# gradientpm/gvpm

Hardware: AMD Instinct MI355X
Metric: photon gather+shift evaluations per second (G-BRE 3D) (higher is better)
Workload: dtype f32; 1 GPU; BASELINE configs[1]: S-cbox + homogeneous medium, G-BRE 3D kernel, 512x512 frame, 1000000 photons/iter, 227 SPPM iters, initialScaleVolume 1.0; technique=bre3d, scene=cbox, photons_per_iter=1000000

## Files before the change

### gvpm_amd/csrc/build_chain.hip

```cpp
#include <hip/hip_runtime.h>

#include <algorithm>

#include "bundle_grid.h"
#include "device_types.h"
#include "shift_device.h"
#include "tile_walk.h"
#include "vec.h"
#include "grid_cells.h"
#include "photon_scatter.h"
#include "scan_block.h"

namespace gvpm {

__device__ __forceinline__ bool lastBlockArrives(uint32_t *ctl, uint32_t blockId, uint32_t nblocks) {
  __shared__ uint32_t isLast;
  asm volatile("s_waitcnt vmcnt(0)" ::: "memory");
  __syncthreads();
  if (threadIdx.x == 0) {
    const uint32_t S = nblocks < 64u ? nblocks : 64u;
    const uint32_t sl = blockId % S;
    const uint32_t expect = (nblocks - sl + S - 1u) / S;
    uint32_t last = 0u;
    if (atomicAdd(&ctl[1u + sl], 1u) == expect - 1u) {
      atomicExch(&ctl[1u + sl], 0u);
      if (atomicAdd(&ctl[0], 1u) == S - 1u) {
        atomicExch(&ctl[0], 0u);
        last = 1u;
      }
    }
    isLast = last;
  }
  __syncthreads();
  return isLast != 0u;
}
__device__ __forceinline__ uint32_t coherentRead(uint32_t *p) { return atomicAdd(p, 0u); }

__device__ __forceinline__ uint32_t ordCode(float f) {
  const uint32_t u = __float_as_uint(f);
  return (u >> 31) ? ~u : (u | 0x80000000u);
}
__device__ __forceinline__ float ordDecode(uint32_t o) { return __uint_as_float((o >> 31) ? (o & 0x7FFFFFFFu) : ~o); }
__global__ void chain_init_buckets_kernel(uint32_t *buckets) {
  const uint32_t t = threadIdx.x;
  buckets[t] = (t % 6u) < 3u ? 0xFFFFFFFFu : 0u;
}

__global__ __launch_bounds__(256) void chain_count_kernel(ChainArgs c) {
  __shared__ float red[6][4];
  const uint32_t b = blockIdx.x;
  if (b == 0) {
    if (threadIdx.x < 8) c.queueCtl[threadIdx.x] = 0u;
    if (threadIdx.x == 8) *c.overflowCtr = 0u;
    if (threadIdx.x == 9) c.nearExt[0] = 1u;
  }
  float mn[3] = {INFINITY, INFINITY, INFINITY}, mx[3] = {-INFINITY, -INFINITY, -INFINITY};
  const bool photons = b < c.nPhBlocks;
  if (photons) {
    const uint32_t i = b * 256u + threadIdx.x;
    if (i < c.n) {
      const float px = c.pos[3 * (size_t)i + 0], py = c.pos[3 * (size_t)i + 1], pz = c.pos[3 * (size_t)i + 2];
      mn[0] = px; mn[1] = py; mn[2] = pz;
      mx[0] = px; mx[1] = py; mx[2] = pz;
      const Grid &g = c.g;
      if (g.mode == 1) {
        const uint32_t k = bundlePhotonKey(g, px, py, pz);
        c.keys[i] = k;
        if (k == GVPM_BUNDLE_DUMP_CELL(g.dim[0])) {
          c.rank[i] = 0xFFFFFFFFu;
        } else {
          c.rank[i] = 0u;
          (void)atomicAdd(&c.sub[(size_t)(i % CELL_STRIPES) * g.ncells + k], 1u);
        }
      } else {
        const int cx = cellCoord(px, g.org[0], g.invCell, g.dim[0]);
        const int cy = cellCoord(py, g.org[1], g.invCell, g.dim[1]);
        const int cz = cellCoord(pz, g.org[2], g.invCell, g.dim[2]);
        const uint32_t k = ((uint32_t)cz * g.dim[1] + cy) * g.dim[0] + cx;
        c.keys[i] = k;
        (void)atomicAdd(&c.counts[k], 1u);
      }
    }
  } else {
    const uint32_t i = (b - c.nPhBlocks) * 256u + threadIdx.x;
    if (i < c.nsets) {
      const gvpm_camera_ray &r = c.rays[(size_t)i * 5];
      const uint32_t px = r.pixel & 0xFFFFu, py = r.pixel >> 16;
      const uint32_t tilesX = (c.width + c.tw - 1) / c.tw;
      const uint32_t tile = (py / c.th) * tilesX + px / c.tw;
      const uint32_t inTile = (py % c.th) * c.tw + px % c.tw;
      const uint32_t k = tile * (uint32_t)(c.tw * c.th) + inTile;
      c.bKeys[i] = k;
      (void)atomicAdd(&c.counts[(size_t)c.beamOff + k], 1u);
      if (GVPM_RAY_VALID(r.info)) {
#pragma unroll
        for (int k3 = 0; k3 < 3; ++k3) {
          const float e0 = r.o[k3], e1 = r.o[k3] + r.d[k3] * r.len;
          mn[k3] = fminf(e0, e1);
          mx[k3] = fmaxf(e0, e1);
        }
      }
    }
  }
  const int wave = threadIdx.x / 64, lane = threadIdx.x % 64;
#pragma unroll
  for (int k = 0; k < 3; ++k) {
    const float lo = wave_min(mn[k]), hi = wave_max(mx[k]);
    if (lane == 0) {
      red[k][wave] = lo;
      red[3 + k][wave] = hi;
    }
  }
  __syncthreads();
  if (threadIdx.x < 6) {
    const int k = threadIdx.x;
    float v = red[k][0];
    for (int w = 1; w < 4; ++w) v = k < 3 ? fminf(v, red[k][w]) : fmaxf(v, red[k][w]);
    uint32_t *slot = c.buckets + (photons ? 0u : 384u) + (b % 64u) * 6u + k;
    if (k < 3) (void)atomicMin(slot, ordCode(v));
    else (void)atomicMax(slot, ordCode(v));
  }
}

__global__ __launch_bounds__(256) void chain_stripes_kernel(const uint32_t *__restrict__ sub, uint32_t *__restrict__ prefix, uint32_t ncells,
                                                            uint32_t *__restrict__ count) {
  const uint32_t k = blockIdx.x * blockDim.x + threadIdx.x;
  if (k >= ncells) return;
  uint32_t run = 0;
#pragma unroll
  for (uint32_t st = 0; st < CELL_STRIPES; ++st) {
    prefix[(size_t)st * ncells + k] = run;
    run += sub[(size_t)st * ncells + k];
  }
  count[k] = run;
}

__global__ __launch_bounds__(256) void chain_scan_reduce_kernel(ChainArgs c) {
  __shared__ uint32_t lds[4];
  __shared__ float red[6][4];
  const uint32_t n = c.scanLen;
  {
    const uint32_t *__restrict__ counts = c.counts;
    const uint32_t base = blockIdx.x * SCAN_TILE + threadIdx.x * SCAN_PER_THREAD;
    uint32_t v = 0;
#pragma unroll
    for (uint32_t k = 0; k < SCAN_PER_THREAD; ++k)
      if (base + k < n) v += counts[base + k];
    uint32_t total;
    (void)block_scan_excl(v, lds, total);
    if (threadIdx.x == 0) (void)atomicExch(&c.blockSum[blockIdx.x], total);
  }
  if (!lastBlockArrives(c.ctl, blockIdx.x, gridDim.x)) return;
  const uint32_t nblocks = gridDim.x;
  const uint32_t per = (nblocks + SCAN_BLOCK - 1u) / SCAN_BLOCK;
  const uint32_t i0 = min(nblocks, threadIdx.x * per), i1 = min(nblocks, i0 + per);
  uint32_t mine = 0;
  for (uint32_t i = i0; i < i1; ++i) mine += coherentRead(&c.blockSum[i]);
  uint32_t total;
  uint32_t run = block_scan_excl(mine, lds, total);
  for (uint32_t i = i0; i < i1; ++i) {
    const uint32_t v = coherentRead(&c.blockSum[i]);
    c.blockSum[i] = run;
    run += v;
  }
  for (uint32_t which = 0; which < 2u; ++which) {
    float v6[6];
#pragma unroll
    for (int k = 0; k < 6; ++k) {
      float v = k < 3 ? INFINITY : -INFINITY;
      if (threadIdx.x < 64u) {
        uint32_t *slot = c.buckets + which * 384u + threadIdx.x * 6u + k;
        v = ordDecode(coherentRead(slot));
        *slot = k < 3 ? 0xFFFFFFFFu : 0u;
      }
      v6[k] = v;
    }
    const int wave = threadIdx.x / 64, lane = threadIdx.x % 64;
    __syncthreads();
#pragma unroll
    for (int k = 0; k < 3; ++k) {
      const float a = wave_min(v6[k]), b = wave_max(v6[3 + k]);
      if (lane == 0) {
        red[k][wave] = a;
        red[3 + k][wave] = b;
      }
    }
    __syncthreads();
    if (threadIdx.x < 6) {
      const int k = threadIdx.x;
      float v = red[k][0];
      for (int w = 1; w < 4; ++w) v = k < 3 ? fminf(v, red[k][w]) : fmaxf(v, red[k][w]);
      c.out6[which * 6u + k] = v;
      if (c.hostB6) c.hostB6[which * 16u + k] = v;
    }
  }
}

__global__ __launch_bounds__(256) void chain_scan_down_kernel(ChainArgs c) {
  __shared__ uint32_t lds[4];
  const uint32_t n = c.scanLen;
  uint32_t *__restrict__ counts = c.counts;
  uint32_t *__restrict__ starts = c.starts;
  const uint32_t zeroBelow = c.g.mode == 1 ? c.beamOff : 0u;
  const uint32_t base = blockIdx.x * SCAN_TILE + threadIdx.x * SCAN_PER_THREAD;
  uint32_t x[SCAN_PER_THREAD], v = 0;
#pragma unroll
  for (uint32_t k = 0; k < SCAN_PER_THREAD; ++k) {
    x[k] = base + k < n ? counts[base + k] : 0u;
    v += x[k];
  }
  uint32_t total;
  uint32_t run = c.blockSum[blockIdx.x] + block_scan_excl(v, lds, total);
#pragma unroll
  for (uint32_t k = 0; k < SCAN_PER_THREAD; ++k) {
    if (base + k < n) {
      starts[base + k] = run;
      if (x[k] && base + k < zeroBelow) counts[base + k] = 0u;
    }
    run += x[k];
  }
}

__global__ __launch_bounds__(256) void chain_mid_kernel(ChainArgs c, uint32_t nSatBlocks, uint32_t nBeamBlocks) {
  const uint32_t b = blockIdx.x;
  if (b < nSatBlocks) {
    satYBody(c.starts, c.g, c.sat, b * 256u + threadIdx.x);
    return;
  }
  const uint32_t *__restrict__ starts = c.starts;
  const uint32_t base = starts[c.beamOff];
  if (b < nSatBlocks + nBeamBlocks) {
    const uint32_t i = (b - nSatBlocks) * 256u + threadIdx.x;
    if (i < c.nsets) {
      const size_t k = (size_t)c.beamOff + c.bKeys[i];
      c.setPerm[starts[k] - base + (atomicSub(&c.counts[k], 1u) - 1u)] = i;
    }
    return;
  }
  const uint32_t t = (b - nSatBlocks - nBeamBlocks) * 256u + threadIdx.x;
  if (t <= c.ntiles) c.tileStart[t] = starts[(size_t)c.beamOff + ((size_t)t << c.tileShift)] - base;
}

struct TailArgs {
  uint32_t ntiles, target, itemCap, nPlan;
  uint4 *items;
  uint2 *itemOff;
  uint32_t *itemCount, *blockTotal;
  RawPhotons raw;
  const uint32_t *keys, *rank, *cellStart, *sub;
  uint32_t *counts;
  uint32_t *subCount;
  uint32_t n, ncells, extCap;
  uint32_t every;
  float dmax;
  NearGrid ng;
  uint32_t *nearExt, *overflow, *origIdx;
  float4 *hot, *cold;
  uint32_t *ctl;
  const uint32_t *bundleFlag;
  uint32_t *hostOut;
  uint32_t pairCapBlocks;
  uint32_t unitCap, unitPairs;
  uint32_t fullVis;
  uint32_t planGroups;
};
constexpr uint32_t TAIL_PLAN_STAGE = 128;
template <int B> constexpr size_t tailLdsBytes() {
  constexpr size_t pl = sizeof(PlanLds<B, TAIL_PLAN_STAGE>) > sizeof(PlanLdsQ<B, TAIL_PLAN_STAGE>) ? sizeof(PlanLds<B, TAIL_PLAN_STAGE>)
                                                                                                  : sizeof(PlanLdsQ<B, TAIL_PLAN_STAGE>);
  return pl > sizeof(ReorderLds) ? pl : sizeof(ReorderLds);
}
constexpr int TAIL_WPE = 6;
template <int B, int MODE> __global__ __launch_bounds__(64) __attribute__((amdgpu_waves_per_eu(TAIL_WPE, TAIL_WPE))) void chain_tail_kernel(GatherArgs a, TailArgs t) {
  __shared__ __attribute__((aligned(16))) unsigned char ldsRaw[tailLdsBytes<B>()];
  const uint32_t b = blockIdx.x, pslot = b / t.every;
  if (b % t.every == 0u && pslot < t.nPlan) {
    if (a.grid.mode != 1 && t.planGroups)
      planBodyQ<B, TAIL_PLAN_STAGE>(a, t.ntiles, t.target, t.items, t.itemCount, t.itemOff, t.blockTotal, t.itemCap, pslot, t.nPlan,
                                    *reinterpret_cast<PlanLdsQ<B, TAIL_PLAN_STAGE> *>(ldsRaw));
    else
      planBody<B, TAIL_PLAN_STAGE>(a, t.ntiles, t.target, t.items, t.itemCount, t.itemOff, t.blockTotal, t.itemCap, pslot, t.nPlan,
                                   *reinterpret_cast<PlanLds<B, TAIL_PLAN_STAGE> *>(ldsRaw));
  }
  else
    reorderBody<MODE>(t.raw, t.keys, t.rank, t.cellStart, t.n, a.cfg, a.bvh, a.tri4, a.ntri, t.dmax, t.ng, t.nearExt, t.extCap, t.hot,
                      t.cold, t.overflow, t.origIdx, t.sub, t.ncells, b - min(t.nPlan, (b + t.every - 1u) / t.every), t.counts,
                      t.subCount, *reinterpret_cast<ReorderLds *>(ldsRaw));
  if (!lastBlockArrives(t.ctl, blockIdx.x, gridDim.x)) return;
  if (threadIdx.x == 0) {
    t.hostOut[0] = coherentRead(t.blockTotal);
    t.hostOut[1] = coherentRead(t.overflow);
    t.hostOut[2] = coherentRead(t.nearExt);
    t.hostOut[3] = coherentRead(t.itemCount);
    t.hostOut[4] = t.bundleFlag ? coherentRead(const_cast<uint32_t *>(t.bundleFlag)) : 0u;
    uint32_t bad = 0u;
    if (t.pairCapBlocks != 0xFFFFFFFFu) {
      const uint32_t blocks = t.hostOut[0], nIt = t.hostOut[3];
      if (blocks > t.pairCapBlocks) bad |= 1u;
      if (nIt > t.itemCap) bad |= 2u;
      if (t.unitCap && (unsigned long long)blocks * 64ull / t.unitPairs + nIt + 64ull > (unsigned long long)t.unitCap) bad |= 4u;
      if (t.hostOut[1] != 0u && !t.fullVis) bad |= 8u;
      if (t.hostOut[4] != 0u) bad |= 16u;
    }
    t.itemCount[7] = bad;
    t.hostOut[5] = bad;
    __threadfence_system();
  }
}

template <int B>
static void launchTail(int mode, uint32_t grid, hipStream_t s, const GatherArgs &a, const TailArgs &t) {
  if (mode == 0) hipLaunchKernelGGL((chain_tail_kernel<B, 0>), dim3(grid), dim3(64), 0, s, a, t);
  else if (mode == 2) hipLaunchKernelGGL((chain_tail_kernel<B, 2>), dim3(grid), dim3(64), 0, s, a, t);
  else hipLaunchKernelGGL((chain_tail_kernel<B, 1>), dim3(grid), dim3(64), 0, s, a, t);
}

void launch_build_chain(ChainArgs c, const GatherArgs &a, const gvpm_photon_soa &raw, int beamsPerWave, uint32_t target, uint4 *items,
                        uint2 *itemOff, uint32_t itemCap, float dmax, const NearGrid &ng, uint32_t extCap, uint32_t *origIdx,
                        uint32_t *hostOut, bool initBuckets, hipStream_t s, uint32_t pairCapBlocks, uint32_t unitCap, uint32_t unitPairs,
                        bool fullVis, bool planGroups) {
  c.nPhBlocks = (c.n + 255u) / 256u;
  c.nBeamBlocks = (c.nsets + 255u) / 256u;
  if (initBuckets) hipLaunchKernelGGL(chain_init_buckets_kernel, dim3(1), dim3(768), 0, s, c.buckets);
  hipLaunchKernelGGL(chain_count_kernel, dim3(c.nPhBlocks + c.nBeamBlocks), dim3(256), 0, s, c);
  if (c.g.mode == 1)
    hipLaunchKernelGGL(chain_stripes_kernel, dim3((c.g.ncells + 255) / 256), dim3(256), 0, s, c.sub, c.sub + (size_t)CELL_STRIPES * c.g.ncells,
                       c.g.ncells, c.counts);
  const uint32_t nScan = (c.scanLen + SCAN_TILE - 1) / SCAN_TILE;
  hipLaunchKernelGGL(chain_scan_reduce_kernel, dim3(nScan), dim3(SCAN_BLOCK), 0, s, c);
  hipLaunchKernelGGL(chain_scan_down_kernel, dim3(nScan), dim3(SCAN_BLOCK), 0, s, c);
  const uint32_t nx1 = c.g.dim[0] + 1;
  const uint32_t nSat = (nx1 * (uint32_t)c.g.dim[2] + 255u) / 256u, nTile = (c.ntiles + 1u + 255u) / 256u;
  hipLaunchKernelGGL(chain_mid_kernel, dim3(nSat + c.nBeamBlocks + nTile), dim3(256), 0, s, c, nSat, c.nBeamBlocks);
  launch_sat_z(c.g, c.sat, s);
  TailArgs t{};
  t.ntiles = c.ntiles;
  t.target = target;
  t.itemCap = itemCap;
  t.planGroups = planGroups ? 1u : 0u;
  {
    const uint32_t per = (t.planGroups && c.g.mode != 1) ? (uint32_t)(64 / (beamsPerWave > 0 ? beamsPerWave : 16)) : 1u;
    const uint32_t want = (c.ntiles + per - 1u) / per;
    t.nPlan = want < 4093u ? std::max(1u, want) : 4093u;
    (void)per;
  }
  t.items = items;
  t.itemOff = itemOff;
  t.itemCount = c.queueCtl;
  t.blockTotal = c.queueCtl + 3;
  t.raw = rawOf(raw);
  t.keys = c.keys;
  t.rank = c.rank;
  t.cellStart = c.starts;
  t.sub = c.g.mode == 1 ? c.sub + (size_t)CELL_STRIPES * c.g.ncells : nullptr;
  t.subCount = c.g.mode == 1 ? c.sub : nullptr;
  t.counts = c.g.mode == 1 ? nullptr : c.counts;
  t.n = c.n;
  t.ncells = c.g.ncells;
  t.extCap = extCap;
  t.dmax = dmax;
  t.ng = ng;
  t.nearExt = c.nearExt;
  t.overflow = c.overflowCtr;
  t.origIdx = origIdx;
  t.hot = const_cast<float4 *>(a.hot);
  t.cold = const_cast<float4 *>(a.cold);
  t.ctl = c.ctl + 65;
  t.bundleFlag = a.bundleFlag;
  t.hostOut = hostOut;
  t.pairCapBlocks = pairCapBlocks;
  t.unitCap = unitCap;
  t.unitPairs = unitPairs ? unitPairs : 1u;
  t.fullVis = fullVis ? 1u : 0u;
  const int mode = a.ntri <= 64u ? 0 : (ng.start ? 2 : 1);
  const uint32_t grid = t.nPlan + (c.n + 63u) / 64u;
  t.every = std::max(1u, grid / std::max(1u, t.nPlan));
  switch (beamsPerWave) {
    case 64: launchTail<64>(mode, grid, s, a, t); break;
    case 32: launchTail<32>(mode, grid, s, a, t); break;
    default: launchTail<16>(mode, grid, s, a, t); break;
  }
}

}
```

### gvpm_amd/csrc/context.h

```cpp
#pragma once
#include <dlfcn.h>
#include <hip/hip_runtime.h>
#include <rccl/rccl.h>

#include <cmath>
#include <cstdio>
#include <cstdlib>
#include <cstring>
#include <algorithm>
#include <chrono>
#include <string>
#include <type_traits>
#include <vector>

#include "device_types.h"
#include "scan_sort.h"
#include "scene_bvh.h"

namespace gvpm {
void launch_bounds(const float *pos, uint32_t n, float *partial, int nblocks, float *out6, float *hostOut,
                   hipStream_t s, const uint32_t *word = nullptr, uint32_t *wordOut = nullptr);
void launch_export_u32(const uint32_t *a, const uint32_t *b, const uint32_t *c, const uint32_t *d, const uint32_t *e, uint32_t *hostOut,
                       hipStream_t s);
uint32_t cell_stripes();
void launch_cell_count(const float *pos, uint32_t n, const Grid &g, uint32_t *keys, uint32_t *rank, uint32_t *count, uint32_t *sub,
                       hipStream_t s, uint32_t *zeroWord = nullptr, uint32_t *oneWord = nullptr);
void launch_sat(const uint32_t *cellStart, const Grid &g, uint32_t *sat, hipStream_t s);
void launch_reorder(const gvpm_photon_soa &raw, const uint32_t *keys, const uint32_t *rank, const uint32_t *cellStart,
                    uint32_t n, const gvpm_params &cfg, const float4 *bvh, const float4 *tri4, uint32_t ntri, float dmax,
                    const NearGrid &ng, uint32_t *nearExt, uint32_t extCap, float4 *hot, float4 *cold, uint32_t *overflow,
                    uint32_t *origIdx, const uint32_t *sub, uint32_t ncells, hipStream_t s);
void launch_near_grid(const float4 *tri4, uint32_t ntri, const NearGrid &g, float reach, uint32_t *counts, uint32_t *tris, int mode,
                      hipStream_t s);
void launch_segment_start(const uint32_t *keys, uint32_t n, uint32_t nseg, uint32_t shift, uint32_t *start,
                          hipStream_t s);
void launch_bundle_fit(const gvpm_camera_ray *rays, uint32_t nsets, int pass, const Grid &g, double *out, hipStream_t s);
void launch_beam_keys(const gvpm_camera_ray *rays, uint32_t nsets, int width, int tw, int th, uint32_t *keys,
                      uint32_t *vals, hipStream_t s);
void launch_beam_count(const gvpm_camera_ray *rays, uint32_t nsets, int width, int tw, int th, uint32_t *keys,
                       uint32_t *rank, uint32_t *count, hipStream_t s);
void launch_beam_scatter(const uint32_t *keys, const uint32_t *rank, const uint32_t *start, uint32_t n,
                         uint32_t *setPerm, hipStream_t s);
void launch_tile_start(const uint32_t *start, uint32_t ntiles, uint32_t shift, uint32_t *tileStart, hipStream_t s);
void launch_beam_cold(const gvpm_photon_soa &raw, const float *endN, uint32_t n, const gvpm_params &cfg,
                      const uint32_t *subCounts, float4 *cold, float4 *aux, hipStream_t s);
void launch_shift_extent(const gvpm_camera_ray *rays, uint32_t nsets, uint32_t *extentBits, hipStream_t s);
void launch_beam_near(float4 *cold, uint32_t n, const float4 *tri4, uint32_t ntri, float r, float eps, const uint32_t *extentBits, float2 *clear, bool freeCone,
                      hipStream_t s);
void launch_beam_near_hist(const float4 *cold, uint32_t n, uint32_t ntri, uint32_t *hist, hipStream_t s);
void launch_build_chain(ChainArgs c, const GatherArgs &a, const gvpm_photon_soa &raw, int beamsPerWave, uint32_t target, uint4 *items,
                        uint2 *itemOff, uint32_t itemCap, float dmax, const NearGrid &ng, uint32_t extCap, uint32_t *origIdx,
                        uint32_t *hostOut, bool initBuckets, hipStream_t s, uint32_t pairCapBlocks = 0xFFFFFFFFu, uint32_t unitCap = 0,
                        uint32_t unitPairs = 1, bool fullVis = false, bool planGroups = true);
void launch_apply_host_shifts(const GatherArgs &a, const gvpm_host_shift *results, uint32_t n, hipStream_t s);
void launch_plan_bre(const GatherArgs &a, int beamsPerWave, uint32_t ntiles, uint32_t target, uint4 *items,
                     uint32_t *itemCount, uint2 *itemOff, uint32_t *blockTotal, uint32_t itemCap, hipStream_t stream);
uint32_t eval_unit_pairs();
void launch_traverse_bre(const GatherArgs &a, int beamsPerWave, const uint4 *items, const uint2 *itemOff,
                         const uint32_t *itemCount, uint32_t *queueHead, uint32_t *pairs, uint32_t *pairCnt,
                         uint32_t nwaves, bool persistent, hipStream_t stream, uint2 *units = nullptr, uint32_t *unitCtl = nullptr,
                         uint32_t unitCap = 0);
void launch_evaluate_primal(const GatherArgs &a, int beamsPerWave, const uint4 *items, const uint2 *itemOff,
                            const uint32_t *itemCount, uint32_t *queueHead, const uint32_t *pairs, const uint32_t *pairCnt,
                            uint32_t nwaves, hipStream_t stream);
void launch_evaluate_bre(const GatherArgs &a, int beamsPerWave, bool fullVis, const uint4 *items, const uint2 *itemOff,
                         const uint32_t *itemCount, uint32_t *queueHead, const uint32_t *pairs, const uint32_t *pairCnt,
                         uint32_t nwaves, bool persistent, hipStream_t stream, const uint2 *units = nullptr,
                         const uint32_t *unitCtl = nullptr, uint32_t unitCap = 0);
uint32_t plan_items_capacity(uint32_t nsets, uint32_t ntiles, int beamsPerWave);
void launch_exact_pass(const GatherArgs &a, unsigned long long *totals, uint32_t *hostOut, hipStream_t s);
void launch_capture_notes(const GatherArgs &a, hipStream_t s, uint32_t nblocks = 256);
void launch_apply_host_shifts_beams(const GatherArgs &a, const gvpm_host_shift *results, uint32_t n, hipStream_t s);
void launch_exact_beams(const GatherArgs &a, unsigned long long *totals, hipStream_t s);
void launch_beam_subcount(const float *p2, const float *p1, uint32_t n, float ls, uint32_t *counts, uint32_t *maxLs,
                          hipStream_t s);
void launch_beam_expand(const float *p2, const float *p1, uint32_t n, const uint32_t *counts, const uint32_t *offsets,
                        const Grid &g, uint32_t *keys, uint32_t *vals, hipStream_t s);
void launch_sub_hot(const uint32_t *sortedIds, uint32_t n, const float4 *aux, float4 *hot, uint32_t *hotFlags, hipStream_t s);
void launch_evaluate_beams(const GatherArgs &a, int beamsPerWave, bool exact, const uint2 *pairs, const uint32_t *sortedKey,
                           const uint32_t *sortedBlock, uint32_t nBlocks, uint32_t *queueHead, uint32_t nwaves,
                           hipStream_t stream);
void launch_traverse_beams(const GatherArgs &a, const uint32_t *hotFlags, int beamsPerWave, const uint4 *items,
                           const uint32_t *itemCount, uint32_t itemCap, uint32_t *queueHead, uint2 *pairs, uint32_t *pairCount,
                           uint32_t pairCap, uint32_t *blockKey, uint32_t *blockVal, uint32_t nwaves, hipStream_t stream);
void launch_evaluate_beams_split(const GatherArgs &a, uint32_t *qId, uint32_t *qMeta, float4 *qK, float *qU, uint32_t *blkCnt,
                                 uint4 *runTab, uint32_t *ctl, const uint2 *pairs, const uint32_t *sortedKey,
                                 const uint32_t *sortedBlock, uint32_t nBlocks, uint32_t *queueHead, uint32_t ncu,
                                 hipStream_t stream);
void launch_gather_vpm(const GatherArgs &a, bool fullVis, bool primal, hipStream_t stream);
void launch_vpm_find(const GatherArgs &a, const VpmSplit &sp, hipStream_t stream);
void launch_vpm_redo(const GatherArgs &a, const VpmSplit &sp, bool fullVis, uint32_t nwaves, hipStream_t stream);
void launch_vpm_eval(const GatherArgs &a, const VpmSplit &sp, bool fullVis, uint32_t wavesPerShard, hipStream_t stream);
void launch_vpm_finish(float *accum, float *iter, float *scaleVol, float *nVol, float *mvol, size_t n, float alpha,
                       uint32_t *maxScaleBits, hipStream_t stream);
void launch_accumulate(float *accum, float *iter, size_t n, uint32_t *zeroWord, hipStream_t stream);
struct PlaneArgs {
  const float4 *test;
  const float *ori, *end, *flux, *w1, *len1;
  const uint32_t *flags;
  uint32_t nplanes, planesPerItem;
};
void launch_plane_records(const PlaneArgs &pa, float4 *out, hipStream_t stream);
void launch_gather_planes(const GatherArgs &a, const PlaneArgs &pa, uint32_t ntiles, uint32_t nchunks,
                          hipStream_t stream);
void launch_finalize(float *accum, const float *iter, size_t n, int it, uint64_t nbPaths, hipStream_t s);
void launch_scale(const float *in, float *out, size_t n, float scale, hipStream_t s);
void launch_film(const float *acc, const float *emission, int w, int h, int it, int reusePrimal, float invDiv,
                 float *thr, float *dx, float *dy, hipStream_t s);
struct PoissonGraphCache {
  hipGraph_t graph = nullptr;
  hipGraphExec_t exec = nullptr;
  void *scratch = nullptr;
  int W = 0, H = 0, cgMax = 0;
  float alpha = 0.f;
};
void poisson_graph_release(PoissonGraphCache &c);
hipError_t poisson_solve_device(const gvpm_poisson_params &prm, int W, int H, const float *dx, const float *dy,
                                const float *tp, const float *direct, float *out, void *scratch,
                                PoissonGraphCache &cache, hipStream_t s);
size_t poisson_scratch_bytes(int W, int H);
}

using namespace gvpm;

template <typename T> struct DevBuf {
  T *p = nullptr;
  size_t cap = 0;
  hipError_t ensure(size_t n) {
    if (n <= cap) return hipSuccess;
    if (p) (void)hipFree(p);
    p = nullptr;
    cap = 0;
    size_t want = n + n / 2 + 64;
    hipError_t e = hipMalloc((void **)&p, want * sizeof(T));
    if (e == hipSuccess) cap = want;
    return e;
  }
  void release() {
    if (p) (void)hipFree(p);
    p = nullptr;
    cap = 0;
  }
  hipError_t reserveExact(size_t c) {
    if (c <= cap) return hipSuccess;
    if (p) (void)hipFree(p);
    p = nullptr;
    cap = 0;
    hipError_t e = hipMalloc((void **)&p, c * sizeof(T));
    if (e == hipSuccess) cap = c;
    return e;
  }
};

constexpr int PHOTON_ARRAYS = 14;
constexpr size_t PHOTON_WORDS = 30;
static inline size_t photonArrayWords(int k) { return k < 8 ? 3 : 1; }
template <typename Soa, typename F> static inline void forEachPhotonArray(Soa &s, F &&f) {
  int k = 0;
  auto each = [&](auto &...a) { (f(k++, a), ...); };
  each(s.pos, s.wi, s.flux, s.parent_pos, s.parent_n, s.prefix_w, s.parent_scat, s.parent_wi, s.parent_pdf, s.edge_pdf, s.parent_rr,
       s.parent_g, s.flags, s.path_id);
}
struct PhotonArrayPtrs {
  const void *p[PHOTON_ARRAYS];
  explicit PhotonArrayPtrs(const gvpm_photon_soa &s) {
    forEachPhotonArray(s, [&](int k, const auto *a) { p[k] = a; });
  }
};
static inline void photonArraysInBlock(gvpm_photon_soa &s, const uint32_t *base, uint64_t n) {
  forEachPhotonArray(s, [&](int k, auto &a) {
    a = reinterpret_cast<std::remove_reference_t<decltype(a)>>(base);
    base += (size_t)n * photonArrayWords(k);
  });
  s.n = n;
}

struct RcclApi {
  void *dl = nullptr;
  decltype(&ncclGetUniqueId) getUniqueId = nullptr;
  decltype(&ncclCommInitRank) commInitRank = nullptr;
  decltype(&ncclAllReduce) allReduce = nullptr;
  decltype(&ncclCommDestroy) commDestroy = nullptr;
  bool load() {
    if (dl) return true;
    dl = dlopen("librccl.so.1", RTLD_NOW | RTLD_LOCAL);
    if (!dl) dl = dlopen("librccl.so", RTLD_NOW | RTLD_LOCAL);
    if (!dl) return false;
    getUniqueId = (decltype(getUniqueId))dlsym(dl, "ncclGetUniqueId");
    commInitRank = (decltype(commInitRank))dlsym(dl, "ncclCommInitRank");
    allReduce = (decltype(allReduce))dlsym(dl, "ncclAllReduce");
    commDestroy = (decltype(commDestroy))dlsym(dl, "ncclCommDestroy");
    return getUniqueId && commInitRank && allReduce && commDestroy;
  }
};
extern RcclApi g_rccl;

#define GVPM_PHASES 3
enum : uint32_t { TRACE_HOST = 1u, TRACE_PLAN = 2u, TRACE_VIS = 4u, TRACE_EXACT = 8u, TRACE_BEAMS = 16u };

struct BuildSet {
  float builtRadius = -1.f;
  DevBuf<float4> hot, cold;
  DevBuf<uint32_t> overflowCtr;
  DevBuf<uint32_t> origIdx;
  DevBuf<uint32_t> cellStart, cellCount, cellSub, sat, keysA, keysB, valsA, valsB;
  DevBuf<uint32_t> beamCount, beamStart;
  DevBuf<float> boundsPartial, bounds6;
  Grid grid;
  SortTemp sortTmp;
  DevBuf<uint32_t> bKeysA, bKeysB, bValsA, setPerm, tileStart;
  uint32_t ntiles = 0;
  int tileW = 4, tileH = 4;
  bool scanSized = false, scanSizedChain = false;
  bool countsClean = false;
  size_t subCleanWords = 0;
  DevBuf<uint32_t> chainBuckets;
  bool bucketsInit = false;
  DevBuf<uint4> items;
  DevBuf<uint2> itemOff;
  DevBuf<uint2> planBoxes;
  DevBuf<uint32_t> queueCtl;
  DevBuf<uint32_t> pairs, pairCnt, nearExt;
  DevBuf<uint2> units;
  DevBuf<uint4> notes;
  DevBuf<uint32_t> notesCount;
  hipEvent_t traversed = nullptr;
  hipEvent_t lastUse = nullptr;
  bool used = false;
  bool lastUseValid = false;
  hipError_t mirrorFrom(const BuildSet &o) {
    hipError_t e = hipSuccess;
#define GVPM_MIRROR(X) if (e == hipSuccess) e = X.reserveExact(o.X.cap)
    GVPM_MIRROR(hot); GVPM_MIRROR(cold); GVPM_MIRROR(overflowCtr); GVPM_MIRROR(origIdx); GVPM_MIRROR(cellStart); GVPM_MIRROR(cellCount); GVPM_MIRROR(cellSub);
    GVPM_MIRROR(sat); GVPM_MIRROR(keysA); GVPM_MIRROR(keysB); GVPM_MIRROR(valsA); GVPM_MIRROR(valsB);
    GVPM_MIRROR(beamCount); GVPM_MIRROR(beamStart); GVPM_MIRROR(boundsPartial); GVPM_MIRROR(bounds6);
    GVPM_MIRROR(bKeysA); GVPM_MIRROR(bKeysB); GVPM_MIRROR(bValsA); GVPM_MIRROR(setPerm); GVPM_MIRROR(tileStart);
    GVPM_MIRROR(items); GVPM_MIRROR(itemOff); GVPM_MIRROR(planBoxes); GVPM_MIRROR(queueCtl); GVPM_MIRROR(pairs); GVPM_MIRROR(pairCnt);
    GVPM_MIRROR(nearExt); GVPM_MIRROR(chainBuckets); GVPM_MIRROR(units);
#undef GVPM_MIRROR
    return e;
  }
  void release() {
    hot.release(); cold.release(); overflowCtr.release(); origIdx.release(); cellStart.release(); cellCount.release(); cellSub.release(); sat.release();
    beamCount.release(); beamStart.release(); keysA.release(); keysB.release();
    valsA.release(); valsB.release(); boundsPartial.release(); bounds6.release(); bKeysA.release(); bKeysB.release();
    bValsA.release(); setPerm.release(); tileStart.release(); items.release(); itemOff.release(); planBoxes.release(); queueCtl.release();
    if (sortTmp.d) (void)hipFree(sortTmp.d);
    sortTmp.d = nullptr;
    sortTmp.bytes = 0;
    pairs.release(); pairCnt.release(); nearExt.release(); chainBuckets.release(); units.release(); notes.release(); notesCount.release();
    if (lastUse) (void)hipEventDestroy(lastUse);
    if (traversed) (void)hipEventDestroy(traversed);
    lastUse = traversed = nullptr;
  }
};

struct gvpm_context {
  int device = 0;
  hipStream_t stream = nullptr;
  hipStream_t streamB = nullptr;
  hipStream_t bstream = nullptr;
  hipStream_t streamC = nullptr;
  hipStream_t streamA2 = nullptr;
  bool travStream = true;
  BuildSet sets[3];
  BuildSet *bs = &sets[0];
  int setIdx = 0;
  bool beamsExact = false;
  bool bundleEnabled = false;
  bool bundleFromEnv = false;
  bool bundleAuto = false;
  int bundleState = 0, bundleViolations = 0;
  int lastGridMode = 0;
  uint32_t lastGridCells = 0;
  float bundleDiv = 2.f;
  Grid bundleGrid{};
  bool buildChain = true;
  DevBuf<uint32_t> chainCtl;
  bool planGroups = true;
  bool planBoxHandOff = true;
  bool beamsFreeCone = true;
  size_t beamPairsInit = (size_t)16 << 20;
  uint32_t beamItemsInit = 0;
  uint32_t beamItemCap = 0;
  bool pipeline = true;
  uint32_t trace = 0;
  gvpm_params cfg;
  gvpm_medium medium;
  bool haveMedium = false;
  std::string err;

  DevBuf<float4> tri4, bvh;
  uint32_t ntri = 0;
  float triMin[3] = {0, 0, 0}, triMax[3] = {0, 0, 0};
  DevBuf<uint32_t> nearGridStart, nearGridTris, nearGridCount;
  NearGrid nearGrid;
  float nearGridReach = -1.f;
  bool useNearGrid = true;

  struct PhotonSlot {
    DevBuf<uint32_t> raw;
    gvpm_photon_soa dev;
    DevBuf<uint32_t> packed;
    bool needUnpack = false;
    bool linked = false;
    hipEvent_t unpacked = nullptr;
    hipEvent_t copied = nullptr;
    hipEvent_t consumed = nullptr, consumedB = nullptr;
    bool read = false;
    int side = 0;
    DevBuf<float> endN, w1, len1;
    DevBuf<uint32_t> endNOct;
    bool octNormals = false;
  };
  enum : int { SIDE_NONE = 0, SIDE_BEAMS = 1, SIDE_PLANES = 2 };
  struct RaySlot {
    DevBuf<gvpm_camera_ray> rays;
    DevBuf<uint32_t> packed;
    DevBuf<uint32_t> compact;
    uint32_t ncompact = 0;
    bool needUnpack = false;
    hipEvent_t unpacked = nullptr;
    uint32_t nsets = 0;
    hipEvent_t copied = nullptr, freed = nullptr;
    bool read = false;
  };
  struct SampleSlot {
    DevBuf<gvpm_vpm_sample> smp;
    DevBuf<uint32_t> packed;
    uint32_t n = 0, nruns = 0;
    bool needUnpack = false;
    hipEvent_t unpacked = nullptr;
    hipEvent_t copied = nullptr, freed = nullptr;
    bool read = false;
  };
  template <typename Slot> struct StagingRing {
    Slot slot[3];
    int cur = 0, pending = -1;
    bool wait = false;
    bool ownedCur = false;
    bool fresh = false;
  };
  StagingRing<PhotonSlot> ph;
  StagingRing<RaySlot> ray;
  StagingRing<SampleSlot> smp;
  hipStream_t copyStream = nullptr;
  uint64_t reqCap = 0;
  DevBuf<gvpm_shift_request> reqHost;
  DevBuf<float4> reqCtx;
  DevBuf<uint32_t> reqCount;
  DevBuf<gvpm_host_shift> reqResults;
  DevBuf<ExEntry> exPay;
  DevBuf<uint32_t> exPayCount;
  DevBuf<uint4> exOvf;
  DevBuf<uint32_t> exOvfCount;
  bool iterClean = false;
  DevBuf<unsigned long long> exTotals;
  uint32_t exPayCap = 1u << 17;
  uint32_t exOvfCap = 1u << 20;
  uint32_t exSince = 0;
  uint32_t exFlushEvery = 8;
  bool exFlushFixed = false;
  uint32_t exSinceAtLast = 8;
  uint32_t *pinExact = nullptr;
  bool reqOutstanding = false;
  bool reqBeams = false;
  GatherArgs reqArgs;
  DevBuf<gvpm_material> materials;
  uint32_t nmaterials = 0;
  std::vector<gvpm_material> materialsHost;
  DevBuf<float4> bsdfs;
  uint32_t nbsdfs = 0;
  bool bsdfMixtures = false;
  gvpm_sensor sensor{};
  bool haveSensor = false;
  gvpm_photon_soa rawDev;
  uint32_t nph = 0;
  gvpm_photon_soa gatheredPh{};
  const gvpm_camera_ray *gatheredRays = nullptr;
  uint32_t gatheredSets = 0;
  bool haveGathered = false;
  int gatheredSide = 0;
  const float *gatheredEndN = nullptr, *gatheredW1 = nullptr, *gatheredLen1 = nullptr;
  const gvpm_vpm_sample *gatheredSamples = nullptr;
  uint32_t gatheredNSamples = 0;
  bool gatheredVpm = false;
  bool havePhotons = false, photonsDirty = false;
  bool nearOverflow = false;
  size_t nearExtWant = 0;
  float cachedB6[6] = {0, 0, 0, 0, 0, 0};
  bool haveCachedBounds = false, boundsPending = false;
  float beamB6[6] = {0, 0, 0, 0, 0, 0};
  bool haveBeamBounds = false, clipGrid = true;
  float *pinB6 = nullptr;
  uint32_t *pinCtl = nullptr;
  uint32_t vpmOrderN = 0;
  uint32_t vpmLaunches = 0;
  bool vpmNoOrder = false;
  float vpmScaleBound = 0.f;
  bool vpmPipeline = true;
  bool vpmSplit = true;
  uint32_t vpmPoolPerBatch = 4;
  uint32_t vpmRedoWaves = 256;
  uint32_t vpmEvalWaves = 12288;
  DevBuf<uint2> vpmPairs, vpmChunkMeta;
  DevBuf<uint32_t> vpmCtl, vpmStatus, vpmRedo;
  DevBuf<VpmSampleState> vpmState;
  hipEvent_t vpmFound = nullptr, vpmRedone = nullptr;
  bool beamsSplit = false;
  DevBuf<uint32_t> splitId, splitMeta, splitBlkCnt, splitCtl;
  DevBuf<float4> splitK;
  DevBuf<float> splitU;
  DevBuf<uint4> splitRuns;
  float *pinBeams = nullptr;

  const gvpm_camera_ray *raysDev = nullptr;
  uint32_t nsets = 0;
  bool haveBeams = false, beamsDirty = false;

  const float *endNDev = nullptr;
  bool haveBeamsMap = false;
  DevBuf<uint32_t> subCounts, subOffsets, beamCtl;
  DevBuf<float4> beamAux;
  DevBuf<float2> beamClear;
  uint32_t nsub = 0;
  float subLen = 0.f, maxSubLen = 0.f;

  const float *w1Dev = nullptr, *len1Dev = nullptr;
  DevBuf<float4> planeTest;
  DevBuf<uint32_t> subFlags;
  DevBuf<uint32_t> shiftExtent;
  bool beamNearStale = true;
  DevBuf<uint32_t> blockKeyA, blockKeyB, blockValA, blockValB;
  DevBuf<uint2> beamPairs;
  bool havePlanes = false;

  const gvpm_vpm_sample *samplesDev = nullptr;
  uint32_t nsamples = 0;
  bool haveSamples = false;
  DevBuf<float> scaleVol, nVol, mvol;
  DevBuf<uint32_t> maxScaleBits;
  double totalEmitted = 0;

  DevBuf<float> accum, accumAll, iter, filmOut, emission;
  bool useAll = false;
  size_t npix = 0;
  float globalScaleVolume = 1.f;
  bool sumMode = false;
  int sumIt = 0;
  DevBuf<float> accumTmp;

  DevBuf<unsigned long long> stats;
  std::vector<std::pair<hipEvent_t, hipEvent_t>> events[GVPM_PHASES];
  size_t eventsHead[GVPM_PHASES] = {0, 0, 0};
  size_t eventsCount[GVPM_PHASES] = {0, 0, 0};

  int beamsPerWave = 16;
  float cellScale = 0.f;
  uint32_t planTarget = 1536;
  bool planTargetSet = false;
  uint32_t nwaves = 2048;
  bool nwavesFromEnv = false;
  uint32_t ncu = 256;
  uint32_t nwavesTrav = 4096;
  bool persistentEval = true, persistentTrav = false;
  bool optimistic = true;
  uint32_t lastItems = 0;
  uint32_t optRefuseEvery = 0, optSteps = 0, optRefused = 0;
  bool evalUnits = true;

  DevBuf<float> poissonScratch, poissonIO;
  PoissonGraphCache poissonGraph;

  ncclComm_t comm = nullptr;
};

#define CHECK_H(h)                                \
  if (!(h)) return GVPM_ERR_INVALID_ARG;          \
  if (hipSetDevice((h)->device) != hipSuccess) {  \
    (h)->err = "hipSetDevice failed";             \
    return GVPM_ERR_HIP;                          \
  }

#define HIP_TRY(h, expr)                                                                      \
  do {                                                                                        \
    hipError_t _e = (expr);                                                                   \
    if (_e != hipSuccess) {                                                                   \
      (h)->err = std::string(#expr) + ": " + hipGetErrorString(_e);                           \
      return GVPM_ERR_HIP;                                                                    \
    }                                                                                         \
  } while (0)

static inline int fail(gvpm_context *h, int code, const char *msg) {
  if (h) h->err = msg;
  return code;
}


namespace gvpm {
void launch_unpack_photons(const uint32_t *packed, uint32_t n, const gvpm_material *table, uint32_t table_n,
                           const gvpm_photon_soa &dst, unsigned long long *bad, hipStream_t s);
void launch_unpack_rays(const uint32_t *packed, uint32_t nsets, gvpm_camera_ray *dst, hipStream_t s);
void launch_unpack_linked(const uint32_t *blob, uint32_t n, const gvpm_material *table, uint32_t table_n, const gvpm_photon_soa &dst,
                          unsigned long long *bad, hipStream_t s);
void launch_unpack_compact_rays(const gvpm_sensor &sensor, const uint32_t *compact, uint32_t ncompact, gvpm_camera_ray *dst,
                                hipStream_t s);
void launch_unpack_normals_oct(const uint32_t *codes, uint32_t n, float *dst, hipStream_t s);
void launch_expand_vpm_runs(const uint32_t *packed, uint32_t nruns, uint32_t n, gvpm_vpm_sample *dst, hipStream_t s);
}

int gvpm_join_exact(gvpm_context *h);
int joinEvalStreams(gvpm_context *h);
int flushHostShifts(gvpm_context *h);
float currentRadius(const gvpm_context *h);
```

### gvpm_amd/csrc/drivers_bre.hip

```cpp
#include "drivers.h"

namespace {

struct BreStep {
  gvpm_context *h;
  int it;
  uint64_t nbPaths;
  bool primal;
  float r;
  EventPair *evBuild = nullptr, *evTrav = nullptr, *evEval = nullptr;
  GatherArgs a;
  uint32_t itemCap = 0;
  uint32_t blocks = 0, nItems = 0;
  ChainPrep cp;
  int attempt = 0;
  bool force3D = false;
  bool rebuilt = false;
  bool chainRan = false;
  bool queued = false;
  bool prevOverflow = false;
  std::chrono::steady_clock::time_point T0;

  void lap(const char *what) {
    if (!(h->trace & TRACE_HOST)) return;
    auto t = std::chrono::steady_clock::now();
    fprintf(stderr, "[host] it=%d %-10s %8.1f us\n", it, what, std::chrono::duration<double, std::micro>(t - T0).count());
    T0 = t;
  }
  bool threeStage() const { return h->pipeline && h->travStream; }
};

int foldRunningSum(gvpm_context *h, int it) {
  h->sumMode = true;
  if (h->sumIt != 0 && it - 1 != h->sumIt) {
    const int rc = gvpm_join_exact(h);
    if (rc != GVPM_OK) return rc;
    launch_scale(h->accum.p, h->accum.p, h->npix * 27, (float)((double)(it - 1) / (double)h->sumIt), h->stream);
  }
  h->sumIt = it;
  return GVPM_OK;
}

int buildOrWait(BreStep &s) {
  gvpm_context *h = s.h;
  s.rebuilt = false;
  s.cp = ChainPrep{};
  if (h->photonsDirty || h->beamsDirty || s.r != h->bs->builtRadius) {
    h->setIdx = (h->setIdx + 1) % (s.threeStage() ? 3 : 2);
    h->bs = &h->sets[h->setIdx];
    if (h->bs->used) HIP_TRY(h, hipStreamWaitEvent(h->bstream, h->bs->lastUse, 0));
    HIP_TRY(h, hipEventRecord(s.evBuild->first, h->bstream));
    s.lap("waitevent");
    {
      int tileShift;
      uint32_t ntilesAll;
      beamTiling(h, h->beamsPerWave, s.cp.tw, s.cp.th, ntilesAll, tileShift);
      tileShift -= 3;
      const uint64_t nkeys = (uint64_t)ntilesAll << tileShift;
      s.cp.on = h->buildChain && h->nph > 0 && h->nsets > 0 && nkeys <= 0x3FFFFFF0ull;
      s.cp.nkeys = (uint32_t)nkeys;
      s.cp.tileShift = (uint32_t)tileShift;
    }
    GridBuild how;
    how.deferred = true;
    how.force3D = s.force3D;
    how.chain = &s.cp;
    int rc = buildGrid(h, s.r, how);
    s.lap("buildGrid");
    if (rc == GVPM_OK) rc = sortBeams(h, 0, &s.cp);
    s.lap("sortBeams");
    if (rc != GVPM_OK) return rc;
    h->photonsDirty = false;
    h->beamsDirty = false;
    h->bs->builtRadius = s.r;
    s.rebuilt = h->nph > 0;
  } else {
    if (h->bs->used) HIP_TRY(h, hipStreamWaitEvent(h->bstream, h->bs->lastUse, 0));
    if (h->bs->used && s.threeStage()) HIP_TRY(h, hipStreamWaitEvent(h->streamC, h->bs->lastUse, 0));
    HIP_TRY(h, hipEventRecord(s.evBuild->first, h->bstream));
  }
  return GVPM_OK;
}

int sizeItemsAndBoxes(BreStep &s) {
  gvpm_context *h = s.h;
  GatherArgs &a = s.a;
  fillArgs(h, a, s.r);
  a.iter = h->accum.p;
  a.iterScale = 1.0f / (float)s.nbPaths;
  if (!a.cfg.reserved[1] && h->cellScale <= 0.f && h->nph <= 2000000u) a.cfg.reserved[1] = 8;
  s.itemCap = plan_items_capacity(h->nsets, h->bs->ntiles, h->beamsPerWave);
  HIP_TRY(h, h->bs->items.ensure(s.itemCap));
  HIP_TRY(h, h->bs->itemOff.ensure(s.itemCap));
  if (h->planBoxHandOff) {
    const Grid &g = h->bs->grid;
    const int kmin = std::max(1, std::min(a.cfg.reserved[2] ? a.cfg.reserved[2] : 8, a.cfg.reserved[1] ? a.cfg.reserved[1] : 6));
    const uint32_t stride = (uint32_t)(std::max(386, std::max(g.dim[0], std::max(g.dim[1], g.dim[2]))) / kmin + 2);
    const size_t chunks = (size_t)h->nsets / (size_t)h->beamsPerWave + h->bs->ntiles + 2;
    if (chunks < (1u << 24) && std::max(g.dim[0], std::max(g.dim[1], g.dim[2])) < 1024) {
      HIP_TRY(h, h->bs->planBoxes.ensure(chunks * stride));
      a.planBoxes = h->bs->planBoxes.p;
      a.planBoxStride = stride;
    }
  }
  HIP_TRY(h, h->bs->queueCtl.ensure(8));
  a.bundleFlag = h->bs->queueCtl.p + 4;
  return ensurePinned(h);
}

int queueGather(BreStep &s, uint32_t blocks, uint32_t nItems, bool optimistic, bool fullVis) {
  gvpm_context *h = s.h;
  GatherArgs &a = s.a;
  const bool primal = s.primal;
  if (!optimistic) {
    HIP_TRY(h, h->bs->pairs.ensure((size_t)blocks * 64u + 64u));
    HIP_TRY(h, h->bs->pairCnt.ensure((size_t)s.itemCap * h->beamsPerWave));
  }
  int rc = nextEvents(h, &s.evTrav, 1);
  if (rc == GVPM_OK) rc = nextEvents(h, &s.evEval, 0);
  if (rc != GVPM_OK) return rc;
  const hipStream_t ts = !h->pipeline ? h->stream : (h->travStream ? h->streamC : h->streamB), es = h->stream;
  uint2 *units = nullptr;
  uint32_t unitCap = 0;
  if (h->evalUnits && h->persistentEval && !primal) {
    if (optimistic) {
      unitCap = (uint32_t)std::min<size_t>(h->bs->units.cap / 2u, 0x3FFFFFFFu);
      units = unitCap ? h->bs->units.p : nullptr;
    } else {
      const uint64_t capU = (uint64_t)blocks * 64u / eval_unit_pairs() + nItems + 64u;
      if (capU < 0x3FFFFFFFull) {
        HIP_TRY(h, h->bs->units.ensure((size_t)capU * 2u));
        unitCap = (uint32_t)std::min<size_t>(h->bs->units.cap / 2u, 0x3FFFFFFFu);
        units = h->bs->units.p;
      }
    }
  }
  if (!primal) {
    if (!h->bs->notes.p) {
      HIP_TRY(h, h->bs->notes.reserveExact(h->exOvfCap));
      HIP_TRY(h, h->bs->notesCount.ensure(4));
      HIP_TRY(h, hipMemsetAsync(h->bs->notesCount.p, 0, 4 * sizeof(uint32_t), es));
    }
    a.exOvf = h->bs->notes.p;
    a.exOvfCount = h->bs->notesCount.p;
    a.exOvfCap = h->exOvfCap;
  }
  if (optimistic && ts != h->bstream) HIP_TRY(h, hipStreamWaitEvent(ts, s.evBuild->second, 0));
  HIP_TRY(h, hipEventRecord(s.evTrav->first, ts));
  launch_traverse_bre(a, h->beamsPerWave, h->bs->items.p, h->bs->itemOff.p, h->bs->queueCtl.p, h->bs->queueCtl.p + 1,
                      h->bs->pairs.p, h->bs->pairCnt.p, h->persistentTrav ? h->nwavesTrav : nItems, h->persistentTrav || optimistic, ts,
                      units, h->bs->queueCtl.p + 5, unitCap);
  HIP_TRY(h, hipEventRecord(s.evTrav->second, ts));
  HIP_TRY(h, hipEventRecord(h->bs->traversed, ts));
  HIP_TRY(h, hipStreamWaitEvent(es, h->bs->traversed, 0));
  const bool smallShare = h->nsets > 0 && (size_t)h->nsets * 6u <= h->npix;
  const uint32_t nwEval = (h->pipeline && !h->nwavesFromEnv && h->ncu && h->nph > 2000000u && !smallShare)
                              ? std::min<uint32_t>(h->ncu * 12u, GVPM_STAT_ROWS) : h->nwaves;
  if (!primal && h->reqCap > 0 && h->cfg.use_manifold && h->bs->origIdx.p) {
    rc = armHostShiftRequests(h, a, 4, true, a.iter, a.iterScale, false, es);
    if (rc != GVPM_OK) return rc;
  }
  HIP_TRY(h, hipEventRecord(s.evEval->first, es));
  if (primal)
    launch_evaluate_primal(a, h->beamsPerWave, h->bs->items.p, h->bs->itemOff.p, h->bs->queueCtl.p, h->bs->queueCtl.p + 2,
                           h->bs->pairs.p, h->bs->pairCnt.p, std::max<uint32_t>(1u, std::min<uint32_t>(nItems, h->ncu * 16u)), es);
  else
    launch_evaluate_bre(a, h->beamsPerWave, fullVis, h->bs->items.p, h->bs->itemOff.p, h->bs->queueCtl.p,
                        h->bs->queueCtl.p + 2, h->bs->pairs.p, h->bs->pairCnt.p, h->persistentEval ? nwEval : nItems, h->persistentEval,
                        es, units, h->bs->queueCtl.p + 5, unitCap);
  HIP_TRY(h, hipEventRecord(s.evEval->second, es));
  if (!primal) launch_capture_notes(a, es);
  HIP_TRY(h, hipEventRecord(h->bs->lastUse, es));
  h->bs->lastUseValid = true;
  if (!primal) return exactAfterGather(h);
  return GVPM_OK;
}

int launchBuildAndPlan(BreStep &s) {
  gvpm_context *h = s.h;
  const ChainPrep &cp = s.cp;
  if (cp.on && s.rebuilt) {
    if (!h->chainCtl.p) {
      HIP_TRY(h, h->chainCtl.ensure(192));
      HIP_TRY(h, hipMemsetAsync(h->chainCtl.p, 0, h->chainCtl.cap * sizeof(uint32_t), h->bstream));
    }
    ChainArgs c{};
    c.pos = h->rawDev.pos;
    c.n = h->nph;
    c.g = h->bs->grid;
    c.keys = h->bs->keysA.p;
    c.rank = h->bs->valsA.p;
    c.counts = h->bs->cellCount.p;
    c.starts = h->bs->cellStart.p;
    c.beamOff = h->bs->grid.ncells + 1u;
    c.scanLen = c.beamOff + cp.nkeys + 1u;
    c.sub = cp.sub;
    HIP_TRY(h, h->bs->chainBuckets.ensure(768));
    c.buckets = h->bs->chainBuckets.p;
    c.out6 = h->bs->bounds6.p;
    c.hostB6 = h->pinB6;
    c.rays = h->raysDev;
    c.nsets = h->nsets;
    c.width = h->cfg.width;
    c.tw = cp.tw;
    c.th = cp.th;
    c.tileShift = cp.tileShift;
    c.ntiles = h->bs->ntiles;
    c.bKeys = h->bs->bKeysA.p;
    c.bRank = h->bs->bValsA.p;
    c.setPerm = h->bs->setPerm.p;
    c.tileStart = h->bs->tileStart.p;
    c.blockSum = reinterpret_cast<uint32_t *>(h->bs->sortTmp.d);
    c.ctl = h->chainCtl.p;
    c.queueCtl = h->bs->queueCtl.p;
    c.overflowCtr = h->bs->overflowCtr.p;
    c.nearExt = h->bs->nearExt.p;
    c.sat = h->bs->sat.p;
    h->boundsPending = h->haveCachedBounds;
    const bool optimistic = h->optimistic && h->pipeline && s.attempt == 0 && !s.primal && h->persistentEval && h->lastItems > 0 &&
                            h->bs->pairs.cap >= 128u && h->bs->pairCnt.cap >= (size_t)s.itemCap * h->beamsPerWave &&
                            (!h->evalUnits || h->bs->units.cap >= 2u);
    const bool fullVisOpt = !h->cfg.visibility_as_written || s.prevOverflow;
    const bool refuse = optimistic && h->optRefuseEvery > 0 && (++h->optSteps % h->optRefuseEvery) == 0;
    launch_build_chain(c, s.a, h->rawDev, h->beamsPerWave, h->planTarget, h->bs->items.p, h->bs->itemOff.p, s.itemCap, cp.dmax, h->nearGrid,
                       (uint32_t)std::min<size_t>(h->bs->nearExt.cap, 0xFFFFFF00u), cp.wantOrig ? h->bs->origIdx.p : nullptr, h->pinCtl,
                       !h->bs->bucketsInit, h->bstream,
                       optimistic ? (refuse ? 0u : (uint32_t)std::min<size_t>((h->bs->pairs.cap - 64u) / 64u, 0xFFFFFFF0u)) : 0xFFFFFFFFu,
                       optimistic && h->evalUnits ? (uint32_t)std::min<size_t>(h->bs->units.cap / 2u, 0x3FFFFFFFu) : 0u, eval_unit_pairs(),
                       fullVisOpt, h->planGroups);
    h->bs->bucketsInit = true;
    s.chainRan = true;
    if (optimistic) {
      HIP_TRY(h, hipEventRecord(s.evBuild->second, h->bstream));
      const uint32_t guess = std::min<uint32_t>(s.itemCap, h->lastItems + h->lastItems / 8u + 256u);
      const int rc = queueGather(s, 0u, guess, true, fullVisOpt);
      if (rc != GVPM_OK) return rc;
      s.queued = true;
    }
  } else {
    HIP_TRY(h, hipMemsetAsync(h->bs->queueCtl.p, 0, 8 * sizeof(uint32_t), h->bstream));
    launch_plan_bre(s.a, h->beamsPerWave, h->bs->ntiles, h->planTarget, h->bs->items.p, h->bs->queueCtl.p, h->bs->itemOff.p,
                    h->bs->queueCtl.p + 3, s.itemCap, h->bstream);
    launch_export_u32(h->bs->queueCtl.p + 3, s.rebuilt ? h->bs->overflowCtr.p : nullptr, s.rebuilt ? h->bs->nearExt.p : nullptr,
                      h->bs->queueCtl.p, h->bs->queueCtl.p + 4, h->pinCtl, h->bstream);
  }
  if (!s.queued) HIP_TRY(h, hipEventRecord(s.evBuild->second, h->bstream));
  s.lap("plan");
  return GVPM_OK;
}

int readCounters(BreStep &s, bool &retry) {
  gvpm_context *h = s.h;
  retry = false;
  HIP_TRY(h, hipStreamSynchronize(h->bstream));
  s.lap("syncB");
  s.blocks = h->pinCtl[0];
  s.nItems = h->pinCtl[3];
  if (s.queued && h->pinCtl[5] != 0u) {
    if (h->trace & TRACE_PLAN) fprintf(stderr, "[plan] optimistic step refused by the build (status %u): queued again\n", h->pinCtl[5]);
    HIP_TRY(h, hipStreamSynchronize(h->stream));
    if (s.threeStage()) HIP_TRY(h, hipStreamSynchronize(h->streamC));
    HIP_TRY(h, hipMemsetAsync(h->bs->queueCtl.p + 1, 0, 2 * sizeof(uint32_t), h->bstream));
    HIP_TRY(h, hipMemsetAsync(h->bs->queueCtl.p + 5, 0, 3 * sizeof(uint32_t), h->bstream));
    HIP_TRY(h, hipStreamSynchronize(h->bstream));
    s.queued = false;
    h->optRefused++;
  }
  if (s.a.grid.mode == 1 && h->pinCtl[4] != 0u && s.attempt == 0) {
    h->bundleState = ++h->bundleViolations > 3 ? -1 : 0;
    h->photonsDirty = true;
    h->boundsPending = false;
    s.force3D = true;
    retry = true;
  }
  return GVPM_OK;
}

int recordBuild(BreStep &s) {
  gvpm_context *h = s.h;
  h->lastGridMode = s.a.grid.mode;
  h->lastGridCells = s.a.grid.ncells;
  if (s.nItems > s.itemCap) return fail(h, GVPM_ERR_STATE, "G-BRE planner produced more work items than its bound");
  if (h->trace & TRACE_PLAN) {
    uint32_t q[4] = {0, 0, 0, 0};
    (void)hipMemcpy(q, h->bs->queueCtl.p, sizeof(q), hipMemcpyDeviceToHost);
    fprintf(stderr, "[plan] items %u staged blocks %u tiles %u sets %u; photons %u, %s %d x %d x %d cells of %g (radius %g)\n", q[0],
            s.blocks, h->bs->ntiles, h->nsets, h->nph, h->bs->grid.mode == 1 ? "bundle cells" : "grid", h->bs->grid.dim[0],
            h->bs->grid.dim[1], h->bs->grid.dim[2], (double)h->bs->grid.cell, (double)s.r);
  }
  if (s.rebuilt) {
    h->nearOverflow = h->cfg.visibility_as_written && h->pinCtl[1] != 0;
    h->nearExtWant = std::max<size_t>(h->nearExtWant, (size_t)h->pinCtl[2] + h->pinCtl[2] / 4);
    if (h->trace & TRACE_VIS)
      fprintf(stderr, "[vis] ntri %u photons %u: %u lists overflowed, extension cursor %u of %zu, fullvis %d\n", h->ntri, h->nph,
              h->pinCtl[1], h->pinCtl[2], h->bs->nearExt.cap, (int)needFullVis(h));
  }
  if (h->boundsPending) {
    h->boundsPending = false;
    for (int c = 0; c < 6; ++c)
      if (!std::isfinite(h->pinB6[c])) return fail(h, GVPM_ERR_INVALID_ARG, "non-finite photon position");
    memcpy(h->cachedB6, h->pinB6, sizeof(h->cachedB6));
  }
  if (s.rebuilt && s.chainRan) {
    bool ok = true;
    for (int c = 0; c < 6; ++c) ok = ok && std::isfinite(h->pinB6[16 + c]);
    h->haveBeamBounds = ok;
    if (ok) memcpy(h->beamB6, h->pinB6 + 16, sizeof(h->beamB6));
  }
  h->lastItems = s.nItems;
  return GVPM_OK;
}

int mirrorSets(gvpm_context *h) {
  if (h->pipeline) {
    for (int k = 0; k < (h->travStream ? 3 : 2); ++k) {
      BuildSet &other = h->sets[k];
      if (&other != h->bs && !other.used && !h->bs->used) HIP_TRY(h, other.mirrorFrom(*h->bs));
    }
  }
  h->bs->used = true;
  return GVPM_OK;
}

int buildAndPlan(BreStep &s) {
  gvpm_context *h = s.h;
  const BuildStreamGuard onBuildStream(h, h->pipeline ? h->streamB : h->stream);
  int rc = foldRunningSum(h, s.it);
  if (rc == GVPM_OK) rc = exactPrepare(h);
  for (s.attempt = 0; rc == GVPM_OK && s.attempt < 2; ++s.attempt) {
    bool retry = false;
    rc = buildOrWait(s);
    if (rc == GVPM_OK) rc = sizeItemsAndBoxes(s);
    if (rc == GVPM_OK) rc = launchBuildAndPlan(s);
    if (rc == GVPM_OK) rc = readCounters(s, retry);
    if (!retry) break;
  }
  if (rc == GVPM_OK) rc = recordBuild(s);
  return rc;
}

}

int gatherBRE(gvpm_context *h, int it, uint64_t nb_paths, bool primal) {
  BreStep s{h, it, nb_paths, primal, currentRadius(h)};
  s.prevOverflow = h->nearOverflow;
  s.T0 = std::chrono::steady_clock::now();
  int rc = nextEvents(h, &s.evBuild, 2);
  if (rc == GVPM_OK) rc = buildAndPlan(s);
  if (rc == GVPM_OK && !s.queued) rc = queueGather(s, s.blocks, s.nItems, false, needFullVis(h));
  if (rc == GVPM_OK) rc = mirrorSets(h);
  if (rc != GVPM_OK) return rc;
  HIP_TRY(h, hipGetLastError());
  s.lap("launchK");
  scaleVolumeAPA(h, it);
  return GVPM_OK;
}
```

### gvpm_amd/csrc/drivers_build.hip

```cpp
#include "drivers.h"

void beamTiling(const gvpm_context *h, int beamsPerWave, int &tw, int &th, uint32_t &ntiles, int &tileShift) {
  tw = 8;
  th = 4;
  if (beamsPerWave == 64) th = 8;
  if (beamsPerWave == 16) tw = 4;
  const uint32_t tilesX = (h->cfg.width + tw - 1) / tw, tilesY = (h->cfg.height + th - 1) / th;
  ntiles = tilesX * tilesY;
  tileShift = ilog2ceil(tw * th) + 3;
}

static int buildNearGrid(gvpm_context *h, float reach) {
  NearGrid g{};
  float ext[3], vol = 1.f;
  for (int c = 0; c < 3; ++c) {
    ext[c] = std::max(h->triMax[c] - h->triMin[c] + 2.02f * reach, 1e-6f);
    vol *= ext[c];
  }
  const float cell = std::cbrt(vol / 262144.f);
  size_t ncells = 1;
  for (int c = 0; c < 3; ++c) {
    g.dim[c] = std::max(1, std::min(256, (int)std::ceil(ext[c] / std::max(cell, 1e-9f))));
    g.org[c] = h->triMin[c] - 1.01f * reach;
    g.inv[c] = (float)g.dim[c] / ext[c];
    ncells *= (size_t)g.dim[c];
  }
  hipStream_t st = h->bstream;
  HIP_TRY(h, h->nearGridStart.ensure(ncells + 1));
  HIP_TRY(h, h->nearGridCount.ensure(ncells + 1));
  HIP_TRY(h, hipMemsetAsync(h->nearGridCount.p, 0, (ncells + 1) * sizeof(uint32_t), st));
  launch_near_grid(h->tri4.p, h->ntri, g, reach, h->nearGridCount.p, nullptr, 0, st);
  HIP_TRY(h, exclusiveSumU32(h->bs->sortTmp, h->nearGridCount.p, h->nearGridStart.p, (uint32_t)ncells + 1, st));
  uint32_t total = 0;
  HIP_TRY(h, hipMemcpyAsync(&total, h->nearGridStart.p + ncells, sizeof(uint32_t), hipMemcpyDeviceToHost, st));
  HIP_TRY(h, hipStreamSynchronize(st));
  HIP_TRY(h, h->nearGridTris.ensure((size_t)total + 1));
  HIP_TRY(h, hipMemsetAsync(h->nearGridCount.p, 0, (ncells + 1) * sizeof(uint32_t), st));
  g.start = h->nearGridStart.p;
  g.tris = h->nearGridTris.p;
  launch_near_grid(h->tri4.p, h->ntri, g, reach, h->nearGridCount.p, h->nearGridTris.p, 1, st);
  HIP_TRY(h, hipGetLastError());
  h->nearGrid = g;
  h->nearGridReach = reach;
  return GVPM_OK;
}

static int fitBundle(gvpm_context *h) {
  h->bundleState = -1;
  if (!h->nsets || !h->raysDev) return GVPM_OK;
  HIP_TRY(h, h->bs->bounds6.ensure(32));
  double *dev = reinterpret_cast<double *>(h->bs->bounds6.p);
  double o[13];
  Grid g{};
  launch_bundle_fit(h->raysDev, h->nsets, 0, g, dev, h->bstream);
  HIP_TRY(h, hipMemcpyAsync(o, dev, sizeof(o), hipMemcpyDeviceToHost, h->bstream));
  HIP_TRY(h, hipStreamSynchronize(h->bstream));
  for (int k = 0; k < 13; ++k)
    if (!std::isfinite(o[k])) return GVPM_OK;
  const double cnt = o[12];
  if (!(cnt >= 1.0)) return GVPM_OK;
  const double xx = o[0], xy = o[1], xz = o[2], yy = o[3], yz = o[4], zz = o[5];
  const double c00 = yy * zz - yz * yz, c01 = xz * yz - xy * zz, c02 = xy * yz - xz * yy;
  const double c11 = xx * zz - xz * xz, c12 = xy * xz - xx * yz, c22 = xx * yy - xy * xy;
  const double det = xx * c00 + xy * c01 + xz * c02;
  if (!(det > 1e-9 * cnt * cnt * cnt)) return GVPM_OK;
  const double C[3] = {(c00 * o[6] + c01 * o[7] + c02 * o[8]) / det, (c01 * o[6] + c11 * o[7] + c12 * o[8]) / det,
                       (c02 * o[6] + c12 * o[7] + c22 * o[8]) / det};
  double A[3] = {o[9], o[10], o[11]};
  const double len = std::sqrt(A[0] * A[0] + A[1] * A[1] + A[2] * A[2]);
  if (!(len > 0.2 * cnt)) return GVPM_OK;
  int sm = 0;
  for (int c = 0; c < 3; ++c) {
    A[c] /= len;
    if (fabs(A[c]) < fabs(A[sm])) sm = c;
  }
  double E[3] = {0, 0, 0}, U[3], V[3];
  E[sm] = 1.0;
  U[0] = A[1] * E[2] - A[2] * E[1]; U[1] = A[2] * E[0] - A[0] * E[2]; U[2] = A[0] * E[1] - A[1] * E[0];
  const double ul = std::sqrt(U[0] * U[0] + U[1] * U[1] + U[2] * U[2]);
  for (int c = 0; c < 3; ++c) U[c] /= ul;
  V[0] = A[1] * U[2] - A[2] * U[1]; V[1] = A[2] * U[0] - A[0] * U[2]; V[2] = A[0] * U[1] - A[1] * U[0];
  double c1 = 0;
  for (int c = 0; c < 3; ++c) {
    g.bo[c] = (float)C[c];
    g.ba[c] = (float)A[c];
    g.bu[c] = (float)U[c];
    g.bv[c] = (float)V[c];
    c1 += fabs(C[c]);
  }
  launch_bundle_fit(h->raysDev, h->nsets, 1, g, dev, h->bstream);
  HIP_TRY(h, hipMemcpyAsync(o, dev, sizeof(o), hipMemcpyDeviceToHost, h->bstream));
  HIP_TRY(h, hipStreamSynchronize(h->bstream));
  for (int k = 0; k < 8; ++k)
    if (!std::isfinite(o[k])) return GVPM_OK;
  if (!(o[4] > 0.15)) return GVPM_OK;
  const double scale = 1.0 + c1 + fabs(o[6]) + fabs(o[7]);
  const double res = std::sqrt(std::max(o[5], 0.0));
  if (res > 4e-6 * scale || o[6] < -4e-6 * scale) return GVPM_OK;
  g.lineTol = (float)(2.0 * res + 4e-6 * scale);
  const double px = std::max(o[1] - o[0], o[3] - o[2]) / (double)std::max(1, std::min(h->cfg.width, h->cfg.height));
  const double pad = 2.0 * px + 1e-5 * (1.0 + fabs(o[0]) + fabs(o[1]) + fabs(o[2]) + fabs(o[3]));
  g.uMin = (float)(o[0] - pad); g.uMax = (float)(o[1] + pad);
  g.vMin = (float)(o[2] - pad); g.vMax = (float)(o[3] + pad);
  g.mode = 1;
  h->bundleGrid = g;
  h->bundleState = 1;
  return GVPM_OK;
}

static Grid bundleCells(const gvpm_context *h, float r, int tileW) {
  Grid g = h->bundleGrid;
  const float range = fmaxf(g.uMax - g.uMin, g.vMax - g.vMin);
  const float tile = range * (float)tileW / (float)std::max(1, std::max(h->cfg.width, h->cfg.height));
  int G = 8;
  while (G < 512 && range / (float)G > tile / h->bundleDiv) G *= 2;
  int levels = 1;
  while ((1 << (levels - 1)) < G) ++levels;
  g.dim[0] = g.dim[1] = G;
  g.dim[2] = 2;
  g.levels = levels;
  g.ncells = (uint32_t)G * (uint32_t)G * 2u;
  g.s0 = range / (float)G;
  g.invS0 = 1.f / g.s0;
  g.radius = r;
  g.org[0] = g.org[1] = g.org[2] = 0.f;
  g.cell = g.s0;
  g.invCell = g.invS0;
  return g;
}

static int photonBounds(gvpm_context *h, const GridBuild &how, bool chain, float b6[6], float &ext) {
  const uint32_t n = h->nph;
  const bool deferred = how.deferred;
  const float *knownB6 = how.knownB6;
  const int nblocks = 1024;
  HIP_TRY(h, h->bs->boundsPartial.ensure(nblocks * 6));
  HIP_TRY(h, h->bs->bounds6.ensure(32));
  {
    const int rcp = ensurePinned(h);
    if (rcp != GVPM_OK) return rcp;
  }
  const bool defer = deferred && h->haveCachedBounds;
  if (!knownB6 && !(chain && defer))
    launch_bounds(h->rawDev.pos, n, h->bs->boundsPartial.p, nblocks, h->bs->bounds6.p, defer ? h->pinB6 : nullptr,
                  h->bstream);
  if (knownB6) {
    memcpy(b6, knownB6, 6 * sizeof(float));
    memcpy(h->cachedB6, b6, 6 * sizeof(float));
    h->haveCachedBounds = true;
  } else if (defer) {
    h->boundsPending = true;
    memcpy(b6, h->cachedB6, 6 * sizeof(float));
  } else {
    HIP_TRY(h, hipMemcpyAsync(b6, h->bs->bounds6.p, 6 * sizeof(float), hipMemcpyDeviceToHost, h->bstream));
    HIP_TRY(h, hipStreamSynchronize(h->bstream));
    memcpy(h->cachedB6, b6, 6 * sizeof(float));
    h->haveCachedBounds = true;
  }
  ext = 0.f;
  for (int c = 0; c < 3; ++c) {
    if (!std::isfinite(b6[c]) || !std::isfinite(b6[3 + c])) return fail(h, GVPM_ERR_INVALID_ARG, "non-finite photon position");
    ext = fmaxf(ext, b6[3 + c] - b6[c]);
  }
  return GVPM_OK;
}

static int sizeGrid(gvpm_context *h, float r, const GridBuild &how, float b6[6], float ext, Grid &g) {
  const uint32_t n = h->nph;
  const bool deferred = how.deferred;
  const float cellScale0 = h->cellScale > 0.f ? h->cellScale : (deferred && n <= 2000000u ? 1.5f : 1.0f);
  if (deferred && h->clipGrid && h->haveBeamBounds) {
    float lo[3], hi[3], cell = cellScale0 * r;
    for (int pass = 0; pass < 2; ++pass) {
      const float pad = 1.01f * r + 2.f * cell;
      float e = 0.f;
      for (int c = 0; c < 3; ++c) {
        lo[c] = fmaxf(b6[c], h->beamB6[c] - pad);
        hi[c] = fminf(b6[3 + c], h->beamB6[3 + c] + pad);
        if (!(lo[c] <= hi[c])) lo[c] = hi[c] = fminf(fmaxf(h->beamB6[c], b6[c]), b6[3 + c]);
        e = fmaxf(e, hi[c] - lo[c]);
      }
      cell = fmaxf(cellScale0 * r, e / 384.f);
      ext = e;
    }
    for (int c = 0; c < 3; ++c) {
      b6[c] = lo[c];
      b6[3 + c] = hi[c];
    }
  }
  g = Grid{};
  const float cellScale = cellScale0;
  float cell = fmaxf(cellScale * r, ext / 384.f);
  if (!(cell > 0.f)) cell = 1.f;
  g.cell = cell;
  g.invCell = 1.f / cell;
  uint64_t nc = 1;
  for (int c = 0; c < 3; ++c) {
    g.org[c] = b6[c] - 0.5f * cell;
    g.dim[c] = (int)floorf((b6[3 + c] - g.org[c]) * g.invCell) + 2;
    nc *= (uint64_t)g.dim[c];
  }
  if (nc > 0x7FFFFFFFull) return fail(h, GVPM_ERR_INVALID_ARG, "grid too large");
  g.ncells = (uint32_t)nc;
  if (deferred && !h->bundleFromEnv && h->bundleAuto) {
    const size_t twice = (size_t)h->nsets * 2u;
    const bool sharded = h->nsets > 0 && (h->bundleEnabled ? twice * 5u <= h->npix * 6u : twice * 5u <= h->npix * 4u);
    if (sharded != h->bundleEnabled) {
      h->bundleEnabled = sharded;
      if (sharded && h->bundleState < 0) h->bundleState = 0;
    }
  }
  if (deferred && h->bundleEnabled && h->bundleState >= 0 && !how.force3D) {
    if (h->bundleState == 0) {
      const int rcf = fitBundle(h);
      if (rcf != GVPM_OK) return rcf;
    }
    if (h->bundleState == 1) g = bundleCells(h, r, h->beamsPerWave == 16 ? 4 : 8);
  }
  return GVPM_OK;
}

static int cellArrays(gvpm_context *h, const Grid &g, bool deferred, bool chain, const ChainPrep *cp, uint32_t *&sub) {
  const uint32_t n = h->nph;
  HIP_TRY(h, h->bs->keysA.ensure(n));
  HIP_TRY(h, h->bs->valsA.ensure(n));
  HIP_TRY(h, h->bs->hot.ensure(n));
  HIP_TRY(h, h->bs->cold.ensure((size_t)n * GVPM_REC_QUADS));
  const size_t worstCells = (size_t)386 * 386 * 386 + 2;
  const size_t keyRoom = chain ? (size_t)cp->nkeys + 4u : 0u;
  {
    const uint32_t *was = h->bs->cellCount.p;
    HIP_TRY(h, h->bs->cellCount.ensure(std::max((size_t)g.ncells + 2, worstCells) + keyRoom));
    if (h->bs->cellCount.p != was) h->bs->countsClean = false;
  }
  HIP_TRY(h, h->bs->cellStart.ensure(std::max((size_t)g.ncells + 2, worstCells) + keyRoom));
  if (!h->bs->scanSized || (chain && !h->bs->scanSizedChain)) {
    HIP_TRY(h, reserveScanTemp(h->bs->sortTmp, (uint32_t)std::min<size_t>(worstCells + keyRoom, 0x7FFFFFF0u)));
    h->bs->scanSized = true;
    h->bs->scanSizedChain = chain;
  }
  if (chain) {
    if (!h->bs->countsClean) HIP_TRY(h, hipMemsetAsync(h->bs->cellCount.p, 0, h->bs->cellCount.cap * sizeof(uint32_t), h->bstream));
    h->bs->countsClean = true;
  } else {
    HIP_TRY(h, hipMemsetAsync(h->bs->cellCount.p, 0, ((size_t)g.ncells + 1) * sizeof(uint32_t), h->bstream));
    h->bs->countsClean = false;
  }
  sub = nullptr;
  if (g.mode == 1) {
    const size_t subWords = (size_t)cell_stripes() * g.ncells;
    const uint32_t *was = h->bs->cellSub.p;
    HIP_TRY(h, h->bs->cellSub.ensure(subWords * (chain ? 2u : 1u)));
    if (!chain || h->bs->cellSub.p != was || h->bs->subCleanWords != subWords)
      HIP_TRY(h, hipMemsetAsync(h->bs->cellSub.p, 0, subWords * sizeof(uint32_t), h->bstream));
    h->bs->subCleanWords = chain ? subWords : 0u;
    sub = h->bs->cellSub.p;
  }
  HIP_TRY(h, h->bs->overflowCtr.ensure(2));
  const size_t extWant = std::min<size_t>(std::max<size_t>((size_t)n * 8u + 4096u, h->nearExtWant), 0xFFFFFF00u);
  HIP_TRY(h, h->bs->nearExt.ensure(extWant));
  if (!chain) {
    launch_cell_count(h->rawDev.pos, n, g, h->bs->keysA.p, h->bs->valsA.p, h->bs->cellCount.p, sub, h->bstream, h->bs->overflowCtr.p,
                      h->bs->nearExt.p);
    HIP_TRY(h, exclusiveSumU32(h->bs->sortTmp, h->bs->cellCount.p, h->bs->cellStart.p, g.ncells + 1, h->bstream));
  }
  if (deferred) {
    const size_t satCells = (size_t)(g.dim[0] + 1) * (g.dim[1] + 1) * (g.dim[2] + 1);
    HIP_TRY(h, h->bs->sat.ensure(std::max(satCells, (size_t)387 * 387 * 387)));
    if (!chain) launch_sat(h->bs->cellStart.p, g, h->bs->sat.p, h->bstream);
  }
  return GVPM_OK;
}

int buildGrid(gvpm_context *h, float r, const GridBuild &how) {
  const uint32_t n = h->nph;
  const bool deferred = how.deferred;
  ChainPrep *cp = how.chain;
  h->boundsPending = false;
  const bool chain = cp && cp->on && n > 0;
  if (cp) cp->on = chain;
  if (n == 0) {
    h->bs->grid = Grid{{0, 0, 0}, 1.f, 1.f, {1, 1, 1}, 1};
    HIP_TRY(h, h->bs->cellStart.ensure(2));
    HIP_TRY(h, hipMemsetAsync(h->bs->cellStart.p, 0, 2 * sizeof(uint32_t), h->bstream));
    return GVPM_OK;
  }
  float b6[6], ext = 0.f;
  Grid g{};
  uint32_t *sub = nullptr;
  int rc = photonBounds(h, how, chain, b6, ext);
  if (rc == GVPM_OK) rc = sizeGrid(h, r, how, b6, ext, g);
  if (rc != GVPM_OK) return rc;
  h->bs->grid = g;
  rc = cellArrays(h, g, deferred, chain, cp, sub);
  if (rc != GVPM_OK) return rc;
  float diag2 = 0.f;
  for (int c = 0; c < 3; ++c) {
    const float lo = fminf(b6[c], h->ntri ? h->triMin[c] : b6[c]), hi = fmaxf(b6[3 + c], h->ntri ? h->triMax[c] : b6[3 + c]);
    diag2 += (hi - lo) * (hi - lo);
  }
  const float lmax = 1.25f * sqrtf(diag2) + 8.f * r + 1e-3f;
  const float dmax = h->cfg.shadow_epsilon * lmax * 1.01f + 1e-6f;
  if (h->ntri > 64u && h->useNearGrid && !(dmax <= h->nearGridReach)) {
    if (h->bstream != h->stream) HIP_TRY(h, hipStreamSynchronize(h->stream));
    if (h->streamA2) HIP_TRY(h, hipStreamSynchronize(h->streamA2));
    const int rcg = buildNearGrid(h, dmax * 1.5f);
    if (rcg != GVPM_OK) return rcg;
  }
  const bool wantOrig = h->reqCap > 0 && h->cfg.use_manifold;
  if (wantOrig) HIP_TRY(h, h->bs->origIdx.ensure((size_t)n + 1));
  if (chain) {
    cp->dmax = dmax;
    cp->wantOrig = wantOrig;
    cp->sub = sub;
    h->nearOverflow = false;
    return GVPM_OK;
  }
  launch_reorder(h->rawDev, h->bs->keysA.p, h->bs->valsA.p, h->bs->cellStart.p, n, h->cfg, h->bvh.p, h->tri4.p, h->ntri, dmax,
                 h->nearGrid, h->bs->nearExt.p, (uint32_t)std::min<size_t>(h->bs->nearExt.cap, 0xFFFFFF00u), h->bs->hot.p,
                 h->bs->cold.p, h->bs->overflowCtr.p, wantOrig ? h->bs->origIdx.p : nullptr, sub, g.ncells, h->bstream);
  HIP_TRY(h, hipGetLastError());
  h->nearOverflow = false;
  if (!deferred && h->cfg.visibility_as_written) {
    launch_export_u32(h->bs->overflowCtr.p, nullptr, nullptr, nullptr, nullptr, h->pinCtl, h->bstream);
    HIP_TRY(h, hipStreamSynchronize(h->bstream));
    h->nearOverflow = h->pinCtl[0] != 0;
  }
  return GVPM_OK;
}

int sortBeams(gvpm_context *h, int beamsPerWave, const ChainPrep *cp) {
  const uint32_t n = h->nsets;
  if (!beamsPerWave) beamsPerWave = h->beamsPerWave;
  int tw, th, tileShift;
  uint32_t ntilesAll;
  beamTiling(h, beamsPerWave, tw, th, ntilesAll, tileShift);
  h->bs->ntiles = ntilesAll;
  h->bs->tileW = tw;
  h->bs->tileH = th;
  HIP_TRY(h, h->bs->tileStart.ensure((size_t)h->bs->ntiles + 2));
  HIP_TRY(h, h->bs->bKeysA.ensure(n + 1));
  HIP_TRY(h, h->bs->bValsA.ensure(n + 1));
  HIP_TRY(h, h->bs->setPerm.ensure(n + 1));
  if (cp && cp->on) return GVPM_OK;
  if (n) {
    const uint64_t nkeys = (uint64_t)h->bs->ntiles << tileShift;
    if (nkeys > 0x7FFFFFF0ull) return fail(h, GVPM_ERR_INVALID_ARG, "film too large for the beam sort");
    HIP_TRY(h, h->bs->beamCount.ensure(nkeys + 2));
    HIP_TRY(h, h->bs->beamStart.ensure(nkeys + 2));
    HIP_TRY(h, hipMemsetAsync(h->bs->beamCount.p, 0, (nkeys + 1) * sizeof(uint32_t), h->bstream));
    launch_beam_count(h->raysDev, n, h->cfg.width, tw, th, h->bs->bKeysA.p, h->bs->bValsA.p, h->bs->beamCount.p, h->bstream);
    HIP_TRY(h, exclusiveSumU32(h->bs->sortTmp, h->bs->beamCount.p, h->bs->beamStart.p, (uint32_t)nkeys + 1, h->bstream));
    launch_beam_scatter(h->bs->bKeysA.p, h->bs->bValsA.p, h->bs->beamStart.p, n, h->bs->setPerm.p, h->bstream);
    launch_tile_start(h->bs->beamStart.p, h->bs->ntiles, (uint32_t)tileShift, h->bs->tileStart.p, h->bstream);
  } else {
    HIP_TRY(h, hipMemsetAsync(h->bs->tileStart.p, 0, ((size_t)h->bs->ntiles + 1) * sizeof(uint32_t), h->bstream));
  }
  HIP_TRY(h, hipGetLastError());
  return GVPM_OK;
}
```

### gvpm_amd/csrc/grid_build.hip

```cpp
#include <hip/hip_runtime.h>

#include "bundle_grid.h"
#include "device_types.h"
#include "shift_device.h"
#include "tile_walk.h"
#include "vec.h"
#include "grid_cells.h"
#include "photon_scatter.h"

namespace gvpm {

__global__ __launch_bounds__(256) void bounds_kernel(const float *__restrict__ pos, uint32_t n, float *partial) {
  __shared__ float red[6][4];
  float mn[3] = {INFINITY, INFINITY, INFINITY}, mx[3] = {-INFINITY, -INFINITY, -INFINITY};
  for (uint32_t i = blockIdx.x * blockDim.x + threadIdx.x; i < n; i += gridDim.x * blockDim.x) {
#pragma unroll
    for (int c = 0; c < 3; ++c) {
      const float v = pos[3 * (size_t)i + c];
      mn[c] = fminf(mn[c], v);
      mx[c] = fmaxf(mx[c], v);
    }
  }
  const int wave = threadIdx.x / 64, lane = threadIdx.x % 64;
#pragma unroll
  for (int c = 0; c < 3; ++c) {
    const float a = wave_min(mn[c]), b = wave_max(mx[c]);
    if (lane == 0) {
      red[c][wave] = a;
      red[3 + c][wave] = b;
    }
  }
  __syncthreads();
  if (threadIdx.x < 6) {
    const int c = threadIdx.x;
    float v = red[c][0];
    for (int w = 1; w < (int)(blockDim.x / 64u); ++w) v = c < 3 ? fminf(v, red[c][w]) : fmaxf(v, red[c][w]);
    partial[blockIdx.x * 6 + c] = v;
  }
}

__global__ void bounds_final_kernel(const float *partial, int nblocks, float *out6, float *hostOut, const uint32_t *word,
                                    uint32_t *wordOut) {
  const int lane = threadIdx.x;
  float lo[3] = {INFINITY, INFINITY, INFINITY}, hi[3] = {-INFINITY, -INFINITY, -INFINITY};
  for (int b = lane; b < nblocks; b += 64)
    for (int c = 0; c < 3; ++c) {
      lo[c] = fminf(lo[c], partial[b * 6 + c]);
      hi[c] = fmaxf(hi[c], partial[b * 6 + 3 + c]);
    }
  for (int c = 0; c < 3; ++c) {
    lo[c] = wave_min(lo[c]);
    hi[c] = wave_max(hi[c]);
  }
  if (lane == 0)
    for (int c = 0; c < 3; ++c) {
      out6[c] = lo[c];
      out6[3 + c] = hi[c];
      if (hostOut) {
        hostOut[c] = lo[c];
        hostOut[3 + c] = hi[c];
      }
    }
  if (lane == 0 && word && wordOut) wordOut[0] = word[0];
}

__global__ void export_u32_kernel(const uint32_t *a, const uint32_t *b, const uint32_t *c, const uint32_t *d,
                                  const uint32_t *e, uint32_t *hostOut) {
  if (threadIdx.x == 0) {
    hostOut[0] = a ? *a : 0u;
    hostOut[1] = b ? *b : 0u;
    hostOut[2] = c ? *c : 0u;
    hostOut[3] = d ? *d : 0u;
    hostOut[4] = e ? *e : 0u;
    __threadfence_system();
  }
}


__global__ __launch_bounds__(256) void cell_count_kernel(const float *__restrict__ pos, uint32_t n, Grid g,
                                                         uint32_t *keys, uint32_t *rank, uint32_t *count, uint32_t *sub,
                                                         uint32_t *zeroWord, uint32_t *oneWord) {
  const uint32_t i = blockIdx.x * blockDim.x + threadIdx.x;
  if (i == 0) {
    if (zeroWord) *zeroWord = 0u;
    if (oneWord) *oneWord = 1u;
  }
  if (i >= n) return;
  uint32_t k;
  if (g.mode == 1) {
    k = bundlePhotonKey(g, pos[3 * (size_t)i + 0], pos[3 * (size_t)i + 1], pos[3 * (size_t)i + 2]);
    keys[i] = k;
    if (k == GVPM_BUNDLE_DUMP_CELL(g.dim[0])) rank[i] = 0xFFFFFFFFu;
    else if (sub) rank[i] = atomicAdd(&sub[(size_t)(i % CELL_STRIPES) * g.ncells + k], 1u);
    else rank[i] = atomicAdd(&count[k], 1u);
    return;
  }
  const int cx = cellCoord(pos[3 * (size_t)i + 0], g.org[0], g.invCell, g.dim[0]);
  const int cy = cellCoord(pos[3 * (size_t)i + 1], g.org[1], g.invCell, g.dim[1]);
  const int cz = cellCoord(pos[3 * (size_t)i + 2], g.org[2], g.invCell, g.dim[2]);
  k = ((uint32_t)cz * g.dim[1] + cy) * g.dim[0] + cx;
  keys[i] = k;
  rank[i] = atomicAdd(&count[k], 1u);
}
__global__ __launch_bounds__(256) void cell_stripes_kernel(uint32_t *sub, uint32_t ncells, uint32_t *count) {
  const uint32_t k = blockIdx.x * blockDim.x + threadIdx.x;
  if (k >= ncells) return;
  uint32_t run = 0;
#pragma unroll
  for (uint32_t st = 0; st < CELL_STRIPES; ++st) {
    const uint32_t c = sub[(size_t)st * ncells + k];
    sub[(size_t)st * ncells + k] = run;
    run += c;
  }
  count[k] = run;
}

__global__ __launch_bounds__(256) void sat_y_kernel(const uint32_t *__restrict__ cellStart, Grid g, uint32_t *sat) {
  satYBody(cellStart, g, sat, blockIdx.x * blockDim.x + threadIdx.x);
}
__global__ __launch_bounds__(256) void sat_z_kernel(Grid g, uint32_t *sat) {
  const uint32_t t = blockIdx.x * blockDim.x + threadIdx.x;
  const uint32_t nx1 = g.dim[0] + 1, ny1 = g.dim[1] + 1;
  if (t >= nx1 * ny1) return;
  const size_t layer = (size_t)nx1 * ny1;
  uint32_t run = 0;
#pragma unroll 8
  for (int z = 0; z < g.dim[2]; ++z) {
    const uint32_t v = sat[(size_t)z * layer + t];
    sat[(size_t)z * layer + t] = run;
    run += v;
  }
  sat[(size_t)g.dim[2] * layer + t] = run;
}

template <int MODE>
__global__ __launch_bounds__(64) void reorder_kernel(RawPhotons r, const uint32_t *__restrict__ keys,
                                                      const uint32_t *__restrict__ rank,
                                                      const uint32_t *__restrict__ cellStart, uint32_t n,
                                                      gvpm_params cfg, const float4 *bvh, const float4 *tri4,
                                                      uint32_t ntri, float dmax, NearGrid ng, uint32_t *nearExt,
                                                      uint32_t extCap, float4 *hot, float4 *cold, uint32_t *overflow,
                                                      uint32_t *origIdx, const uint32_t *__restrict__ sub, uint32_t ncells) {
  __shared__ ReorderLds L;
  reorderBody<MODE>(r, keys, rank, cellStart, n, cfg, bvh, tri4, ntri, dmax, ng, nearExt, extCap, hot, cold, overflow, origIdx, sub,
                    ncells, blockIdx.x, nullptr, nullptr, L);
}

__global__ __launch_bounds__(64) void near_grid_kernel(const float4 *__restrict__ tri4, uint32_t ntri, NearGrid g, float reach,
                                                       uint32_t *counts, uint32_t *tris, int mode) {
  const uint32_t i = blockIdx.x;
  if (i >= ntri) return;
  const float4 t0 = tri4[3 * (size_t)i], t1 = tri4[3 * (size_t)i + 1], t2 = tri4[3 * (size_t)i + 2];
  const f3 a = mk3(t0.x, t0.y, t0.z), e1 = mk3(t1.x, t1.y, t1.z), e2 = mk3(t2.x, t2.y, t2.z), n = mk3(t0.w, t1.w, t2.w);
  int lo[3], hi[3];
  float cs[3];
#pragma unroll
  for (int k = 0; k < 3; ++k) {
    const float ak = comp(a, k), bk = comp(e1, k), ck = comp(e2, k);
    const float l = ak + fminf(0.f, fminf(bk, ck)) - reach * 1.001f, h = ak + fmaxf(0.f, fmaxf(bk, ck)) + reach * 1.001f;
    cs[k] = 1.f / g.inv[k];
    lo[k] = max(0, (int)floorf((l - g.org[k]) * g.inv[k]) - 1);
    hi[k] = min(g.dim[k] - 1, (int)floorf((h - g.org[k]) * g.inv[k]) + 1);
  }
  const float slab = reach * 1.001f + 0.5f * 1.001f * (fabsf(n.x) * cs[0] + fabsf(n.y) * cs[1] + fabsf(n.z) * cs[2]) + 1e-6f * (cs[0] + cs[1] + cs[2]);
  const bool flat = n.x == 0.f && n.y == 0.f && n.z == 0.f;
  const int nx = hi[0] - lo[0] + 1, ny = hi[1] - lo[1] + 1, nz = hi[2] - lo[2] + 1;
  if (nx <= 0 || ny <= 0 || nz <= 0) return;
  const long long ncell = (long long)nx * ny * nz;
  for (long long q = threadIdx.x; q < ncell; q += blockDim.x) {
        const int x = lo[0] + (int)(q % nx), y = lo[1] + (int)((q / nx) % ny), z = lo[2] + (int)(q / ((long long)nx * ny));
        const f3 c = mk3(g.org[0] + ((float)x + 0.5f) * cs[0], g.org[1] + ((float)y + 0.5f) * cs[1], g.org[2] + ((float)z + 0.5f) * cs[2]);
        if (!flat && fabsf(dot(n, c - a)) > slab + cs[0] + cs[1] + cs[2]) continue;
        const uint32_t cell = ((uint32_t)z * (uint32_t)g.dim[1] + (uint32_t)y) * (uint32_t)g.dim[0] + (uint32_t)x;
        if (mode == 0) atomicAdd(&counts[cell], 1u);
        else tris[g.start[cell] + atomicAdd(&counts[cell], 1u)] = i;
  }
}
void launch_near_grid(const float4 *tri4, uint32_t ntri, const NearGrid &g, float reach, uint32_t *counts, uint32_t *tris, int mode,
                      hipStream_t s) {
  if (ntri) hipLaunchKernelGGL(near_grid_kernel, dim3(ntri), dim3(64), 0, s, tri4, ntri, g, reach, counts, tris, mode);
}

__global__ __launch_bounds__(256) void segment_start_kernel(const uint32_t *__restrict__ keys, uint32_t n,
                                                            uint32_t nseg, uint32_t shift, uint32_t *start) {
  const uint32_t c = blockIdx.x * blockDim.x + threadIdx.x;
  if (c > nseg) return;
  uint32_t lo = 0, hi = n;
  while (lo < hi) {
    const uint32_t mid = (lo + hi) >> 1;
    if ((keys[mid] >> shift) < c) lo = mid + 1;
    else hi = mid;
  }
  start[c] = lo;
}

void launch_bounds(const float *pos, uint32_t n, float *partial, int nblocks, float *out6, float *hostOut,
                   hipStream_t s, const uint32_t *word, uint32_t *wordOut) {
  hipLaunchKernelGGL(bounds_kernel, dim3(nblocks), dim3(64), 0, s, pos, n, partial);
  hipLaunchKernelGGL(bounds_final_kernel, dim3(1), dim3(64), 0, s, partial, nblocks, out6, hostOut, word, wordOut);
}

void launch_export_u32(const uint32_t *a, const uint32_t *b, const uint32_t *c, const uint32_t *d, const uint32_t *e,
                       uint32_t *hostOut, hipStream_t s) {
  hipLaunchKernelGGL(export_u32_kernel, dim3(1), dim3(64), 0, s, a, b, c, d, e, hostOut);
}

__global__ __launch_bounds__(1024) void bundle_fit_kernel(const gvpm_camera_ray *__restrict__ rays, uint32_t nsets, int pass, Grid g,
                                                          double *out) {
  constexpr int NV = 13;
  __shared__ double red[NV][16];
  double v[NV];
  auto kind = [&](int k) { return pass == 0 ? 0 : ((k == 0 || k == 2 || k == 4 || k == 6) ? 1 : (k < 8 ? 2 : 0)); };
  for (int k = 0; k < NV; ++k) v[k] = kind(k) == 0 ? 0.0 : (kind(k) == 1 ? (double)INFINITY : -(double)INFINITY);
  for (uint32_t i = threadIdx.x; i < nsets; i += blockDim.x) {
    const gvpm_camera_ray &r = rays[(size_t)i * 5];
    if (!GVPM_RAY_VALID(r.info)) continue;
    const double dx = r.d[0], dy = r.d[1], dz = r.d[2];
    if (pass == 0) {
      const double ox = r.o[0], oy = r.o[1], oz = r.o[2];
      const double od = ox * dx + oy * dy + oz * dz;
      v[0] += 1.0 - dx * dx; v[1] -= dx * dy; v[2] -= dx * dz;
      v[3] += 1.0 - dy * dy; v[4] -= dy * dz; v[5] += 1.0 - dz * dz;
      v[6] += ox - dx * od; v[7] += oy - dy * od; v[8] += oz - dz * od;
      v[9] += dx; v[10] += dy; v[11] += dz;
      v[12] += 1.0;
    } else {
      const double dA = dx * g.ba[0] + dy * g.ba[1] + dz * g.ba[2];
      const double inv = 1.0 / fmax(dA, 1e-30);
      const double u = (dx * g.bu[0] + dy * g.bu[1] + dz * g.bu[2]) * inv;
      const double w = (dx * g.bv[0] + dy * g.bv[1] + dz * g.bv[2]) * inv;
      const double wx = (double)r.o[0] - g.bo[0], wy = (double)r.o[1] - g.bo[1], wz = (double)r.o[2] - g.bo[2];
      const double sd = wx * dx + wy * dy + wz * dz;
      const double px = wx - sd * dx, py = wy - sd * dy, pz = wz - sd * dz;
      v[0] = fmin(v[0], u); v[1] = fmax(v[1], u);
      v[2] = fmin(v[2], w); v[3] = fmax(v[3], w);
      v[4] = fmin(v[4], dA);
      v[5] = fmax(v[5], px * px + py * py + pz * pz);
      v[6] = fmin(v[6], sd);
      v[7] = fmax(v[7], sd);
    }
  }
  const int wave = threadIdx.x >> 6, lane = threadIdx.x & 63;
  for (int k = 0; k < NV; ++k) {
    double x = v[k];
    for (int o = 32; o > 0; o >>= 1) {
      const double y = __shfl_xor(x, o, 64);
      x = kind(k) == 0 ? x + y : (kind(k) == 1 ? fmin(x, y) : fmax(x, y));
    }
    if (lane == 0) red[k][wave] = x;
  }
  __syncthreads();
  if (threadIdx.x < NV) {
    const int k = threadIdx.x;
    double x = red[k][0];
    for (int w = 1; w < (int)(blockDim.x >> 6); ++w) x = kind(k) == 0 ? x + red[k][w] : (kind(k) == 1 ? fmin(x, red[k][w]) : fmax(x, red[k][w]));
    out[k] = x;
  }
}
void launch_bundle_fit(const gvpm_camera_ray *rays, uint32_t nsets, int pass, const Grid &g, double *out, hipStream_t s) {
  hipLaunchKernelGGL(bundle_fit_kernel, dim3(1), dim3(1024), 0, s, rays, nsets, pass, g, out);
}

void launch_sat_z(const Grid &g, uint32_t *sat, hipStream_t s) {
  const uint32_t nx1 = g.dim[0] + 1, ny1 = g.dim[1] + 1;
  hipLaunchKernelGGL(sat_z_kernel, dim3((nx1 * ny1 + 255) / 256), dim3(256), 0, s, g, sat);
}
void launch_sat(const uint32_t *cellStart, const Grid &g, uint32_t *sat, hipStream_t s) {
  const uint32_t nx1 = g.dim[0] + 1;
  hipLaunchKernelGGL(sat_y_kernel, dim3((nx1 * g.dim[2] + 255) / 256), dim3(256), 0, s, cellStart, g, sat);
  launch_sat_z(g, sat, s);
}

uint32_t cell_stripes() { return CELL_STRIPES; }
void launch_cell_count(const float *pos, uint32_t n, const Grid &g, uint32_t *keys, uint32_t *rank, uint32_t *count, uint32_t *sub,
                       hipStream_t s, uint32_t *zeroWord, uint32_t *oneWord) {
  if (g.mode != 1) sub = nullptr;
  hipLaunchKernelGGL(cell_count_kernel, dim3((n + 255) / 256), dim3(256), 0, s, pos, n, g, keys, rank, count, sub, zeroWord, oneWord);
  if (sub) hipLaunchKernelGGL(cell_stripes_kernel, dim3((g.ncells + 255) / 256), dim3(256), 0, s, sub, g.ncells, count);
}

void launch_reorder(const gvpm_photon_soa &raw, const uint32_t *keys, const uint32_t *rank, const uint32_t *cellStart,
                    uint32_t n, const gvpm_params &cfg, const float4 *bvh, const float4 *tri4, uint32_t ntri, float dmax,
                    const NearGrid &ng, uint32_t *nearExt, uint32_t extCap, float4 *hot, float4 *cold, uint32_t *overflow,
                    uint32_t *origIdx, const uint32_t *sub, uint32_t ncells, hipStream_t s) {
  const RawPhotons r = rawOf(raw);
#define GVPM_REORDER(M) \
  hipLaunchKernelGGL(reorder_kernel<M>, dim3((n + 63) / 64), dim3(64), 0, s, r, keys, rank, cellStart, n, cfg, bvh, tri4, ntri, \
                     dmax, ng, nearExt, extCap, hot, cold, overflow, origIdx, sub, ncells)
  if (ntri <= 64u) GVPM_REORDER(0);
  else if (ng.start) GVPM_REORDER(2);
  else GVPM_REORDER(1);
#undef GVPM_REORDER
}

void launch_segment_start(const uint32_t *keys, uint32_t n, uint32_t nseg, uint32_t shift, uint32_t *start,
                          hipStream_t s) {
  hipLaunchKernelGGL(segment_start_kernel, dim3((nseg + 1 + 255) / 256), dim3(256), 0, s, keys, n, nseg, shift, start);
}

}
```

### gvpm_amd/csrc/gvpm_api.hip

```cpp
#include "bsdf_table.h"
#include "context.h"
#include <cfloat>

RcclApi g_rccl;

static const char *validateParams(const gvpm_params *p) {
  if (p->abi_version != GVPM_ABI_VERSION) return "abi_version mismatch";
  if (p->width <= 0 || p->height <= 0 || p->width > 65535 || p->height > 65535) return "bad film size";
  if (p->vol_technique < GVPM_VOL_BRE2D || p->vol_technique > GVPM_VOL_PLANE0D) return "unknown vol_technique";
  const bool use3D = p->vol_technique == GVPM_DISTANCE || p->vol_technique == GVPM_VOL_BRE3D ||
                     (p->vol_technique >= GVPM_BEAM_BEAM_3D_NAIVE && p->vol_technique <= GVPM_BEAM_BEAM_3D_OPTIMIZED);
  if (p->use_shift_null && !use3D && p->vol_technique != GVPM_BEAM_BEAM_1D)
    return "Not possible to shift null without using 3D kernel";
  if (p->max_depth <= 1 && p->max_depth != -1 && p->max_depth != 0) return "Maximum depth must be set to \"2\" or higher!";
  if (!(p->bsphere_radius > 0.f)) return "bsphere_radius must be positive";
  if (!(p->epsilon > 0.f) || !(p->shadow_epsilon > 0.f)) return "epsilon / shadow_epsilon must be positive";
  if (!std::isfinite(p->alpha) || !(p->alpha > 0.f) || p->alpha > 1.f) return "alpha must be in (0, 1]";
  if (p->vol_technique == GVPM_VOL_PLANE0D && p->min_depth < 2) return "Impossible to use plane with minDepth smaller than 2";
  if (!p->no_medium_shift) return "noMediumShift=false is not supported (shiftPhotonMedium is SAssert(false))";
  return nullptr;
}

extern "C" {

int gvpm_abi_version(void) { return GVPM_ABI_VERSION; }

const char *gvpm_last_error(const gvpm_context *h) { return h ? h->err.c_str() : "null handle"; }

int gvpm_create(const gvpm_params *params, int device, gvpm_context **out) {
  if (!params || !out) return GVPM_ERR_INVALID_ARG;
  *out = nullptr;
  if (validateParams(params)) {
    const char *m = validateParams(params);
    return (strstr(m, "shift null") || strstr(m, "noMediumShift")) ? GVPM_ERR_UNSUPPORTED : GVPM_ERR_INVALID_ARG;
  }
  int ndev = 0;
  if (hipGetDeviceCount(&ndev) != hipSuccess || ndev <= 0 || device < 0 || device >= ndev) return GVPM_ERR_NO_DEVICE;
  if (hipSetDevice(device) != hipSuccess) return GVPM_ERR_NO_DEVICE;
  gvpm_context *h = new gvpm_context();
  h->device = device;
  h->cfg = *params;
  int prA = 0, prB = 1, prC = -1;
  {
    int least = 0, greatest = 0;
    if (hipDeviceGetStreamPriorityRange(&least, &greatest) == hipSuccess) {
      prB = std::min(prB, least);
      prC = std::max(prC, greatest);
    }
  }
  if (const char *e = getenv("GVPM_STREAM_PRIORITIES")) (void)sscanf(e, "%d,%d,%d", &prA, &prB, &prC);
  if (hipStreamCreateWithPriority(&h->stream, hipStreamNonBlocking, prA) != hipSuccess ||
      hipStreamCreateWithPriority(&h->streamB, hipStreamNonBlocking, prB) != hipSuccess ||
      hipStreamCreateWithPriority(&h->streamC, hipStreamNonBlocking, prC) != hipSuccess ||
      hipStreamCreateWithPriority(&h->streamA2, hipStreamNonBlocking, prA) != hipSuccess ||
      hipEventCreateWithFlags(&h->sets[0].lastUse, hipEventDisableTiming) != hipSuccess ||
      hipEventCreateWithFlags(&h->sets[1].lastUse, hipEventDisableTiming) != hipSuccess ||
      hipEventCreateWithFlags(&h->sets[2].lastUse, hipEventDisableTiming) != hipSuccess ||
      hipEventCreateWithFlags(&h->sets[0].traversed, hipEventDisableTiming) != hipSuccess ||
      hipEventCreateWithFlags(&h->sets[1].traversed, hipEventDisableTiming) != hipSuccess ||
      hipEventCreateWithFlags(&h->sets[2].traversed, hipEventDisableTiming) != hipSuccess) {
    gvpm_destroy(h);
    return GVPM_ERR_HIP;
  }
  if (hipStreamCreateWithFlags(&h->copyStream, hipStreamNonBlocking) != hipSuccess) {
    gvpm_destroy(h);
    return GVPM_ERR_HIP;
  }
  for (int k = 0; k < 3; ++k)
    for (hipEvent_t *e : {&h->ph.slot[k].copied, &h->ph.slot[k].unpacked, &h->ph.slot[k].consumed, &h->ph.slot[k].consumedB,
                          &h->ray.slot[k].copied, &h->ray.slot[k].unpacked, &h->ray.slot[k].freed,
                          &h->smp.slot[k].copied, &h->smp.slot[k].unpacked, &h->smp.slot[k].freed})
      if (hipEventCreateWithFlags(e, hipEventDisableTiming) != hipSuccess) {
        gvpm_destroy(h);
        return GVPM_ERR_HIP;
      }
  h->bstream = h->stream;
  if (const char *e = getenv("GVPM_BEAMS_PER_WAVE")) {
    int v = atoi(e);
    if (v == 16 || v == 32 || v == 64) h->beamsPerWave = v;
  }
  h->cfg.reserved[0] = 0;
  if (const char *e = getenv("GVPM_DEBUG_FLAGS")) h->cfg.reserved[0] = atoi(e);
  if (const char *e = getenv("GVPM_TRAV_PREFILTER"))
    if (!atoi(e)) h->cfg.reserved[0] |= 128;
  if (const char *e = getenv("GVPM_RECORD_PREFETCH")) h->cfg.reserved[0] |= atoi(e) ? 64 : 32;
  h->cfg.reserved[1] = 0;
  if (const char *e = getenv("GVPM_SLAB_LAYERS")) h->cfg.reserved[1] = atoi(e);
  h->cfg.reserved[2] = 0;
  if (const char *e = getenv("GVPM_SLAB_LAYERS_X")) h->cfg.reserved[2] = atoi(e);
  h->cfg.reserved[4] = h->cfg.reserved[5] = 0;
  if (const char *e = getenv("GVPM_EXACT_ALL")) h->cfg.reserved[4] = atoi(e) ? 1 : 0;
  if (h->cfg.reserved[4]) h->exPayCap = 1u << 20;
  h->cfg.reserved[3] = 0;
  if (const char *e = getenv("GVPM_COALESCE_AT")) h->cfg.reserved[3] = atoi(e);
  if (const char *e = getenv("GVPM_PLAN_TARGET")) {
    int v = atoi(e);
    if (v >= 64 && v <= (1 << 24)) h->planTarget = (uint32_t)v, h->planTargetSet = true;
  }
  {
    hipDeviceProp_t prop;
    if (hipGetDeviceProperties(&prop, device) == hipSuccess && prop.multiProcessorCount > 0)
      h->nwaves = (uint32_t)prop.multiProcessorCount * 8u, h->ncu = (uint32_t)prop.multiProcessorCount;
    if (const char *e = getenv("GVPM_WAVES_PER_CU")) {
      int v = atoi(e);
      if (v >= 1 && v <= 32 && prop.multiProcessorCount > 0) h->nwaves = (uint32_t)prop.multiProcessorCount * v, h->nwavesFromEnv = true;
    }
  }
  h->nwavesTrav = h->ncu * 16u;
  if (const char *e = getenv("GVPM_TRAV_WAVES_PER_CU")) {
    int v = atoi(e);
    if (v >= 1 && v <= 32) h->nwavesTrav = h->ncu * (uint32_t)v;
  }
  {
    if (h->nwavesTrav > GVPM_STAT_ROWS) h->nwavesTrav = GVPM_STAT_ROWS;
    if (h->nwaves > GVPM_STAT_ROWS) h->nwaves = GVPM_STAT_ROWS;
  }
  if (const char *e = getenv("GVPM_PIPELINE")) h->pipeline = atoi(e) != 0;
  if (!h->pipeline && !getenv("GVPM_WAVES_PER_CU") && h->ncu) h->nwaves = std::min<uint32_t>(h->ncu * 12u, GVPM_STAT_ROWS);
  if (const char *e = getenv("GVPM_PERSISTENT")) h->persistentEval = (atoi(e) & 1) != 0, h->persistentTrav = (atoi(e) & 2) != 0;
  if (const char *e = getenv("GVPM_NEAR_GRID")) h->useNearGrid = atoi(e) != 0;
  if (const char *e = getenv("GVPM_TRAV_STREAM")) h->travStream = atoi(e) != 0;
  if (const char *e = getenv("GVPM_BEAMS_FP64")) h->beamsExact = atoi(e) != 0;
  if (const char *e = getenv("GVPM_BEAMS_FREE_CONE")) h->beamsFreeCone = atoi(e) != 0;
  if (const char *e = getenv("GVPM_PLAN_BOXES")) h->planBoxHandOff = atoi(e) != 0;
  if (const char *e = getenv("GVPM_BUILD_CHAIN")) h->buildChain = atoi(e) != 0;
  if (const char *e = getenv("GVPM_PLAN_GROUPS")) h->planGroups = atoi(e) != 0;
  if (const char *e = getenv("GVPM_EVAL_UNITS")) h->evalUnits = atoi(e) != 0;
  if (const char *e = getenv("GVPM_EVAL_GENERIC"))
    if (atoi(e)) h->cfg.reserved[0] |= GVPM_EVAL_FORCE_GENERIC;
  if (const char *e = getenv("GVPM_OPTIMISTIC")) h->optimistic = atoi(e) != 0;
  if (const char *e = getenv("GVPM_OPTIMISTIC_REFUSE")) h->optRefuseEvery = (uint32_t)std::max(0, atoi(e));
  if (const char *e = getenv("GVPM_CLIP_GRID")) h->clipGrid = atoi(e) != 0;
  if (getenv("GVPM_TRACE_HOST")) h->trace |= TRACE_HOST;
  if (getenv("GVPM_TRACE_PLAN")) h->trace |= TRACE_PLAN;
  if (getenv("GVPM_TRACE_VIS")) h->trace |= TRACE_VIS;
  if (getenv("GVPM_TRACE_EXACT")) h->trace |= TRACE_EXACT;
  if (getenv("GVPM_BEAMS_TRACE")) h->trace |= TRACE_BEAMS;
  if (const char *e = getenv("GVPM_VPM_ORDER")) h->vpmNoOrder = atoi(e) == 0;
  if (const char *e = getenv("GVPM_VPM_SPLIT")) h->vpmSplit = atoi(e) != 0;
  if (const char *e = getenv("GVPM_VPM_PIPELINE")) h->vpmPipeline = atoi(e) != 0;
  if (const char *e = getenv("GVPM_VPM_POOL")) h->vpmPoolPerBatch = (uint32_t)std::max(0, atoi(e));
  if (const char *e = getenv("GVPM_VPM_EVAL_WAVES")) h->vpmEvalWaves = (uint32_t)std::max(64, atoi(e));
  if (const char *e = getenv("GVPM_VPM_REDO_WAVES")) h->vpmRedoWaves = (uint32_t)std::max(1, atoi(e));
  if (const char *e = getenv("GVPM_BEAMS_SPLIT")) h->beamsSplit = atoi(e) != 0;
  if (const char *e = getenv("GVPM_BUNDLE_AUTO")) h->bundleAuto = atoi(e) != 0;
  if (const char *e = getenv("GVPM_BUNDLE")) {
    h->bundleEnabled = atoi(e) != 0;
    h->bundleFromEnv = true;
  }
  if (const char *e = getenv("GVPM_BUNDLE_DIV")) {
    const float v = (float)atof(e);
    if (v >= 0.25f && v <= 16.f) h->bundleDiv = v;
  }
  if (const char *e = getenv("GVPM_BEAM_PAIRS_INIT")) {
    const long long v = atoll(e);
    if (v >= 64 && v <= ((long long)1 << 31)) h->beamPairsInit = (size_t)v;
  }
  if (const char *e = getenv("GVPM_BEAM_ITEMS_INIT")) {
    const long long v = atoll(e);
    if (v >= 1 && v <= ((long long)1 << 30)) h->beamItemsInit = (uint32_t)v;
  }
  if (const char *e = getenv("GVPM_EXACT_EVERY")) {
    const int v = atoi(e);
    if (v >= 1 && v <= 1000000) {
      h->exFlushEvery = (uint32_t)v;
      h->exFlushFixed = true;
    }
  }
  if (const char *e = getenv("GVPM_CELL_SCALE")) {
    float v = (float)atof(e);
    if (v >= 0.25f && v <= 8.f) h->cellScale = v;
  }
  h->npix = (size_t)params->width * params->height;
  if (h->accum.ensure(h->npix * 27) != hipSuccess || h->iter.ensure(h->npix * 27) != hipSuccess ||
      h->stats.ensure(8 * GVPM_STAT_ROWS) != hipSuccess || h->scaleVol.ensure(h->npix) != hipSuccess ||
      h->nVol.ensure(h->npix) != hipSuccess || h->mvol.ensure(h->npix) != hipSuccess ||
      h->maxScaleBits.ensure(2) != hipSuccess || h->exTotals.ensure(32) != hipSuccess ||
      h->exPayCount.ensure(4) != hipSuccess || h->exOvfCount.ensure(4) != hipSuccess) {
    gvpm_destroy(h);
    return GVPM_ERR_HIP;
  }
  *out = h;
  int rc = gvpm_reset(h);
  if (rc != GVPM_OK) {
    gvpm_destroy(h);
    *out = nullptr;
  }
  return rc;
}

int gvpm_destroy(gvpm_context *h) {
  if (!h) return GVPM_ERR_INVALID_ARG;
  (void)hipSetDevice(h->device);
  if (h->stream) (void)hipStreamSynchronize(h->stream);
  if (h->comm && g_rccl.commDestroy) g_rccl.commDestroy(h->comm);
  for (auto &v : h->events)
    for (auto &e : v) {
      (void)hipEventDestroy(e.first);
      (void)hipEventDestroy(e.second);
    }
  if (h->streamB) (void)hipStreamSynchronize(h->streamB);
  if (h->streamC) (void)hipStreamSynchronize(h->streamC);
  if (h->streamA2) (void)hipStreamSynchronize(h->streamA2);
  for (BuildSet &b : h->sets) b.release();
  h->tri4.release(); h->bvh.release();
  for (auto &ps : h->ph.slot) {
    ps.raw.release();
    ps.packed.release();
    ps.endN.release(); ps.w1.release(); ps.len1.release(); ps.endNOct.release();
    if (ps.unpacked) (void)hipEventDestroy(ps.unpacked);
    if (ps.copied) (void)hipEventDestroy(ps.copied);
    if (ps.consumed) (void)hipEventDestroy(ps.consumed);
    if (ps.consumedB) (void)hipEventDestroy(ps.consumedB);
  }
  for (auto &rs : h->ray.slot) {
    rs.rays.release();
    rs.packed.release();
    rs.compact.release();
    if (rs.unpacked) (void)hipEventDestroy(rs.unpacked);
    if (rs.copied) (void)hipEventDestroy(rs.copied);
    if (rs.freed) (void)hipEventDestroy(rs.freed);
  }
  for (auto &ss : h->smp.slot) {
    ss.smp.release();
    ss.packed.release();
    if (ss.unpacked) (void)hipEventDestroy(ss.unpacked);
    if (ss.copied) (void)hipEventDestroy(ss.copied);
    if (ss.freed) (void)hipEventDestroy(ss.freed);
  }
  if (h->copyStream) (void)hipStreamDestroy(h->copyStream);
  h->materials.release();
  h->reqHost.release(); h->reqCtx.release(); h->reqCount.release(); h->reqResults.release();
  h->subCounts.release(); h->subOffsets.release();
  h->beamCtl.release(); h->beamAux.release(); h->beamClear.release();
  h->nearGridStart.release(); h->nearGridTris.release(); h->nearGridCount.release();
  h->planeTest.release(); h->beamPairs.release(); h->subFlags.release(); h->shiftExtent.release();
  h->blockKeyA.release(); h->blockKeyB.release(); h->blockValA.release(); h->blockValB.release();
  h->scaleVol.release(); h->nVol.release(); h->mvol.release(); h->maxScaleBits.release();
  poisson_graph_release(h->poissonGraph);
  h->accumTmp.release();
  h->chainCtl.release();
  h->poissonScratch.release(); h->poissonIO.release();
  h->accum.release(); h->accumAll.release(); h->iter.release(); h->filmOut.release(); h->emission.release(); h->stats.release();
  h->exPay.release(); h->exPayCount.release(); h->exOvf.release(); h->exOvfCount.release(); h->exTotals.release();
  if (h->pinB6) (void)hipHostFree(h->pinB6);
  if (h->pinExact) (void)hipHostFree(h->pinExact);
  if (h->pinBeams) (void)hipHostFree(h->pinBeams);
  h->splitId.release(); h->splitMeta.release(); h->splitBlkCnt.release(); h->splitCtl.release(); h->splitK.release();
  h->splitU.release(); h->splitRuns.release();
  if (h->stream) (void)hipStreamDestroy(h->stream);
  if (h->streamB) (void)hipStreamDestroy(h->streamB);
  if (h->streamC) (void)hipStreamDestroy(h->streamC);
  if (h->streamA2) (void)hipStreamDestroy(h->streamA2);
  h->vpmPairs.release(); h->vpmChunkMeta.release(); h->vpmCtl.release(); h->vpmStatus.release(); h->vpmRedo.release(); h->vpmState.release();
  if (h->vpmFound) (void)hipEventDestroy(h->vpmFound);
  if (h->vpmRedone) (void)hipEventDestroy(h->vpmRedone);
  delete h;
  return GVPM_OK;
}

int gvpm_reset(gvpm_context *h) {
  CHECK_H(h);
  {
    const int rcj = joinEvalStreams(h);
    if (rcj != GVPM_OK) return rcj;
  }
  h->reqOutstanding = false;
  h->reqBeams = false;
  if (h->reqCount.p) HIP_TRY(h, hipMemsetAsync(h->reqCount.p, 0, 8, h->stream));
  h->vpmOrderN = 0;
  h->vpmLaunches = 0;
  HIP_TRY(h, hipMemsetAsync(h->exPayCount.p, 0, 4 * sizeof(uint32_t), h->stream));
  HIP_TRY(h, hipMemsetAsync(h->exOvfCount.p, 0, 4 * sizeof(uint32_t), h->stream));
  h->exSince = 0;
  HIP_TRY(h, hipMemsetAsync(h->exTotals.p, 0, 32 * sizeof(unsigned long long), h->stream));
  HIP_TRY(h, hipMemsetAsync(h->accum.p, 0, h->npix * 27 * sizeof(float), h->stream));
  HIP_TRY(h, hipMemsetAsync(h->stats.p, 0, 8 * GVPM_STAT_ROWS * sizeof(unsigned long long), h->stream));
  h->globalScaleVolume = h->cfg.initial_scale_volume;
  h->sumIt = 0;
  h->bundleState = 0;
  h->bundleViolations = 0;
  HIP_TRY(h, hipMemsetAsync(h->iter.p, 0, h->npix * 27 * sizeof(float), h->stream));
  HIP_TRY(h, hipMemsetAsync(h->mvol.p, 0, h->npix * sizeof(float), h->stream));
  h->iterClean = true;
  for (size_t &u : h->eventsHead) u = 0;
  for (size_t &u : h->eventsCount) u = 0;
  h->useAll = false;
  h->totalEmitted = 0;
  {
    std::vector<float> init(h->npix, h->cfg.initial_scale_volume);
    HIP_TRY(h, hipMemcpyAsync(h->scaleVol.p, init.data(), h->npix * sizeof(float), hipMemcpyHostToDevice, h->stream));
    HIP_TRY(h, hipMemsetAsync(h->nVol.p, 0, h->npix * sizeof(float), h->stream));
    uint32_t bits;
    const float sc = h->cfg.initial_scale_volume;
    memcpy(&bits, &sc, 4);
    HIP_TRY(h, hipMemcpyAsync(h->maxScaleBits.p, &bits, 4, hipMemcpyHostToDevice, h->stream));
    HIP_TRY(h, hipStreamSynchronize(h->stream));
    h->vpmScaleBound = sc;
    if (h->pinCtl) h->pinCtl[32] = 0u;
  }
  return GVPM_OK;
}

int gvpm_upload_scene(gvpm_context *h, const gvpm_triangles *t) {
  CHECK_H(h);
  if (int rcj = gvpm_join_exact(h)) return rcj;
  if (!t || (t->n && (!t->v0 || !t->e1 || !t->e2))) return fail(h, GVPM_ERR_INVALID_ARG, "null triangle arrays");
  BvhBuild bvh;
  buildSceneBvh(t->v0, t->e1, t->e2, t->n, bvh);
  std::vector<float> packed(12 * (size_t)t->n + 12, 0.f);
  for (uint32_t k = 0; k < t->n; ++k) {
    const uint32_t i = bvh.order[k];
    const float *a = t->v0 + 3 * (size_t)i, *b = t->e1 + 3 * (size_t)i, *c = t->e2 + 3 * (size_t)i;
    float n[3] = {b[1] * c[2] - b[2] * c[1], b[2] * c[0] - b[0] * c[2], b[0] * c[1] - b[1] * c[0]};
    const float l = sqrtf(n[0] * n[0] + n[1] * n[1] + n[2] * n[2]);
    for (int q = 0; q < 3; ++q) n[q] = l > 0.f ? n[q] / l : 0.f;
    float *o = packed.data() + 12 * (size_t)k;
    for (int q = 0; q < 3; ++q) {
      o[q] = a[q];
      o[4 + q] = b[q];
      o[8 + q] = c[q];
      o[4 * q + 3] = n[q];
    }
  }
  HIP_TRY(h, h->tri4.ensure(3 * (size_t)t->n + 3));
  HIP_TRY(h, h->bvh.ensure(bvh.nodes.size() / 4 + 2));
  HIP_TRY(h, hipMemcpyAsync(h->tri4.p, packed.data(), packed.size() * sizeof(float), hipMemcpyHostToDevice, h->stream));
  HIP_TRY(h, hipMemcpyAsync(h->bvh.p, bvh.nodes.data(), bvh.nodes.size() * sizeof(float), hipMemcpyHostToDevice,
                            h->stream));
  HIP_TRY(h, hipStreamSynchronize(h->stream));
  h->ntri = t->n;
  for (int c = 0; c < 3; ++c) {
    h->triMin[c] = INFINITY;
    h->triMax[c] = -INFINITY;
  }
  for (uint32_t i = 0; i < t->n; ++i)
    for (int c = 0; c < 3; ++c) {
      const float a = t->v0[3 * i + c], b = a + t->e1[3 * i + c], d = a + t->e2[3 * i + c];
      h->triMin[c] = fminf(h->triMin[c], fminf(a, fminf(b, d)));
      h->triMax[c] = fmaxf(h->triMax[c], fmaxf(a, fmaxf(b, d)));
    }
  h->photonsDirty = h->havePhotons;
  h->nearGridReach = -1.f;
  h->nearGrid = NearGrid();
  return GVPM_OK;
}

int gvpm_upload_medium(gvpm_context *h, const gvpm_medium *m) {
  CHECK_H(h);
  if (int rcj = gvpm_join_exact(h)) return rcj;
  if (!m) return fail(h, GVPM_ERR_INVALID_ARG, "null medium");
  bool finite = std::isfinite(m->g) && std::isfinite(m->medium_sampling_weight);
  for (int c = 0; c < 3; ++c) finite = finite && std::isfinite(m->sigma_a[c]) && std::isfinite(m->sigma_s[c]) && std::isfinite(m->sigma_t[c]);
  if (!finite) return fail(h, GVPM_ERR_INVALID_ARG, "medium: every field must be finite");
  if (m->sigma_t[0] != m->sigma_t[1] || m->sigma_t[0] != m->sigma_t[2])
    return fail(h, GVPM_ERR_UNSUPPORTED, "Not possible to have different albedo values...");
  if (!(m->sigma_t[0] > 0.f)) return fail(h, GVPM_ERR_INVALID_ARG, "sigma_t must be positive");
  if (!(fabsf(m->g) < 1.f)) return fail(h, GVPM_ERR_INVALID_ARG, "medium: the HG mean cosine g must lie in (-1, 1)");
  if (!(m->medium_sampling_weight > 0.f && m->medium_sampling_weight <= 1.f))
    return fail(h, GVPM_ERR_INVALID_ARG, "medium: medium_sampling_weight must lie in (0, 1]");
  for (int c = 0; c < 3; ++c) {
    if (m->sigma_s[c] < 0.f) return fail(h, GVPM_ERR_INVALID_ARG, "medium: sigma_s must not be negative");
    if (m->sigma_s[c] > m->sigma_t[c]) return fail(h, GVPM_ERR_INVALID_ARG, "medium: sigma_s must not exceed sigma_t");
  }
  h->medium = *m;
  h->haveMedium = true;
  return GVPM_OK;
}

static int checkBsdfTail(gvpm_context *h, const gvpm_bsdf *table, uint32_t i, uint32_t n, const char *missing, const char *invalid) {
  const int kind = table[i].kind, tail = gvpm::bsdfTailEntries(kind);
  if (n - i <= (uint32_t)tail) return fail(h, GVPM_ERR_INVALID_ARG, missing);
  float raw[16 * GVPM_RTRANS_ENTRIES];
  memcpy(raw, &table[i + 1], tail * sizeof(gvpm_bsdf));
  for (int j = 0; j < 16 * tail; ++j)
    if (!gvpm::bsdfTailWordValid(kind, j, raw[j])) return fail(h, GVPM_ERR_INVALID_ARG, invalid);
  return GVPM_OK;
}

static int checkBsdf(gvpm_context *h, const gvpm_bsdf *table, uint32_t i, uint32_t n, const std::vector<uint8_t> &isHead) {
  using namespace gvpm;
  const gvpm_bsdf &b = table[i];
  const bool weightOk = bsdfWeightValid(b.specular_sampling_weight);
  const bool ward = b.kind == GVPM_BSDF_WARD || b.kind == GVPM_BSDF_WARD_ANISO;
  const bool conductor = b.kind == GVPM_BSDF_ROUGHCONDUCTOR || b.kind == GVPM_BSDF_ROUGHCONDUCTOR_ANISO;
  if (b.kind == GVPM_BSDF_PHONG) {
    if (!(b.exponent >= 0.f) || !weightOk) return fail(h, GVPM_ERR_INVALID_ARG, "Phong: exponent >= 0 and a sampling weight in [0, 1]");
  } else if (ward || conductor) {
    const bool aniso = bsdfTailEntries(b.kind) != 0;
    float alphaV = b.exponent;
    if (aniso) {
      if (int rc = checkBsdfTail(h, table, i, n, "anisotropic Ward / rough conductor: the frame entry behind the head is missing",
                                 "frame entry: tangent and alphaV are +0 or normal floats; 12 zero words behind them"))
        return rc;
      float fr[4];
      memcpy(fr, &table[i + 1], sizeof fr);
      const double sl = std::sqrt((double)fr[0] * fr[0] + (double)fr[1] * fr[1] + (double)fr[2] * fr[2]);
      if (!(std::fabs(sl - 1.0) <= 1e-3)) return fail(h, GVPM_ERR_INVALID_ARG, "frame entry: the tangent is a unit vector (to 1e-3)");
      alphaV = fr[3];
      if (!bsdfAlphaValid(b.exponent) || !bsdfAlphaValid(alphaV))
        return fail(h, GVPM_ERR_INVALID_ARG, "anisotropic Ward / rough conductor: alphaU, alphaV >= 1e-4");
    } else if (conductor && !bsdfAlphaValid(b.exponent)) {
      return fail(h, GVPM_ERR_INVALID_ARG, "rough conductor: alpha >= 1e-4 (the reference clamps it)");
    }
    if (ward) {
      if (!(0.5f * (b.exponent + alphaV) >= 0.05f) || !weightOk)
        return fail(h, GVPM_ERR_INVALID_ARG,
                    aniso ? "Ward: 0.5 (alphaU + alphaV) >= 0.05 (both components) and a sampling weight in [0, 1]"
                          : "Ward: alpha >= 0.05 (both components) and a sampling weight in [0, 1]");
      if (!bsdfWardVariantValid(b)) return fail(h, GVPM_ERR_UNSUPPORTED, "Ward: variant ward / ward-duer / balanced, both components");
    } else if (!bsdfMicrofacetValid(b)) {
      return fail(h, GVPM_ERR_UNSUPPORTED, "rough conductor: Beckmann, GGX or Phong / Ashikhmin-Shirley");
    } else if (!bsdfSampleVisibleValid(b)) {
      return fail(h, GVPM_ERR_INVALID_ARG, "rough conductor: the Phong / Ashikhmin-Shirley distribution samples all normals (sample_visible = 0)");
    }
  } else if (b.kind == GVPM_BSDF_ROUGHPLASTIC || b.kind == GVPM_BSDF_PLASTIC) {
    const bool rough = b.kind == GVPM_BSDF_ROUGHPLASTIC;
    if (rough && !bsdfAlphaValid(b.exponent)) return fail(h, GVPM_ERR_INVALID_ARG, "rough plastic: alpha >= 1e-4 (the reference clamps it)");
    if (rough && !bsdfMicrofacetValid(b)) return fail(h, GVPM_ERR_UNSUPPORTED, "rough plastic: Beckmann, GGX or Phong");
    if (rough && !bsdfSampleVisibleValid(b)) return fail(h, GVPM_ERR_INVALID_ARG, "rough plastic: the Phong / Ashikhmin-Shirley distribution samples all normals (sample_visible = 0)");
    if (!(b.eta[0] >= 1.f && b.eta[0] <= FLT_MAX) || !(b.eta[1] >= 0.f && b.eta[1] < 1.f) || !weightOk)
      return fail(h, GVPM_ERR_INVALID_ARG, "plastic: eta >= 1 and finite, Fdr in [0, 1), a sampling weight in [0, 1]");
    if (rough ? !(b.k[0] == 0.f || b.k[0] == 1.f || b.k[0] == 2.f) : b.k[0] != 2.f)
// ... 346 lines not shown
```

### gvpm_amd/csrc/near_lists.h

```cpp
#pragma once
#include <hip/hip_runtime.h>

#include "device_types.h"
#include "vec.h"

namespace gvpm {

__device__ __forceinline__ bool nearTriangle(f3 P, const float4 *tri4, uint32_t i, float dmax) {
  const float4 t0 = tri4[3 * (size_t)i], t1 = tri4[3 * (size_t)i + 1], t2 = tri4[3 * (size_t)i + 2];
  const f3 a = mk3(t0.x, t0.y, t0.z), b = mk3(t1.x, t1.y, t1.z), c = mk3(t2.x, t2.y, t2.z);
  const f3 n = mk3(t0.w, t1.w, t2.w);
  if (fabsf(dot(n, P - a)) > dmax * 1.0001f) return false;
  bool out = false;
#pragma unroll
  for (int k = 0; k < 3; ++k) {
    const float ak = comp(a, k), bk = comp(b, k), ck = comp(c, k), pk = comp(P, k);
    const float lo = ak + fminf(0.f, fminf(bk, ck)), hi = ak + fmaxf(0.f, fmaxf(bk, ck));
    if (pk < lo - dmax || pk > hi + dmax) out = true;
  }
  return !out;
}
template <int MODE, class F>
__device__ __forceinline__ void nearVisit(f3 P, const float4 *bvh, const float4 *tri4, uint32_t ntri, float dmax,
                                          const NearGrid &ng, F f) {
  if (MODE == 0) {
    for (uint32_t i = 0; i < ntri; ++i)
      if (nearTriangle(P, tri4, i, dmax)) f(i);
    return;
  }
  if (MODE == 2) {
    const float cx = (P.x - ng.org[0]) * ng.inv[0], cy = (P.y - ng.org[1]) * ng.inv[1], cz = (P.z - ng.org[2]) * ng.inv[2];
    if (!(cx >= 0.f && cy >= 0.f && cz >= 0.f && cx < (float)ng.dim[0] && cy < (float)ng.dim[1] && cz < (float)ng.dim[2])) return;
    const uint32_t c = ((uint32_t)cz * (uint32_t)ng.dim[1] + (uint32_t)cy) * (uint32_t)ng.dim[0] + (uint32_t)cx;
    const uint32_t e0 = ng.start[c], e1 = ng.start[c + 1];
    for (uint32_t e = e0; e < e1; ++e) {
      const uint32_t i = ng.tris[e];
      if (nearTriangle(P, tri4, i, dmax)) f(i);
    }
    return;
  }
  uint32_t stack[32];
  int sp = 0;
  uint32_t cur = 0;
  const float pad = dmax * 1.0001f;
  for (;;) {
    const float4 lo = bvh[2 * (size_t)cur], hi = bvh[2 * (size_t)cur + 1];
    bool descend = false;
    if (P.x >= lo.x - pad && P.x <= hi.x + pad && P.y >= lo.y - pad && P.y <= hi.y + pad && P.z >= lo.z - pad &&
        P.z <= hi.z + pad) {
      const uint32_t first = __float_as_uint(lo.w), count = __float_as_uint(hi.w);
      if (count == 0u) {
        if (sp < 32) stack[sp++] = first + 1u;
        cur = first;
        descend = true;
      } else {
        for (uint32_t i = first; i < first + count; ++i)
          if (nearTriangle(P, tri4, i, dmax)) f(i);
      }
    }
    if (!descend) {
      if (sp == 0) break;
      cur = stack[--sp];
    }
  }
}
__device__ __forceinline__ bool ownWall(f3 P, f3 pn, const float4 *tri4, uint32_t i, float eps, float &cstar) {
  const float4 t0 = tri4[3 * (size_t)i], t1 = tri4[3 * (size_t)i + 1], t2 = tri4[3 * (size_t)i + 2];
  const f3 a = mk3(t0.x, t0.y, t0.z), n = mk3(t0.w, t1.w, t2.w);
  const float tol = 1e-6f * (1.f + fabsf(P.x) + fabsf(P.y) + fabsf(P.z) + fabsf(a.x) + fabsf(a.y) + fabsf(a.z));
  const float align = dot(n, pn);
  if (!(fabsf(align) > 0.9999995f && fabsf(dot(n, P - a)) <= tol)) return false;
  const double e1x = t1.x, e1y = t1.y, e1z = t1.z, e2x = t2.x, e2y = t2.y, e2z = t2.z;
  const double nx = e1y * e2z - e1z * e2y, ny = e1z * e2x - e1x * e2z, nz = e1x * e2y - e1y * e2x;
  const double delta = nx * ((double)P.x - (double)a.x) + ny * ((double)P.y - (double)a.y) + nz * ((double)P.z - (double)a.z);
  const bool front = align > 0.f ? delta >= 0.0 : delta <= 0.0;
  if (!front) {
    const double nl = sqrt(nx * nx + ny * ny + nz * nz);
    if (nl > 0.0) cstar = fmaxf(cstar, (float)(fabs(delta) / (nl * (double)eps)) * 1.000001f);
  }
  return true;
}

template <int MODE>
__device__ __forceinline__ void nearOccluders(f3 P, f3 pn, const float4 *bvh, const float4 *tri4, uint32_t ntri, float dmax,
                                              const NearGrid &ng, uint32_t *ext, uint32_t extCap, float eps, uint32_t &w0, uint32_t &w1,
                                              uint32_t &w2, float &cstarOut) {
  w0 = w1 = w2 = 0xFFFFFFFFu;
  cstarOut = 0.f;
  if (ntri == 0u) return;
  const bool narrow = ntri <= GVPM_NEAR_NARROW_MAX, wide = !narrow && ntri <= GVPM_NEAR_WIDE_MAX;
  const uint32_t cap = narrow ? 12u : (wide ? 6u : 0u);
  uint32_t cnt = 0, a0 = 0xFFFFFFFFu, a1 = 0xFFFFFFFFu, a2 = 0xFFFFFFFFu;
  float cstar = 0.f;
  nearVisit<MODE>(P, bvh, tri4, ntri, dmax, ng, [&](uint32_t i) {
    if (ownWall(P, pn, tri4, i, eps, cstar)) return;
    if (cnt < cap) {
      uint32_t word, sh, m;
      if (narrow) { word = cnt >> 2; sh = 8u * (cnt & 3u); m = ~(0xFFu << sh); }
      else        { word = cnt >> 1; sh = 16u * (cnt & 1u); m = ~(0xFFFFu << sh); }
      const uint32_t v = i << sh;
      if (word == 0u) a0 = (a0 & m) | v;
      else if (word == 1u) a1 = (a1 & m) | v;
      else a2 = (a2 & m) | v;
    }
    cnt++;
  });
  cstarOut = cstar;
  const uint32_t capC = cstar > 0.f ? (cap * 2u) / 3u : cap;
  if (cnt <= capC) {
    w0 = a0; w1 = a1; w2 = cstar > 0.f ? __float_as_uint(cstar) : a2;
    return;
  }
  const uint32_t off = atomicAdd(ext, cnt + 1u);
  if ((unsigned long long)off + cnt + 1u > extCap) {
    w0 = 0xFEFFFFFFu;
    return;
  }
  ext[off] = cnt;
  uint32_t k = 0;
  float dummy = 0.f;
  nearVisit<MODE>(P, bvh, tri4, ntri, dmax, ng, [&](uint32_t i) {
    if (!ownWall(P, pn, tri4, i, eps, dummy)) ext[off + 1u + (k++)] = i;
  });
  w0 = 0xFDFFFFFFu;
  w1 = off;
  if (cstar > 0.f) w2 = __float_as_uint(cstar);
}

}
```

### gvpm_amd/csrc/photon_scatter.h

```cpp
#pragma once
#include <hip/hip_runtime.h>

#include "device_types.h"
#include "grid_cells.h"
#include "near_lists.h"
#include "shift_device.h"
#include "vec.h"

namespace gvpm {

struct RawPhotons {
  const float *pos, *wi, *flux, *parent_pos, *parent_n, *prefix_w, *parent_scat, *parent_wi;
  const float *parent_pdf, *edge_pdf, *parent_rr, *parent_g;
  const uint32_t *flags, *path_id;
};
inline RawPhotons rawOf(const gvpm_photon_soa &s) {
  return RawPhotons{s.pos,       s.wi,         s.flux,     s.parent_pos, s.parent_n, s.prefix_w, s.parent_scat,
                    s.parent_wi, s.parent_pdf, s.edge_pdf, s.parent_rr,  s.parent_g, s.flags,    s.path_id};
}

__device__ __forceinline__ float4 ld3(const float *p, uint32_t i, float w) {
  return make_float4(p[3 * (size_t)i], p[3 * (size_t)i + 1], p[3 * (size_t)i + 2], w);
}

struct ReorderLds {
  float4 stg[64][GVPM_REC_QUADS / 2 + 1];
  uint32_t dstIdx[64];
};
template <int MODE>
__device__ __forceinline__ void reorderBody(const RawPhotons &r, const uint32_t *__restrict__ keys,
                                            const uint32_t *__restrict__ rank,
                                            const uint32_t *__restrict__ cellStart, uint32_t n,
                                            const gvpm_params &cfg, const float4 *bvh, const float4 *tri4,
                                            uint32_t ntri, float dmax, const NearGrid &ng, uint32_t *nearExt,
                                            uint32_t extCap, float4 *hot, float4 *cold, uint32_t *overflow,
                                            uint32_t *origIdx, const uint32_t *__restrict__ sub, uint32_t ncells, uint32_t bid,
                                            uint32_t *counts, uint32_t *subCount, ReorderLds &L) {
  auto &stg = L.stg;
  auto &dstIdx = L.dstIdx;
  const uint32_t src = bid * 64u + threadIdx.x;
  const int t = threadIdx.x;
  constexpr int HALF = GVPM_REC_QUADS / 2;
  dstIdx[t] = 0xFFFFFFFFu;
  float4 q4 = make_float4(0.f, 0.f, 0.f, 0.f), q5 = q4, q6 = q4, q7 = q4;
  const bool live = src < n && (counts || rank[src] != 0xFFFFFFFFu);
  if (live) {
    uint32_t i;
    if (counts) i = cellStart[keys[src]] + (atomicSub(&counts[keys[src]], 1u) - 1u);
    else if (subCount) {
      const size_t sk = (size_t)(src % CELL_STRIPES) * ncells + keys[src];
      i = cellStart[keys[src]] + sub[sk] + (atomicSub(&subCount[sk], 1u) - 1u);
    } else i = cellStart[keys[src]] + rank[src] + (sub ? sub[(size_t)(src % CELL_STRIPES) * ncells + keys[src]] : 0u);
    uint32_t bits = r.flags[src] & ~((1u << 6) | (1u << GVPM_HOT_PARITY_BIT));
    if (photonContributes(bits, cfg)) bits |= 1u << 6;
    bits |= (r.path_id[src] & 1u) << GVPM_HOT_PARITY_BIT;
    const float4 h0 = ld3(r.pos, src, __uint_as_float(bits));
    hot[i] = h0;
    if (origIdx) origIdx[i] = src;
    stg[t][0] = h0;
    stg[t][1] = ld3(r.wi, src, r.parent_pdf[src]);
    stg[t][2] = ld3(r.flux, src, r.edge_pdf[src]);
    stg[t][3] = ld3(r.parent_pos, src, r.parent_rr[src]);
    q4 = ld3(r.parent_n, src, r.parent_g[src]);
    const f3 P = mk3(r.parent_pos[3 * (size_t)src], r.parent_pos[3 * (size_t)src + 1], r.parent_pos[3 * (size_t)src + 2]);
    uint32_t w0, w1, w2;
    const f3 PN = mk3(q4.x, q4.y, q4.z);
    float cstar;
    nearOccluders<MODE>(P, PN, bvh, tri4, ntri, dmax, ng, nearExt, extCap, cfg.epsilon, w0, w1, w2, cstar);
    if ((w0 >> 24) == 0xFEu) atomicAdd(overflow, 1u);
    stg[t][0].w = __uint_as_float((bits & ~(1u << 15)) | (cstar > 0.f ? 1u << 15 : 0u));
    q5 = ld3(r.prefix_w, src, __uint_as_float(w0));
    q6 = ld3(r.parent_scat, src, __uint_as_float(w1));
    q7 = ld3(r.parent_wi, src, __uint_as_float(w2));
    dstIdx[t] = i;
  }
  __syncthreads();
  for (int e = t; e < 64 * HALF; e += 64) {
    const int rec = e / HALF, part = e % HALF;
    const uint32_t i = dstIdx[rec];
    if (i != 0xFFFFFFFFu) cold[(size_t)i * GVPM_REC_QUADS + part] = stg[rec][part];
  }
  __syncthreads();
  if (live) {
    stg[t][0] = q4;
    stg[t][1] = q5;
    stg[t][2] = q6;
    stg[t][3] = q7;
  }
  __syncthreads();
  for (int e = t; e < 64 * HALF; e += 64) {
    const int rec = e / HALF, part = e % HALF;
    const uint32_t i = dstIdx[rec];
    if (i != 0xFFFFFFFFu) cold[(size_t)i * GVPM_REC_QUADS + HALF + part] = stg[rec][part];
  }
}

}
```

### gvpm_amd/csrc/tile_walk.h

```cpp
#pragma once
#include <hip/hip_runtime.h>

#include "bundle_grid.h"
#include "device_types.h"
#include "shift_device.h"
#include "vec.h"

namespace gvpm {

constexpr int STAGE = 256;
constexpr int QCAP = 128;
constexpr int PLAN_MAX_ITEMS = 256;

template <int B> struct RayTile {
  float4 ray4[5][3][B];
  float gop[5][B];
  float rnd[B];
  uint32_t pix[B];
  uint32_t edge[B];
};

template <int B> struct TileLds : RayTile<B> {
  double acc[27][B];
  float4 stage[STAGE];
// ... 60 lines not shown
                                                   int lane) {
  for (int idx = lane; idx < B * 20; idx += 64) {
    const int b = idx / 20, k = (idx % 20) / 4, q = idx % 4;
    float4 v = make_float4(0.f, 0.f, 0.f, 0.f);
    bool valid = false;
    if ((uint32_t)b < nb) {
      const uint32_t set = a.setPerm[setBase + b];
      const gvpm_camera_ray *ray = a.rays + (size_t)set * 5 + k;
      v = reinterpret_cast<const float4 *>(ray)[q];
      if (q == 0) valid = GVPM_RAY_VALID(ray->info) != 0;
    }
    if (q == 0) {
      const float l = fabsf(v.w);
      v.w = valid ? l : -fmaxf(l, 1e-30f);
      s.ray4[k][0][b] = v;
    } else if (q < 3) {
      s.ray4[k][q][b] = v;
    } else {
      s.gop[k][b] = v.x;
      if (k == 0) {
        s.rnd[b] = v.z;
        s.pix[b] = __float_as_uint(v.w);
        s.edge[b] = GVPM_RAY_EDGE(__float_as_uint(v.y));
      }
    }
  }
}

template <int B>
__device__ __forceinline__ void loadTileRays(const GatherArgs &a, RayTile<B> &s, uint32_t setBase, uint32_t nb,
                                             int lane) {
  loadTileRaysNoSync<B>(a, s, setBase, nb, lane);
  __syncthreads();
}

struct BaseInfo {
  float rnd;
  uint32_t pix, edge;
};
template <int B>
__device__ __forceinline__ RayReg loadBaseDirect(const GatherArgs &a, uint32_t setBase, uint32_t nb, int lane,
                                                 BaseInfo &bi) {
  RayReg r;
  r.o = r.d = r.eye = mk3(0.f);
  r.len = r.pdf = r.jac = r.gop = 0.f;
  r.valid = false;
  bi.rnd = 0.f;
  bi.pix = bi.edge = 0u;
  const int b = lane % B;
  if ((uint32_t)b < nb) {
    const uint32_t set = a.setPerm[setBase + b];
    const float4 *ray = reinterpret_cast<const float4 *>(a.rays + (size_t)set * 5);
    const float4 q0 = ray[0], q1 = ray[1], q2 = ray[2], q3 = ray[3];
    r.o = mk3(q0.x, q0.y, q0.z);
    r.len = fabsf(q0.w);
    r.d = mk3(q1.x, q1.y, q1.z);
    r.pdf = q1.w;
    r.eye = mk3(q2.x, q2.y, q2.z);
    r.jac = q2.w;
    r.gop = q3.x;
    const uint32_t info = __float_as_uint(q3.y);
    r.valid = GVPM_RAY_VALID(info) != 0;
    bi.edge = GVPM_RAY_EDGE(info);
    bi.rnd = q3.z;
    bi.pix = __float_as_uint(q3.w);
  }
  return r;
}

__device__ __forceinline__ void tileSetupFrom(const GatherArgs &a, const RayReg &base, bool valid, TileWalk &w);

template <int B>
__device__ __forceinline__ void tileSetup(const GatherArgs &a, const RayTile<B> &s, uint32_t nb, int lane,
                                          TileWalk &w) {
  const int b = lane % B;
  const RayReg base = loadRay(s, 0, b);
  tileSetupFrom(a, base, (uint32_t)b < nb && base.valid, w);
}

__device__ __forceinline__ void tileSetupFrom(const GatherArgs &a, const RayReg &base, bool valid, TileWalk &w) {
  w.base = base;
  w.beamValid = valid;
  w.bundleBad = false;
  if (a.grid.mode == 1) {
    float u = 0.f, v = 0.f;
    const bool ok = bundleRayUV(a.grid, base.o.x, base.o.y, base.o.z, base.d.x, base.d.y, base.d.z, u, v);
    w.bundleBad = __ballot(valid && !ok) != 0ull;
    w.bu0 = wave_min(valid ? u : INFINITY); w.bu1 = wave_max(valid ? u : -INFINITY);
    w.bv0 = wave_min(valid ? v : INFINITY); w.bv1 = wave_max(valid ? v : -INFINITY);
    w.any = w.bu0 <= w.bu1 && a.nph > 0 && !w.bundleBad;
    w.A = 0;
    w.cA0 = 0;
    w.cA1 = w.any ? a.grid.levels - 1 : -1;
    w.K = 1;
    w.dimA = a.grid.levels;
    w.pad = 0.f;
    return;
  }
  const float r = a.radius, eps = a.cfg.epsilon;
  const float mint = eps, maxt = w.base.len - eps;
  int A;
  {
    const float ax = fabsf(w.base.d.x), ay = fabsf(w.base.d.y), az = fabsf(w.base.d.z);
    const int my = (ax >= ay && ax >= az) ? 0 : (ay >= az ? 1 : 2);
    const int n0 = __popcll(__ballot(w.beamValid && my == 0));
    const int n1 = __popcll(__ballot(w.beamValid && my == 1));
    const int n2 = __popcll(__ballot(w.beamValid && my == 2));
    A = (n0 >= n1 && n0 >= n2) ? 0 : (n1 >= n2 ? 1 : 2);
  }
  w.A = A;
  const int U = (A + 1) % 3, V = (A + 2) % 3;
  w.oA = comp(w.base.o, A); w.dA = comp(w.base.d, A);
  w.oU = comp(w.base.o, U); w.dU = comp(w.base.d, U);
  w.oV = comp(w.base.o, V); w.dV = comp(w.base.d, V);
  const f3 org = mk3(a.grid.org[0], a.grid.org[1], a.grid.org[2]);
  w.orgA = comp(org, A); w.orgU = comp(org, U); w.orgV = comp(org, V);
  const int dimA = A == 0 ? a.grid.dim[0] : (A == 1 ? a.grid.dim[1] : a.grid.dim[2]);
  w.dimU = U == 0 ? a.grid.dim[0] : (U == 1 ? a.grid.dim[1] : a.grid.dim[2]);
  w.dimV = V == 0 ? a.grid.dim[0] : (V == 1 ? a.grid.dim[1] : a.grid.dim[2]);
  w.pad = r * 1.01f + 1e-6f;
  w.t0 = mint - 2.f * r;
  w.t1 = maxt + 2.f * r;
  float aLo = INFINITY, aHi = -INFINITY;
  if (w.beamValid) {
    const float e0 = w.oA + w.dA * w.t0, e1 = w.oA + w.dA * w.t1;
    aLo = fminf(e0, e1) - w.pad;
    aHi = fmaxf(e0, e1) + w.pad;
  }
  aLo = wave_min(aLo);
  aHi = wave_max(aHi);
  w.any = aLo <= aHi && a.nph > 0;
  w.cA0 = 1;
  w.cA1 = 0;
  w.dimA = dimA;
  if (w.any) {
    w.cA0 = min(max(0, (int)floorf((aLo - w.orgA) * a.grid.invCell)), dimA - 1);
    w.cA1 = min(max(0, (int)floorf((aHi - w.orgA) * a.grid.invCell)), dimA - 1);
  }
  w.K = (A == 0) ? (a.cfg.reserved[2] ? a.cfg.reserved[2] : 8) : (a.cfg.reserved[1] ? a.cfg.reserved[1] : 6);
}

struct TileCyl {
  f3 o, d;
  float R2, s0, s1;
  bool ok;
};
__device__ __forceinline__ TileCyl tileCylinder(const RayReg &base, bool valid, float tLo, float tHi, float rad, float slack) {
  TileCyl c;
  c.o = mk3(0.f);
  c.d = mk3(0.f, 0.f, 1.f);
  c.R2 = INFINITY;
  c.s0 = -INFINITY;
  c.s1 = INFINITY;
  c.ok = false;
  const float nv = (float)__popcll(__ballot(valid));
  f3 so = valid ? base.o : mk3(0.f), sd = valid ? base.d : mk3(0.f);
#pragma unroll
  for (int o = 32; o > 0; o >>= 1) {
    so.x += __shfl_xor(so.x, o, 64); so.y += __shfl_xor(so.y, o, 64); so.z += __shfl_xor(so.z, o, 64);
    sd.x += __shfl_xor(sd.x, o, 64); sd.y += __shfl_xor(sd.y, o, 64); sd.z += __shfl_xor(sd.z, o, 64);
  }
  const float dl = fsqrt(dot(sd, sd));
  if (!(nv > 0.f && dl > 0.5f * nv)) return c;
  c.o = so * frcp(nv);
  c.d = sd * frcp(dl);
  float rho2 = 0.f, s0 = INFINITY, s1 = -INFINITY;
  if (valid) {
#pragma unroll
    for (int e = 0; e < 2; ++e) {
      const f3 q = (base.o - c.o) + base.d * (e ? tHi : tLo);
      const float sq = dot(q, c.d);
      const f3 pq = q - c.d * sq;
      rho2 = fmaxf(rho2, dot(pq, pq));
      s0 = fminf(s0, sq);
      s1 = fmaxf(s1, sq);
    }
  }
  const float rho = fsqrt(wave_max(rho2));
  s0 = wave_min(s0);
  s1 = wave_max(s1);
  const float own = 4e-6f * (fabsf(c.o.x) + fabsf(c.o.y) + fabsf(c.o.z) + fabsf(s0) + fabsf(s1) + rho + rad) + slack;
  const float R = (rad + rho) * 1.0001f + own;
  c.R2 = R * R;
  c.s0 = s0 - rad * 1.0001f - own;
  c.s1 = s1 + rad * 1.0001f + own;
  c.ok = true;
  return c;
}
__device__ __forceinline__ bool insideCylinder(const TileCyl &c, f3 p) {
  const f3 wv = p - c.o;
  const float sq = dot(wv, c.d);
  return dot(wv, wv) - sq * sq < c.R2 && sq > c.s0 && sq < c.s1;
}

struct CellBox {
  int bx0, bx1, by0, by1, bz0, bz1;
};

struct BeamSlab {
  float oA, dA, oU, dU, oV, dV, t0, t1;
};
__device__ __forceinline__ bool beamFootprint(const BeamSlab &q, float lo, float hi, float pad, float &uLo, float &uHi,
                                              float &vLo, float &vHi) {
  float ta = q.t0, tb = q.t1;
  bool act = true;
  if (fabsf(q.dA) > 1e-12f) {
    const float inv = 1.f / q.dA;
    const float s0 = (lo - q.oA) * inv, s1 = (hi - q.oA) * inv;
    ta = fmaxf(ta, fminf(s0, s1));
    tb = fminf(tb, fmaxf(s0, s1));
    act = ta <= tb;
  } else {
    act = q.oA >= lo && q.oA <= hi;
  }
  if (!act) return false;
  const float u0 = q.oU + q.dU * ta, u1 = q.oU + q.dU * tb, v0 = q.oV + q.dV * ta, v1 = q.oV + q.dV * tb;
  uLo = fminf(u0, u1) - pad; uHi = fmaxf(u0, u1) + pad;
  vLo = fminf(v0, v1) - pad; vHi = fmaxf(v0, v1) + pad;
  return true;
}

__device__ __forceinline__ void slabRange(const GatherArgs &a, const TileWalk &w, int cA, int cAe, float &lo, float &hi) {
  lo = cA == 0 ? -INFINITY : w.orgA + cA * a.grid.cell - w.pad;
  hi = cAe == w.dimA - 1 ? INFINITY : w.orgA + (cAe + 1) * a.grid.cell + w.pad;
}

__device__ __forceinline__ bool boxFromFootprint(const GatherArgs &a, const TileWalk &w, int cA, int cAe, float uLo,
                                                 float uHi, float vLo, float vHi, CellBox &bx) {
  if (!(uLo <= uHi)) return false;
  const int cU0 = min(max(0, (int)floorf((uLo - w.orgU) * a.grid.invCell)), w.dimU - 1);
  const int cU1 = min(max(0, (int)floorf((uHi - w.orgU) * a.grid.invCell)), w.dimU - 1);
  const int cV0 = min(max(0, (int)floorf((vLo - w.orgV) * a.grid.invCell)), w.dimV - 1);
  const int cV1 = min(max(0, (int)floorf((vHi - w.orgV) * a.grid.invCell)), w.dimV - 1);
  const int A = w.A;
  bx.bx0 = A == 0 ? cA : (A == 1 ? cV0 : cU0); bx.bx1 = A == 0 ? cAe : (A == 1 ? cV1 : cU1);
  bx.by0 = A == 0 ? cU0 : (A == 1 ? cA : cV0); bx.by1 = A == 0 ? cU1 : (A == 1 ? cAe : cV1);
  bx.bz0 = A == 0 ? cV0 : (A == 1 ? cU0 : cA); bx.bz1 = A == 0 ? cV1 : (A == 1 ? cU1 : cAe);
  return true;
}

__device__ __forceinline__ bool slabBox(const GatherArgs &a, const TileWalk &w, int cA, int cAe, CellBox &bx) {
  if (a.grid.mode == 1) {
    const BundleBox b = bundleTileBox(a.grid, cA, w.bu0, w.bu1, w.bv0, w.bv1);
    bx.bx0 = b.x0; bx.bx1 = b.x1; bx.by0 = b.y0; bx.by1 = b.y1; bx.bz0 = bx.bz1 = b.z;
    return true;
  }
  float lo, hi;
  slabRange(a, w, cA, cAe, lo, hi);
  float uLo = INFINITY, uHi = -INFINITY, vLo = INFINITY, vHi = -INFINITY;
  if (w.beamValid) {
    const BeamSlab q{w.oA, w.dA, w.oU, w.dU, w.oV, w.dV, w.t0, w.t1};
    float a0, a1, b0, b1;
    if (beamFootprint(q, lo, hi, w.pad, a0, a1, b0, b1)) {
      uLo = a0; uHi = a1; vLo = b0; vHi = b1;
    }
  }
  uLo = wave_min(uLo); uHi = wave_max(uHi);
  vLo = wave_min(vLo); vHi = wave_max(vHi);
  return boxFromFootprint(a, w, cA, cAe, uLo, uHi, vLo, vHi, bx);
}

__device__ __forceinline__ uint2 packCellBox(const CellBox &bx) {
  return make_uint2((uint32_t)bx.bx0 | ((uint32_t)bx.bx1 << 10) | ((uint32_t)bx.by0 << 20),
                    (uint32_t)bx.by1 | ((uint32_t)bx.bz0 << 10) | ((uint32_t)bx.bz1 << 20));
}
__device__ __forceinline__ bool unpackCellBox(uint2 p, CellBox &bx) {
  bx.bx0 = (int)(p.x & 1023u); bx.bx1 = (int)((p.x >> 10) & 1023u); bx.by0 = (int)((p.x >> 20) & 1023u);
  bx.by1 = (int)(p.y & 1023u); bx.bz0 = (int)((p.y >> 10) & 1023u); bx.bz1 = (int)((p.y >> 20) & 1023u);
  return p.x != 0xFFFFFFFFu;
}

__device__ __forceinline__ void boxRange(const GatherArgs &a, const CellBox &bx, int ri, int nranges, uint32_t &start,
                                         uint32_t &count) {
  start = 0;
  count = 0;
  if (ri < nranges) {
    const int nyr = bx.by1 - bx.by0 + 1;
    const int y = bx.by0 + ri % nyr, z = bx.bz0 + ri / nyr;
    const uint32_t row = ((uint32_t)z * a.grid.dim[1] + y) * a.grid.dim[0];
    start = a.cellStart[row + bx.bx0];
    count = a.cellStart[row + bx.bx1 + 1] - start;
  }
}

__device__ __forceinline__ uint32_t boxCount(const GatherArgs &a, const CellBox &bx, int lane) {
  const int nranges = (bx.by1 - bx.by0 + 1) * (bx.bz1 - bx.bz0 + 1);
  uint32_t c = 0;
  for (int rbase = 0; rbase < nranges; rbase += 64) {
    uint32_t st, cnt;
    boxRange(a, bx, rbase + lane, nranges, st, cnt);
    c += cnt;
  }
#pragma unroll
  for (int o = 32; o > 0; o >>= 1) c += __shfl_xor(c, o, 64);
  return c;
}

template <int B, uint32_t PLAN_STAGE = 512> struct PlanLds {
  uint4 stItem[PLAN_STAGE];
  uint32_t stStaged[PLAN_STAGE];
  float pb[8][B];
  uint32_t pvalid[B];
};
template <int B, uint32_t PLAN_STAGE>
__device__ __forceinline__ void planBody(const GatherArgs &a, uint32_t ntiles, uint32_t target, uint4 *items, uint32_t *itemCount,
                                         uint2 *itemOff, uint32_t *blockTotal, uint32_t itemCap, uint32_t bid, uint32_t nblk,
                                         PlanLds<B, PLAN_STAGE> &L) {
  const bool splitHeavy = itemOff == nullptr;
  auto &pb = L.pb;
  auto &pvalid = L.pvalid;
  auto &stItem = L.stItem;
  auto &stStaged = L.stStaged;
  const int lane = threadIdx.x;
  uint32_t nStaged = 0;
  auto flush = [&]() {
    __syncthreads();
    for (uint32_t base = 0; base < nStaged; base += 64) {
      const uint32_t k = base + lane;
      const bool live = k < nStaged;
      const uint4 itv = live ? stItem[k] : make_uint4(0u, 0u, 0u, 0u);
      const uint32_t stg = live ? stStaged[k] : 0u;
      const uint32_t blocks = live ? (uint32_t)(((unsigned long long)stg * (itv.y & 0xFFu) + 63ull) / 64ull) : 0u;
      const uint32_t bIncl = wave_scan_incl(blocks, lane);
      const uint32_t bTotal = __shfl(bIncl, 63, 64);
      const uint32_t n = min(64u, nStaged - base);
      uint32_t slot0 = 0, blk0 = 0;
      if (lane == 0) {
        slot0 = atomicAdd(itemCount, n);
        if (itemOff) blk0 = atomicAdd(blockTotal, bTotal);
      }
      slot0 = __shfl(slot0, 0, 64);
      blk0 = __shfl(blk0, 0, 64);
      if (live && slot0 + lane < itemCap) {
        items[slot0 + lane] = itv;
        if (itemOff) itemOff[slot0 + lane] = make_uint2(blk0 + (bIncl - blocks), stg);
      }
    }
    nStaged = 0;
    __syncthreads();
  };
  for (uint32_t tile = bid; tile < ntiles; tile += nblk) {
  const uint32_t tileBeg = a.tileStart[tile], tileEnd = a.tileStart[tile + 1];
  for (uint32_t setBase = tileBeg; setBase < tileEnd; setBase += B) {
    const uint32_t nb = min((uint32_t)B, tileEnd - setBase);
    BaseInfo bi;
    const RayReg base = loadBaseDirect<B>(a, setBase, nb, lane, bi);
    TileWalk w;
    tileSetupFrom(a, base, base.valid, w);
    if (w.bundleBad && lane == 0 && a.bundleFlag) atomicOr(a.bundleFlag, 1u);
    if (!w.any) continue;
    __syncthreads();
    if (lane < B && a.grid.mode != 1) {
      pb[0][lane] = w.oA; pb[1][lane] = w.dA; pb[2][lane] = w.oU; pb[3][lane] = w.dU;
      pb[4][lane] = w.oV; pb[5][lane] = w.dV; pb[6][lane] = w.t0; pb[7][lane] = w.t1;
      pvalid[lane] = w.beamValid ? 1u : 0u;
    }
    __syncthreads();
    const int nsteps = (w.cA1 - w.cA0 + w.K) / w.K;
    for (int sbase = 0; sbase < nsteps; sbase += 64) {
      const int step = sbase + lane;
      const bool live = step < nsteps;
      const int cA = w.cA0 + step * w.K, cAe = min(cA + w.K - 1, w.cA1);
      uint32_t cnt = 0;
      if (live) {
        CellBox bx;
        bool haveBox;
        if (a.grid.mode == 1) {
          haveBox = slabBox(a, w, cA, cAe, bx);
        } else {
          float lo, hi;
          slabRange(a, w, cA, cAe, lo, hi);
          float uLo = INFINITY, uHi = -INFINITY, vLo = INFINITY, vHi = -INFINITY;
#pragma unroll 1
          for (uint32_t j = 0; j < nb; ++j) {
            if (!pvalid[j]) continue;
            const BeamSlab q{pb[0][j], pb[1][j], pb[2][j], pb[3][j], pb[4][j], pb[5][j], pb[6][j], pb[7][j]};
            float a0, a1, b0, b1;
            if (beamFootprint(q, lo, hi, w.pad, a0, a1, b0, b1)) {
              uLo = fminf(uLo, a0); uHi = fmaxf(uHi, a1);
              vLo = fminf(vLo, b0); vHi = fmaxf(vHi, b1);
            }
          }
          haveBox = boxFromFootprint(a, w, cA, cAe, uLo, uHi, vLo, vHi, bx);
        }
        if (a.planBoxes && (uint32_t)step < a.planBoxStride)
          a.planBoxes[(size_t)(setBase / B + tile) * a.planBoxStride + step] = haveBox ? packCellBox(bx) : make_uint2(0xFFFFFFFFu, 0u);
        if (haveBox) {
          const uint32_t nx1 = a.grid.dim[0] + 1, ny1 = a.grid.dim[1] + 1;
          const uint32_t *T = a.sat;
          const size_t z0 = (size_t)bx.bz0 * ny1, z1 = (size_t)(bx.bz1 + 1) * ny1;
          const uint32_t y0 = bx.by0, y1 = bx.by1 + 1, x0 = bx.bx0, x1 = bx.bx1 + 1;
          cnt = (T[(z1 + y1) * nx1 + x1] - T[(z1 + y1) * nx1 + x0] - T[(z1 + y0) * nx1 + x1] + T[(z1 + y0) * nx1 + x0]) -
                (T[(z0 + y1) * nx1 + x1] - T[(z0 + y1) * nx1 + x0] - T[(z0 + y0) * nx1 + x1] + T[(z0 + y0) * nx1 + x0]);
        }
      }
      const uint32_t incl = wave_scan_incl(cnt, lane);
      const uint32_t excl = incl - cnt;
      const uint32_t id = excl / target;
      const uint32_t idPrev = __shfl_up(id, 1, 64), idNext = __shfl_down(id, 1, 64);
      const bool first = live && (lane == 0 || id != idPrev);
      const bool liveNext = lane < 63 && step + 1 < nsteps;
      const bool closes = live && (!liveNext || idNext != id);
      const unsigned long long firstMask = __ballot(first);
      const unsigned long long below = firstMask & (lane == 63 ? ~0ull : ((2ull << lane) - 1ull));
      const int fl = below ? 63 - __clzll(below) : 0;
      const uint32_t exclFirst = __shfl(excl, fl, 64);
      const int cAFirst = __shfl(cA, fl, 64);
      const uint32_t staged = incl - exclFirst;
      const bool emit = closes && staged > 0u;
      const unsigned long long emitMask = __ballot(emit);
      if (emitMask && !splitHeavy && a.grid.mode == 1) {
        for (unsigned long long em = emitMask; em; em &= em - 1ull) {
          const int src = __ffsll((long long)em) - 1;
          const uint32_t stg = __shfl(staged, src, 64);
          const uint32_t cF = (uint32_t)__shfl(cAFirst, src, 64), cE = (uint32_t)__shfl(cAe, src, 64);
          const uint32_t wmax = stg / (uint32_t)STAGE + (cE - cF + 1u);
          uint32_t parts = stg > 2u * target ? min(PLAN_STAGE, (stg + target - 1u) / target) : 1u;
          parts = max(1u, min(parts, wmax));
          const uint32_t capP = parts > 1u ? min(stg, ((wmax + parts - 1u) / parts) * (uint32_t)STAGE) : stg;
          if (nStaged + parts > PLAN_STAGE) flush();
          for (uint32_t pp = (uint32_t)lane; pp < parts; pp += 64u) {
            stItem[nStaged + pp] = make_uint4(setBase, nb | ((setBase / B + tile) << 8), cF | (parts > 1u ? (pp << 8) | (parts << 20) : 0u), cE);
            stStaged[nStaged + pp] = capP;
          }
          nStaged += parts;
        }
      } else if (emitMask && !splitHeavy) {
        if (nStaged + 64u > PLAN_STAGE) flush();
        if (emit) {
          const uint32_t k = nStaged + (uint32_t)__popcll(emitMask & ((1ull << lane) - 1ull));
          stItem[k] = make_uint4(setBase, nb | ((setBase / B + tile) << 8), (uint32_t)cAFirst, (uint32_t)cAe);
          stStaged[k] = staged;
        }
        nStaged += (uint32_t)__popcll(emitMask);
      } else if (emitMask) {
        for (unsigned long long em = emitMask; em; em &= em - 1ull) {
          const int src = __ffsll((long long)em) - 1;
          const uint32_t stg = __shfl(staged, src, 64);
          const uint32_t cF = (uint32_t)__shfl(cAFirst, src, 64), cE = (uint32_t)__shfl(cAe, src, 64);
          const uint32_t parts = stg > 2u * target ? min(PLAN_STAGE, (stg + target - 1u) / target) : 1u;
          if (nStaged + parts > PLAN_STAGE) flush();
          for (uint32_t pp = (uint32_t)lane; pp < parts; pp += 64u) {
            stItem[nStaged + pp] = make_uint4(setBase, nb | (parts > 1u ? (pp << 8) | (parts << 20) : 0u), cF, cE);
            stStaged[nStaged + pp] = (stg + parts - 1u) / parts;
          }
          nStaged += parts;
        }
      }
    }
  }
  }
  if (nStaged) flush();
}
template <int B, uint32_t PLAN_STAGE> struct PlanLdsQ {
  uint4 stItem[PLAN_STAGE];
  uint32_t stStaged[PLAN_STAGE];
  float pb[64 / B][8][B];
  uint32_t pvalid[64 / B][B];
};
template <int B> __device__ __forceinline__ float group_min(float v) {
#pragma unroll
  for (int o = B / 2; o > 0; o >>= 1) v = fminf(v, __shfl_xor(v, o, 64));
  return v;
}
template <int B> __device__ __forceinline__ float group_max(float v) {
#pragma unroll
  for (int o = B / 2; o > 0; o >>= 1) v = fmaxf(v, __shfl_xor(v, o, 64));
  return v;
}
template <int B, uint32_t PLAN_STAGE>
__device__ __forceinline__ void planBodyQ(const GatherArgs &a, uint32_t ntiles, uint32_t target, uint4 *items, uint32_t *itemCount,
                                          uint2 *itemOff, uint32_t *blockTotal, uint32_t itemCap, uint32_t bid, uint32_t nblk,
                                          PlanLdsQ<B, PLAN_STAGE> &L) {
  constexpr int G = 64 / B;
  auto &stItem = L.stItem;
  auto &stStaged = L.stStaged;
  const int lane = threadIdx.x, q = lane / B, bl = lane % B;
  const unsigned long long gm = (B == 64 ? ~0ull : ((1ull << (B & 63)) - 1ull) << (q * B));
  uint32_t nStaged = 0;
  auto flush = [&]() {
    __syncthreads();
    for (uint32_t base = 0; base < nStaged; base += 64) {
      const uint32_t k = base + lane;
      const bool live = k < nStaged;
      const uint4 itv = live ? stItem[k] : make_uint4(0u, 0u, 0u, 0u);
      const uint32_t stg = live ? stStaged[k] : 0u;
      const uint32_t blocks = live ? (uint32_t)(((unsigned long long)stg * (itv.y & 0xFFu) + 63ull) / 64ull) : 0u;
      const uint32_t bIncl = wave_scan_incl(blocks, lane);
      const uint32_t bTotal = __shfl(bIncl, 63, 64);
      const uint32_t n = min(64u, nStaged - base);
      uint32_t slot0 = 0, blk0 = 0;
      if (lane == 0) {
        slot0 = atomicAdd(itemCount, n);
        blk0 = atomicAdd(blockTotal, bTotal);
      }
      slot0 = __shfl(slot0, 0, 64);
      blk0 = __shfl(blk0, 0, 64);
      if (live && slot0 + lane < itemCap) {
        items[slot0 + lane] = itv;
        itemOff[slot0 + lane] = make_uint2(blk0 + (bIncl - blocks), stg);
      }
    }
    nStaged = 0;
    __syncthreads();
  };
  const float r = a.radius, eps = a.cfg.epsilon;
  for (uint32_t t0 = bid; t0 < ntiles; t0 += nblk * G) {
    const uint32_t tile = t0 + (uint32_t)q * nblk;
    const bool haveTile = tile < ntiles;
    const uint32_t tileBeg = haveTile ? a.tileStart[tile] : 0u, tileEnd = haveTile ? a.tileStart[tile + 1] : 0u;
    for (uint32_t setBase = tileBeg; __ballot(setBase < tileEnd) != 0ull; setBase += B) {
      const uint32_t nb = setBase < tileEnd ? min((uint32_t)B, tileEnd - setBase) : 0u;
      BaseInfo bi;
      const RayReg base = loadBaseDirect<B>(a, setBase, nb, lane, bi);
      const bool beamValid = base.valid;
      int A;
      {
        const float ax = fabsf(base.d.x), ay = fabsf(base.d.y), az = fabsf(base.d.z);
        const int my = (ax >= ay && ax >= az) ? 0 : (ay >= az ? 1 : 2);
        const int n0 = __popcll(__ballot(beamValid && my == 0) & gm);
        const int n1 = __popcll(__ballot(beamValid && my == 1) & gm);
        const int n2 = __popcll(__ballot(beamValid && my == 2) & gm);
        A = (n0 >= n1 && n0 >= n2) ? 0 : (n1 >= n2 ? 1 : 2);
      }
      TileWalk w;
      w.base = base;
      w.beamValid = beamValid;
      w.bundleBad = false;
      w.A = A;
      const int U = (A + 1) % 3, V = (A + 2) % 3;
      w.oA = comp(base.o, A); w.dA = comp(base.d, A);
      w.oU = comp(base.o, U); w.dU = comp(base.d, U);
      w.oV = comp(base.o, V); w.dV = comp(base.d, V);
      const f3 org = mk3(a.grid.org[0], a.grid.org[1], a.grid.org[2]);
      w.orgA = comp(org, A); w.orgU = comp(org, U); w.orgV = comp(org, V);
      const int dimA = A == 0 ? a.grid.dim[0] : (A == 1 ? a.grid.dim[1] : a.grid.dim[2]);
      w.dimU = U == 0 ? a.grid.dim[0] : (U == 1 ? a.grid.dim[1] : a.grid.dim[2]);
      w.dimV = V == 0 ? a.grid.dim[0] : (V == 1 ? a.grid.dim[1] : a.grid.dim[2]);
      w.dimA = dimA;
      w.pad = r * 1.01f + 1e-6f;
      w.t0 = eps - 2.f * r;
      w.t1 = (base.len - eps) + 2.f * r;
      float aLo = INFINITY, aHi = -INFINITY;
      if (beamValid) {
        const float e0 = w.oA + w.dA * w.t0, e1 = w.oA + w.dA * w.t1;
        aLo = fminf(e0, e1) - w.pad;
        aHi = fmaxf(e0, e1) + w.pad;
      }
      aLo = group_min<B>(aLo);
      aHi = group_max<B>(aHi);
      w.any = aLo <= aHi && a.nph > 0;
      w.cA0 = 1;
      w.cA1 = 0;
      if (w.any) {
        w.cA0 = min(max(0, (int)floorf((aLo - w.orgA) * a.grid.invCell)), dimA - 1);
        w.cA1 = min(max(0, (int)floorf((aHi - w.orgA) * a.grid.invCell)), dimA - 1);
      }
      w.K = (A == 0) ? (a.cfg.reserved[2] ? a.cfg.reserved[2] : 8) : (a.cfg.reserved[1] ? a.cfg.reserved[1] : 6);
      if (__ballot(w.any) == 0ull) continue;
      __syncthreads();
      L.pb[q][0][bl] = w.oA; L.pb[q][1][bl] = w.dA; L.pb[q][2][bl] = w.oU; L.pb[q][3][bl] = w.dU;
      L.pb[q][4][bl] = w.oV; L.pb[q][5][bl] = w.dV; L.pb[q][6][bl] = w.t0; L.pb[q][7][bl] = w.t1;
      L.pvalid[q][bl] = beamValid ? 1u : 0u;
      __syncthreads();
      const int nsteps = w.any ? (w.cA1 - w.cA0 + w.K) / w.K : 0;
      int maxSteps = nsteps;
#pragma unroll
      for (int o = 32; o >= B; o >>= 1) maxSteps = max(maxSteps, __shfl_xor(maxSteps, o, 64));
      const uint32_t chunkOrd = setBase / B + tile;
      for (int sbase = 0; sbase < maxSteps; sbase += B) {
        const int step = sbase + bl;
        const bool live = step < nsteps;
        const int cA = w.cA0 + step * w.K, cAe = min(cA + w.K - 1, w.cA1);
        uint32_t cnt = 0;
        if (live) {
          CellBox bx;
          float lo, hi;
          slabRange(a, w, cA, cAe, lo, hi);
          float uLo = INFINITY, uHi = -INFINITY, vLo = INFINITY, vHi = -INFINITY;
#pragma unroll 1
          for (uint32_t j = 0; j < nb; ++j) {
            if (!L.pvalid[q][j]) continue;
            const BeamSlab qs{L.pb[q][0][j], L.pb[q][1][j], L.pb[q][2][j], L.pb[q][3][j], L.pb[q][4][j], L.pb[q][5][j], L.pb[q][6][j], L.pb[q][7][j]};
            float a0, a1, b0, b1;
            if (beamFootprint(qs, lo, hi, w.pad, a0, a1, b0, b1)) {
              uLo = fminf(uLo, a0); uHi = fmaxf(uHi, a1);
              vLo = fminf(vLo, b0); vHi = fmaxf(vHi, b1);
            }
          }
          const bool haveBox = boxFromFootprint(a, w, cA, cAe, uLo, uHi, vLo, vHi, bx);
          if (a.planBoxes && (uint32_t)step < a.planBoxStride)
            a.planBoxes[(size_t)chunkOrd * a.planBoxStride + step] = haveBox ? packCellBox(bx) : make_uint2(0xFFFFFFFFu, 0u);
          if (haveBox) {
            const uint32_t nx1 = a.grid.dim[0] + 1, ny1 = a.grid.dim[1] + 1;
            const uint32_t *T = a.sat;
            const size_t z0 = (size_t)bx.bz0 * ny1, z1 = (size_t)(bx.bz1 + 1) * ny1;
            const uint32_t y0 = bx.by0, y1 = bx.by1 + 1, x0 = bx.bx0, x1 = bx.bx1 + 1;
            cnt = (T[(z1 + y1) * nx1 + x1] - T[(z1 + y1) * nx1 + x0] - T[(z1 + y0) * nx1 + x1] + T[(z1 + y0) * nx1 + x0]) -
                  (T[(z0 + y1) * nx1 + x1] - T[(z0 + y1) * nx1 + x0] - T[(z0 + y0) * nx1 + x1] + T[(z0 + y0) * nx1 + x0]);
          }
        }
        uint32_t incl = cnt;
#pragma unroll
        for (int o = 1; o < B; o <<= 1) {
          const uint32_t nv = __shfl_up(incl, o, 64);
          if (bl >= o) incl += nv;
        }
        const uint32_t excl = incl - cnt;
        const uint32_t id = excl / target;
        const uint32_t idPrev = __shfl_up(id, 1, 64), idNext = __shfl_down(id, 1, 64);
        const bool first = live && (bl == 0 || id != idPrev);
        const bool liveNext = bl < B - 1 && step + 1 < nsteps;
        const bool closes = live && (!liveNext || idNext != id);
        const unsigned long long firstMask = __ballot(first) & gm;
        const unsigned long long below = firstMask & (lane == 63 ? ~0ull : ((2ull << lane) - 1ull));
        const int fl = below ? 63 - __clzll(below) : lane;
        const uint32_t exclFirst = __shfl(excl, fl, 64);
        const int cAFirst = __shfl(cA, fl, 64);
        const uint32_t staged = incl - exclFirst;
        const bool emit = closes && staged > 0u;
        const unsigned long long emitMask = __ballot(emit);
        if (emitMask) {
          if (nStaged + 64u > PLAN_STAGE) flush();
          if (emit) {
            const uint32_t k = nStaged + (uint32_t)__popcll(emitMask & ((1ull << lane) - 1ull));
            stItem[k] = make_uint4(setBase, nb | (chunkOrd << 8), (uint32_t)cAFirst, (uint32_t)cAe);
            stStaged[k] = staged;
          }
          nStaged += (uint32_t)__popcll(emitMask);
        }
      }
    }
  }
  if (nStaged) flush();
}

template <int B>
__global__ __launch_bounds__(64) void plan_kernel(GatherArgs a, uint32_t ntiles, uint32_t target, uint4 *items,
                                                  uint32_t *itemCount, uint2 *itemOff, uint32_t *blockTotal,
                                                  uint32_t itemCap) {
  __shared__ PlanLds<B, 512> L;
  planBody<B, 512>(a, ntiles, target, items, itemCount, itemOff, blockTotal, itemCap, blockIdx.x, gridDim.x, L);
}

}
```

Measured before the change: 6538 Mevals/s.

## Add scalar-load near-occluder scan and reduce register pressure in plan bodies

Adds a scalar (uniform address space) triangle scan mode for small meshes, so triangle data is read via scalar loads instead of per-lane vector loads. The scan is selected by default through a new nearScalar flag. Plan bodies now hoist wave-uniform values with readfirstlane and recompute lane-derived values behind opaque asm to shorten live ranges. SAT lookups use 32-bit byte offsets instead of size_t index arithmetic. This aims to cut VGPR pressure and vector memory traffic in the tail and reorder kernels, at the cost of extra recomputation and a preprocessor-gated debug split.

```diff
diff --git a/gvpm_amd/csrc/build_chain.hip b/gvpm_amd/csrc/build_chain.hip
--- a/gvpm_amd/csrc/build_chain.hip
+++ b/gvpm_amd/csrc/build_chain.hip
@@ -274,18 +274,24 @@
 template <int B, int MODE> __global__ __launch_bounds__(64) __attribute__((amdgpu_waves_per_eu(TAIL_WPE, TAIL_WPE))) void chain_tail_kernel(GatherArgs a, TailArgs t) {
   __shared__ __attribute__((aligned(16))) unsigned char ldsRaw[tailLdsBytes<B>()];
   const uint32_t b = blockIdx.x, pslot = b / t.every;
+#if !defined(GVPM_TAIL_ONLY) || GVPM_TAIL_ONLY == 1
   if (b % t.every == 0u && pslot < t.nPlan) {
     if (a.grid.mode != 1 && t.planGroups)
       planBodyQ<B, TAIL_PLAN_STAGE>(a, t.ntiles, t.target, t.items, t.itemCount, t.itemOff, t.blockTotal, t.itemCap, pslot, t.nPlan,
                                     *reinterpret_cast<PlanLdsQ<B, TAIL_PLAN_STAGE> *>(ldsRaw));
     else
-      planBody<B, TAIL_PLAN_STAGE>(a, t.ntiles, t.target, t.items, t.itemCount, t.itemOff, t.blockTotal, t.itemCap, pslot, t.nPlan,
+      planBody<B, TAIL_PLAN_STAGE, true>(a, t.ntiles, t.target, t.items, t.itemCount, t.itemOff, t.blockTotal, t.itemCap, pslot, t.nPlan,
                                    *reinterpret_cast<PlanLds<B, TAIL_PLAN_STAGE> *>(ldsRaw));
   }
   else
+#endif
+#if !defined(GVPM_TAIL_ONLY) || GVPM_TAIL_ONLY == 2
     reorderBody<MODE>(t.raw, t.keys, t.rank, t.cellStart, t.n, a.cfg, a.bvh, a.tri4, a.ntri, t.dmax, t.ng, t.nearExt, t.extCap, t.hot,
                       t.cold, t.overflow, t.origIdx, t.sub, t.ncells, b - min(t.nPlan, (b + t.every - 1u) / t.every), t.counts,
                       t.subCount, *reinterpret_cast<ReorderLds *>(ldsRaw));
+#else
+    (void)0;
+#endif
   if (!lastBlockArrives(t.ctl, blockIdx.x, gridDim.x)) return;
   if (threadIdx.x == 0) {
     t.hostOut[0] = coherentRead(t.blockTotal);
@@ -310,15 +316,16 @@
 
 template <int B>
 static void launchTail(int mode, uint32_t grid, hipStream_t s, const GatherArgs &a, const TailArgs &t) {
-  if (mode == 0) hipLaunchKernelGGL((chain_tail_kernel<B, 0>), dim3(grid), dim3(64), 0, s, a, t);
-  else if (mode == 2) hipLaunchKernelGGL((chain_tail_kernel<B, 2>), dim3(grid), dim3(64), 0, s, a, t);
-  else hipLaunchKernelGGL((chain_tail_kernel<B, 1>), dim3(grid), dim3(64), 0, s, a, t);
+  if (mode == NEAR_SCAN_SCALAR) hipLaunchKernelGGL((chain_tail_kernel<B, NEAR_SCAN_SCALAR>), dim3(grid), dim3(64), 0, s, a, t);
+  else if (mode == NEAR_SCAN_VECTOR) hipLaunchKernelGGL((chain_tail_kernel<B, NEAR_SCAN_VECTOR>), dim3(grid), dim3(64), 0, s, a, t);
+  else if (mode == NEAR_GRID) hipLaunchKernelGGL((chain_tail_kernel<B, NEAR_GRID>), dim3(grid), dim3(64), 0, s, a, t);
+  else hipLaunchKernelGGL((chain_tail_kernel<B, NEAR_BVH>), dim3(grid), dim3(64), 0, s, a, t);
 }
 
 void launch_build_chain(ChainArgs c, const GatherArgs &a, const gvpm_photon_soa &raw, int beamsPerWave, uint32_t target, uint4 *items,
                         uint2 *itemOff, uint32_t itemCap, float dmax, const NearGrid &ng, uint32_t extCap, uint32_t *origIdx,
                         uint32_t *hostOut, bool initBuckets, hipStream_t s, uint32_t pairCapBlocks, uint32_t unitCap, uint32_t unitPairs,
-                        bool fullVis, bool planGroups) {
+                        bool fullVis, bool planGroups, bool nearScalar) {
   c.nPhBlocks = (c.n + 255u) / 256u;
   c.nBeamBlocks = (c.nsets + 255u) / 256u;
   if (initBuckets) hipLaunchKernelGGL(chain_init_buckets_kernel, dim3(1), dim3(768), 0, s, c.buckets);
@@ -372,7 +379,7 @@
   t.unitCap = unitCap;
   t.unitPairs = unitPairs ? unitPairs : 1u;
   t.fullVis = fullVis ? 1u : 0u;
-  const int mode = a.ntri <= 64u ? 0 : (ng.start ? 2 : 1);
+  const int mode = nearMode(a.ntri, ng, nearScalar);
   const uint32_t grid = t.nPlan + (c.n + 63u) / 64u;
   t.every = std::max(1u, grid / std::max(1u, t.nPlan));
   switch (beamsPerWave) {
diff --git a/gvpm_amd/csrc/context.h b/gvpm_amd/csrc/context.h
--- a/gvpm_amd/csrc/context.h
+++ b/gvpm_amd/csrc/context.h
@@ -29,7 +29,7 @@
 void launch_reorder(const gvpm_photon_soa &raw, const uint32_t *keys, const uint32_t *rank, const uint32_t *cellStart,
                     uint32_t n, const gvpm_params &cfg, const float4 *bvh, const float4 *tri4, uint32_t ntri, float dmax,
                     const NearGrid &ng, uint32_t *nearExt, uint32_t extCap, float4 *hot, float4 *cold, uint32_t *overflow,
-                    uint32_t *origIdx, const uint32_t *sub, uint32_t ncells, hipStream_t s);
+                    uint32_t *origIdx, const uint32_t *sub, uint32_t ncells, hipStream_t s, bool nearScalar = true);
 void launch_near_grid(const float4 *tri4, uint32_t ntri, const NearGrid &g, float reach, uint32_t *counts, uint32_t *tris, int mode,
                       hipStream_t s);
 void launch_segment_start(const uint32_t *keys, uint32_t n, uint32_t nseg, uint32_t shift, uint32_t *start,
@@ -51,7 +51,7 @@
 void launch_build_chain(ChainArgs c, const GatherArgs &a, const gvpm_photon_soa &raw, int beamsPerWave, uint32_t target, uint4 *items,
                         uint2 *itemOff, uint32_t itemCap, float dmax, const NearGrid &ng, uint32_t extCap, uint32_t *origIdx,
                         uint32_t *hostOut, bool initBuckets, hipStream_t s, uint32_t pairCapBlocks = 0xFFFFFFFFu, uint32_t unitCap = 0,
-                        uint32_t unitPairs = 1, bool fullVis = false, bool planGroups = true);
+                        uint32_t unitPairs = 1, bool fullVis = false, bool planGroups = true, bool nearScalar = true);
 void launch_apply_host_shifts(const GatherArgs &a, const gvpm_host_shift *results, uint32_t n, hipStream_t s);
 void launch_plan_bre(const GatherArgs &a, int beamsPerWave, uint32_t ntiles, uint32_t target, uint4 *items,
                      uint32_t *itemCount, uint2 *itemOff, uint32_t *blockTotal, uint32_t itemCap, hipStream_t stream);
@@ -297,6 +297,7 @@
   NearGrid nearGrid;
   float nearGridReach = -1.f;
   bool useNearGrid = true;
+  bool nearScalar = true;
 
   struct PhotonSlot {
     DevBuf<uint32_t> raw;
diff --git a/gvpm_amd/csrc/drivers_bre.hip b/gvpm_amd/csrc/drivers_bre.hip
--- a/gvpm_amd/csrc/drivers_bre.hip
+++ b/gvpm_amd/csrc/drivers_bre.hip
@@ -227,7 +227,7 @@
                        !h->bs->bucketsInit, h->bstream,
                        optimistic ? (refuse ? 0u : (uint32_t)std::min<size_t>((h->bs->pairs.cap - 64u) / 64u, 0xFFFFFFF0u)) : 0xFFFFFFFFu,
                        optimistic && h->evalUnits ? (uint32_t)std::min<size_t>(h->bs->units.cap / 2u, 0x3FFFFFFFu) : 0u, eval_unit_pairs(),
-                       fullVisOpt, h->planGroups);
+                       fullVisOpt, h->planGroups, h->nearScalar);
     h->bs->bucketsInit = true;
     s.chainRan = true;
     if (optimistic) {
diff --git a/gvpm_amd/csrc/drivers_build.hip b/gvpm_amd/csrc/drivers_build.hip
--- a/gvpm_amd/csrc/drivers_build.hip
+++ b/gvpm_amd/csrc/drivers_build.hip
@@ -318,7 +318,7 @@
   }
   launch_reorder(h->rawDev, h->bs->keysA.p, h->bs->valsA.p, h->bs->cellStart.p, n, h->cfg, h->bvh.p, h->tri4.p, h->ntri, dmax,
                  h->nearGrid, h->bs->nearExt.p, (uint32_t)std::min<size_t>(h->bs->nearExt.cap, 0xFFFFFF00u), h->bs->hot.p,
-                 h->bs->cold.p, h->bs->overflowCtr.p, wantOrig ? h->bs->origIdx.p : nullptr, sub, g.ncells, h->bstream);
+                 h->bs->cold.p, h->bs->overflowCtr.p, wantOrig ? h->bs->origIdx.p : nullptr, sub, g.ncells, h->bstream, h->nearScalar);
   HIP_TRY(h, hipGetLastError());
   h->nearOverflow = false;
   if (!deferred && h->cfg.visibility_as_written) {
diff --git a/gvpm_amd/csrc/grid_build.hip b/gvpm_amd/csrc/grid_build.hip
--- a/gvpm_amd/csrc/grid_build.hip
+++ b/gvpm_amd/csrc/grid_build.hip
@@ -282,14 +282,17 @@
 void launch_reorder(const gvpm_photon_soa &raw, const uint32_t *keys, const uint32_t *rank, const uint32_t *cellStart,
                     uint32_t n, const gvpm_params &cfg, const float4 *bvh, const float4 *tri4, uint32_t ntri, float dmax,
                     const NearGrid &ng, uint32_t *nearExt, uint32_t extCap, float4 *hot, float4 *cold, uint32_t *overflow,
-                    uint32_t *origIdx, const uint32_t *sub, uint32_t ncells, hipStream_t s) {
+                    uint32_t *origIdx, const uint32_t *sub, uint32_t ncells, hipStream_t s, bool nearScalar) {
   const RawPhotons r = rawOf(raw);
 #define GVPM_REORDER(M) \
   hipLaunchKernelGGL(reorder_kernel<M>, dim3((n + 63) / 64), dim3(64), 0, s, r, keys, rank, cellStart, n, cfg, bvh, tri4, ntri, \
                      dmax, ng, nearExt, extCap, hot, cold, overflow, origIdx, sub, ncells)
-  if (ntri <= 64u) GVPM_REORDER(0);
-  else if (ng.start) GVPM_REORDER(2);
-  else GVPM_REORDER(1);
+  switch (nearMode(ntri, ng, nearScalar)) {
+    case NEAR_SCAN_SCALAR: GVPM_REORDER(NEAR_SCAN_SCALAR); break;
+    case NEAR_SCAN_VECTOR: GVPM_REORDER(NEAR_SCAN_VECTOR); break;
+    case NEAR_GRID: GVPM_REORDER(NEAR_GRID); break;
+    default: GVPM_REORDER(NEAR_BVH); break;
+  }
 #undef GVPM_REORDER
 }
 
diff --git a/gvpm_amd/csrc/gvpm_api.hip b/gvpm_amd/csrc/gvpm_api.hip
--- a/gvpm_amd/csrc/gvpm_api.hip
+++ b/gvpm_amd/csrc/gvpm_api.hip
@@ -119,6 +119,7 @@
   if (!h->pipeline && !getenv("GVPM_WAVES_PER_CU") && h->ncu) h->nwaves = std::min<uint32_t>(h->ncu * 12u, GVPM_STAT_ROWS);
   if (const char *e = getenv("GVPM_PERSISTENT")) h->persistentEval = (atoi(e) & 1) != 0, h->persistentTrav = (atoi(e) & 2) != 0;
   if (const char *e = getenv("GVPM_NEAR_GRID")) h->useNearGrid = atoi(e) != 0;
+  if (const char *e = getenv("GVPM_NEAR_SCALAR")) h->nearScalar = atoi(e) != 0;
   if (const char *e = getenv("GVPM_TRAV_STREAM")) h->travStream = atoi(e) != 0;
   if (const char *e = getenv("GVPM_BEAMS_FP64")) h->beamsExact = atoi(e) != 0;
   if (const char *e = getenv("GVPM_BEAMS_FREE_CONE")) h->beamsFreeCone = atoi(e) != 0;
diff --git a/gvpm_amd/csrc/near_lists.h b/gvpm_amd/csrc/near_lists.h
--- a/gvpm_amd/csrc/near_lists.h
+++ b/gvpm_amd/csrc/near_lists.h
@@ -6,8 +6,23 @@
 
 namespace gvpm {
 
-__device__ __forceinline__ bool nearTriangle(f3 P, const float4 *tri4, uint32_t i, float dmax) {
-  const float4 t0 = tri4[3 * (size_t)i], t1 = tri4[3 * (size_t)i + 1], t2 = tri4[3 * (size_t)i + 2];
+
+struct Tri3 {
+  float4 t0, t1, t2;
+};
+__device__ __forceinline__ Tri3 loadTri(const float4 *tri4, uint32_t i) {
+  return Tri3{tri4[3 * (size_t)i], tri4[3 * (size_t)i + 1], tri4[3 * (size_t)i + 2]};
+}
+typedef const __attribute__((address_space(4))) float *UniformF32;
+__device__ __forceinline__ UniformF32 uniformView(const float4 *tri4) {
+  return (UniformF32)(reinterpret_cast<const float *>(tri4));
+}
+__device__ __forceinline__ Tri3 loadTriUniform(UniformF32 tab, uint32_t i) {
+  const UniformF32 p = tab + 12u * (size_t)i;
+  return Tri3{make_float4(p[0], p[1], p[2], p[3]), make_float4(p[4], p[5], p[6], p[7]), make_float4(p[8], p[9], p[10], p[11])};
+}
+__device__ __forceinline__ bool nearTriangle(f3 P, const Tri3 &t, float dmax) {
+  const float4 t0 = t.t0, t1 = t.t1, t2 = t.t2;
   const f3 a = mk3(t0.x, t0.y, t0.z), b = mk3(t1.x, t1.y, t1.z), c = mk3(t2.x, t2.y, t2.z);
   const f3 n = mk3(t0.w, t1.w, t2.w);
   if (fabsf(dot(n, P - a)) > dmax * 1.0001f) return false;
@@ -20,10 +35,18 @@
   }
   return !out;
 }
+__device__ __forceinline__ bool nearTriangle(f3 P, const float4 *tri4, uint32_t i, float dmax) {
+  return nearTriangle(P, loadTri(tri4, i), dmax);
+}
+constexpr int NEAR_SCAN_SCALAR = 0, NEAR_BVH = 1, NEAR_GRID = 2, NEAR_SCAN_VECTOR = 3;
+inline int nearMode(uint32_t ntri, const NearGrid &ng, bool scalarScan) {
+  return ntri <= 64u ? (scalarScan ? NEAR_SCAN_SCALAR : NEAR_SCAN_VECTOR) : (ng.start ? NEAR_GRID : NEAR_BVH);
+}
 template <int MODE, class F>
 __device__ __forceinline__ void nearVisit(f3 P, const float4 *bvh, const float4 *tri4, uint32_t ntri, float dmax,
                                           const NearGrid &ng, F f) {
-  if (MODE == 0) {
+  static_assert(MODE != NEAR_SCAN_SCALAR, "the scalar scan is nearOccluders' own loop");
+  if (MODE == NEAR_SCAN_VECTOR) {
     for (uint32_t i = 0; i < ntri; ++i)
       if (nearTriangle(P, tri4, i, dmax)) f(i);
     return;
@@ -64,12 +87,16 @@
     }
   }
 }
-__device__ __forceinline__ bool ownWall(f3 P, f3 pn, const float4 *tri4, uint32_t i, float eps, float &cstar) {
-  const float4 t0 = tri4[3 * (size_t)i], t1 = tri4[3 * (size_t)i + 1], t2 = tri4[3 * (size_t)i + 2];
+struct OwnWall {
+  bool own;
+  float cstar;
+};
+__device__ __forceinline__ OwnWall ownWall(f3 P, f3 pn, const Tri3 &t, float eps, float cstar) {
+  const float4 t0 = t.t0, t1 = t.t1, t2 = t.t2;
   const f3 a = mk3(t0.x, t0.y, t0.z), n = mk3(t0.w, t1.w, t2.w);
   const float tol = 1e-6f * (1.f + fabsf(P.x) + fabsf(P.y) + fabsf(P.z) + fabsf(a.x) + fabsf(a.y) + fabsf(a.z));
   const float align = dot(n, pn);
-  if (!(fabsf(align) > 0.9999995f && fabsf(dot(n, P - a)) <= tol)) return false;
+  if (!(fabsf(align) > 0.9999995f && fabsf(dot(n, P - a)) <= tol)) return OwnWall{false, cstar};
   const double e1x = t1.x, e1y = t1.y, e1z = t1.z, e2x = t2.x, e2y = t2.y, e2z = t2.z;
   const double nx = e1y * e2z - e1z * e2y, ny = e1z * e2x - e1x * e2z, nz = e1x * e2y - e1y * e2x;
   const double delta = nx * ((double)P.x - (double)a.x) + ny * ((double)P.y - (double)a.y) + nz * ((double)P.z - (double)a.z);
@@ -78,53 +105,80 @@
     const double nl = sqrt(nx * nx + ny * ny + nz * nz);
     if (nl > 0.0) cstar = fmaxf(cstar, (float)(fabs(delta) / (nl * (double)eps)) * 1.000001f);
   }
-  return true;
+  return OwnWall{true, cstar};
 }
 
+struct NearScan {
+  uint32_t cnt, a0, a1, a2;
+  float cstar;
+};
+__device__ __forceinline__ NearScan nearAppend(NearScan s, f3 P, f3 pn, const Tri3 &t, uint32_t i, float eps, bool narrow, uint32_t cap) {
+  const OwnWall o = ownWall(P, pn, t, eps, s.cstar);
+  s.cstar = o.cstar;
+  if (o.own) return s;
+  if (s.cnt < cap) {
+    uint32_t word, sh, m;
+    if (narrow) { word = s.cnt >> 2; sh = 8u * (s.cnt & 3u); m = ~(0xFFu << sh); }
+    else        { word = s.cnt >> 1; sh = 16u * (s.cnt & 1u); m = ~(0xFFFFu << sh); }
+    const uint32_t v = i << sh;
+    if (word == 0u) s.a0 = (s.a0 & m) | v;
+    else if (word == 1u) s.a1 = (s.a1 & m) | v;
+    else s.a2 = (s.a2 & m) | v;
+  }
+  s.cnt++;
+  return s;
+}
+
+struct NearList {
+  uint32_t w0, w1, w2;
+  float cstar;
+};
 template <int MODE>
-__device__ __forceinline__ void nearOccluders(f3 P, f3 pn, const float4 *bvh, const float4 *tri4, uint32_t ntri, float dmax,
-                                              const NearGrid &ng, uint32_t *ext, uint32_t extCap, float eps, uint32_t &w0, uint32_t &w1,
-                                              uint32_t &w2, float &cstarOut) {
-  w0 = w1 = w2 = 0xFFFFFFFFu;
-  cstarOut = 0.f;
-  if (ntri == 0u) return;
-  const bool narrow = ntri <= GVPM_NEAR_NARROW_MAX, wide = !narrow && ntri <= GVPM_NEAR_WIDE_MAX;
+__device__ __forceinline__ NearList nearOccluders(f3 P, f3 pn, const float4 *bvh, const float4 *tri4, uint32_t ntri, float dmax,
+                                                  const NearGrid &ng, uint32_t *ext, uint32_t extCap, float eps) {
+  NearList r{0xFFFFFFFFu, 0xFFFFFFFFu, 0xFFFFFFFFu, 0.f};
+  if (ntri == 0u) return r;
+  constexpr bool LINEAR = MODE == NEAR_SCAN_SCALAR || MODE == NEAR_SCAN_VECTOR;
+  const bool narrow = LINEAR || ntri <= GVPM_NEAR_NARROW_MAX, wide = !narrow && ntri <= GVPM_NEAR_WIDE_MAX;
   const uint32_t cap = narrow ? 12u : (wide ? 6u : 0u);
-  uint32_t cnt = 0, a0 = 0xFFFFFFFFu, a1 = 0xFFFFFFFFu, a2 = 0xFFFFFFFFu;
-  float cstar = 0.f;
-  nearVisit<MODE>(P, bvh, tri4, ntri, dmax, ng, [&](uint32_t i) {
-    if (ownWall(P, pn, tri4, i, eps, cstar)) return;
-    if (cnt < cap) {
-      uint32_t word, sh, m;
-      if (narrow) { word = cnt >> 2; sh = 8u * (cnt & 3u); m = ~(0xFFu << sh); }
-      else        { word = cnt >> 1; sh = 16u * (cnt & 1u); m = ~(0xFFFFu << sh); }
-      const uint32_t v = i << sh;
-      if (word == 0u) a0 = (a0 & m) | v;
-      else if (word == 1u) a1 = (a1 & m) | v;
-      else a2 = (a2 & m) | v;
+  NearScan s{0u, 0xFFFFFFFFu, 0xFFFFFFFFu, 0xFFFFFFFFu, 0.f};
+  if constexpr (MODE == NEAR_SCAN_SCALAR) {
+    const UniformF32 tab = uniformView(tri4);
+    for (uint32_t i = 0; i < ntri; ++i) {
+      const Tri3 t = loadTriUniform(tab, i);
+      if (nearTriangle(P, t, dmax)) s = nearAppend(s, P, pn, t, i, eps, narrow, cap);
     }
-    cnt++;
-  });
-  cstarOut = cstar;
+  } else {
+    nearVisit<MODE>(P, bvh, tri4, ntri, dmax, ng, [&](uint32_t i) { s = nearAppend(s, P, pn, loadTri(tri4, i), i, eps, narrow, cap); });
+  }
+  const float cstar = s.cstar;
+  r.cstar = cstar;
   const uint32_t capC = cstar > 0.f ? (cap * 2u) / 3u : cap;
-  if (cnt <= capC) {
-    w0 = a0; w1 = a1; w2 = cstar > 0.f ? __float_as_uint(cstar) : a2;
-    return;
+  if (s.cnt <= capC) {
+    r.w0 = s.a0; r.w1 = s.a1; r.w2 = cstar > 0.f ? __float_as_uint(cstar) : s.a2;
+    return r;
   }
-  const uint32_t off = atomicAdd(ext, cnt + 1u);
-  if ((unsigned long long)off + cnt + 1u > extCap) {
-    w0 = 0xFEFFFFFFu;
-    return;
+  const uint32_t off = atomicAdd(ext, s.cnt + 1u);
+  if ((unsigned long long)off + s.cnt + 1u > extCap) {
+    r.w0 = 0xFEFFFFFFu;
+    return r;
   }
-  ext[off] = cnt;
+  ext[off] = s.cnt;
   uint32_t k = 0;
-  float dummy = 0.f;
-  nearVisit<MODE>(P, bvh, tri4, ntri, dmax, ng, [&](uint32_t i) {
-    if (!ownWall(P, pn, tri4, i, eps, dummy)) ext[off + 1u + (k++)] = i;
-  });
-  w0 = 0xFDFFFFFFu;
-  w1 = off;
-  if (cstar > 0.f) w2 = __float_as_uint(cstar);
+  if constexpr (MODE == NEAR_SCAN_SCALAR) {
+    for (uint32_t i = 0; i < ntri; ++i) {
+      const Tri3 t = loadTri(tri4, i);
+      if (nearTriangle(P, t, dmax) && !ownWall(P, pn, t, eps, 0.f).own) ext[off + 1u + (k++)] = i;
+    }
+  } else {
+    nearVisit<MODE>(P, bvh, tri4, ntri, dmax, ng, [&](uint32_t i) {
+      if (!ownWall(P, pn, loadTri(tri4, i), eps, 0.f).own) ext[off + 1u + (k++)] = i;
+    });
+  }
+  r.w0 = 0xFDFFFFFFu;
+  r.w1 = off;
+  if (cstar > 0.f) r.w2 = __float_as_uint(cstar);
+  return r;
 }
 
 }
diff --git a/gvpm_amd/csrc/photon_scatter.h b/gvpm_amd/csrc/photon_scatter.h
--- a/gvpm_amd/csrc/photon_scatter.h
+++ b/gvpm_amd/csrc/photon_scatter.h
@@ -63,10 +63,10 @@
     stg[t][3] = ld3(r.parent_pos, src, r.parent_rr[src]);
     q4 = ld3(r.parent_n, src, r.parent_g[src]);
     const f3 P = mk3(r.parent_pos[3 * (size_t)src], r.parent_pos[3 * (size_t)src + 1], r.parent_pos[3 * (size_t)src + 2]);
-    uint32_t w0, w1, w2;
     const f3 PN = mk3(q4.x, q4.y, q4.z);
-    float cstar;
-    nearOccluders<MODE>(P, PN, bvh, tri4, ntri, dmax, ng, nearExt, extCap, cfg.epsilon, w0, w1, w2, cstar);
+    const NearList nl = nearOccluders<MODE>(P, PN, bvh, tri4, ntri, dmax, ng, nearExt, extCap, cfg.epsilon);
+    const uint32_t w0 = nl.w0, w1 = nl.w1, w2 = nl.w2;
+    const float cstar = nl.cstar;
     if ((w0 >> 24) == 0xFEu) atomicAdd(overflow, 1u);
     stg[t][0].w = __uint_as_float((bits & ~(1u << 15)) | (cstar > 0.f ? 1u << 15 : 0u));
     q5 = ld3(r.prefix_w, src, __uint_as_float(w0));
diff --git a/gvpm_amd/csrc/tile_walk.h b/gvpm_amd/csrc/tile_walk.h
--- a/gvpm_amd/csrc/tile_walk.h
+++ b/gvpm_amd/csrc/tile_walk.h
@@ -386,7 +386,15 @@
   float pb[8][B];
   uint32_t pvalid[B];
 };
-template <int B, uint32_t PLAN_STAGE>
+__device__ __forceinline__ float uniformF32(float x) { return __uint_as_float(__builtin_amdgcn_readfirstlane(__float_as_uint(x))); }
+__device__ __forceinline__ int opaqueLane(int lane) {
+  asm volatile("" : "+v"(lane));
+  return lane;
+}
+__device__ __forceinline__ uint32_t ldU32At(const uint32_t *base, uint32_t byteOff) {
+  return *reinterpret_cast<const uint32_t *>(reinterpret_cast<const char *>(base) + byteOff);
+}
+template <int B, uint32_t PLAN_STAGE, bool LEAN = false>
 __device__ __forceinline__ void planBody(const GatherArgs &a, uint32_t ntiles, uint32_t target, uint4 *items, uint32_t *itemCount,
                                          uint2 *itemOff, uint32_t *blockTotal, uint32_t itemCap, uint32_t bid, uint32_t nblk,
                                          PlanLds<B, PLAN_STAGE> &L) {
@@ -431,6 +439,12 @@
     const RayReg base = loadBaseDirect<B>(a, setBase, nb, lane, bi);
     TileWalk w;
     tileSetupFrom(a, base, base.valid, w);
+    if constexpr (LEAN) {
+      const float r = a.radius, eps = a.cfg.epsilon;
+      w.pad = uniformF32(r * 1.01f + 1e-6f);
+      w.t0 = uniformF32(eps - 2.f * r);
+      w.t1 = (w.base.len - eps) + uniformF32(2.f * r);
+    }
     if (w.bundleBad && lane == 0 && a.bundleFlag) atomicOr(a.bundleFlag, 1u);
     if (!w.any) continue;
     __syncthreads();
@@ -480,13 +494,14 @@
       }
       const uint32_t incl = wave_scan_incl(cnt, lane);
       const uint32_t excl = incl - cnt;
+      const int ln = LEAN ? opaqueLane(lane) : lane;
       const uint32_t id = excl / target;
       const uint32_t idPrev = __shfl_up(id, 1, 64), idNext = __shfl_down(id, 1, 64);
-      const bool first = live && (lane == 0 || id != idPrev);
-      const bool liveNext = lane < 63 && step + 1 < nsteps;
+      const bool first = live && (ln == 0 || id != idPrev);
+      const bool liveNext = ln < 63 && step + 1 < nsteps;
       const bool closes = live && (!liveNext || idNext != id);
       const unsigned long long firstMask = __ballot(first);
-      const unsigned long long below = firstMask & (lane == 63 ? ~0ull : ((2ull << lane) - 1ull));
+      const unsigned long long below = firstMask & (ln == 63 ? ~0ull : ((2ull << ln) - 1ull));
       const int fl = below ? 63 - __clzll(below) : 0;
       const uint32_t exclFirst = __shfl(excl, fl, 64);
       const int cAFirst = __shfl(cA, fl, 64);
@@ -512,7 +527,7 @@
       } else if (emitMask && !splitHeavy) {
         if (nStaged + 64u > PLAN_STAGE) flush();
         if (emit) {
-          const uint32_t k = nStaged + (uint32_t)__popcll(emitMask & ((1ull << lane) - 1ull));
+          const uint32_t k = nStaged + (uint32_t)__popcll(emitMask & ((1ull << ln) - 1ull));
           stItem[k] = make_uint4(setBase, nb | ((setBase / B + tile) << 8), (uint32_t)cAFirst, (uint32_t)cAe);
           stStaged[k] = staged;
         }
@@ -559,8 +574,8 @@
   constexpr int G = 64 / B;
   auto &stItem = L.stItem;
   auto &stStaged = L.stStaged;
-  const int lane = threadIdx.x, q = lane / B, bl = lane % B;
-  const unsigned long long gm = (B == 64 ? ~0ull : ((1ull << (B & 63)) - 1ull) << (q * B));
+  const int lane = threadIdx.x;
+  auto groupMask = [](int q) { return B == 64 ? ~0ull : ((1ull << (B & 63)) - 1ull) << (q * B); };
   uint32_t nStaged = 0;
   auto flush = [&]() {
     __syncthreads();
@@ -589,14 +604,17 @@
     __syncthreads();
   };
   const float r = a.radius, eps = a.cfg.epsilon;
+  const float padU = uniformF32(r * 1.01f + 1e-6f), t0U = uniformF32(eps - 2.f * r), r2U = uniformF32(2.f * r);
   for (uint32_t t0 = bid; t0 < ntiles; t0 += nblk * G) {
-    const uint32_t tile = t0 + (uint32_t)q * nblk;
+    const uint32_t tile = t0 + (uint32_t)(opaqueLane(lane) / B) * nblk;
     const bool haveTile = tile < ntiles;
     const uint32_t tileBeg = haveTile ? a.tileStart[tile] : 0u, tileEnd = haveTile ? a.tileStart[tile + 1] : 0u;
     for (uint32_t setBase = tileBeg; __ballot(setBase < tileEnd) != 0ull; setBase += B) {
       const uint32_t nb = setBase < tileEnd ? min((uint32_t)B, tileEnd - setBase) : 0u;
       BaseInfo bi;
       const RayReg base = loadBaseDirect<B>(a, setBase, nb, lane, bi);
+      const int ln1 = opaqueLane(lane), q = ln1 / B, bl = ln1 % B;
+      const unsigned long long gm = groupMask(q);
       const bool beamValid = base.valid;
       int A;
       {
@@ -622,9 +640,9 @@
       w.dimU = U == 0 ? a.grid.dim[0] : (U == 1 ? a.grid.dim[1] : a.grid.dim[2]);
       w.dimV = V == 0 ? a.grid.dim[0] : (V == 1 ? a.grid.dim[1] : a.grid.dim[2]);
       w.dimA = dimA;
-      w.pad = r * 1.01f + 1e-6f;
-      w.t0 = eps - 2.f * r;
-      w.t1 = (base.len - eps) + 2.f * r;
+      w.pad = padU;
+      w.t0 = t0U;
+      w.t1 = (base.len - eps) + r2U;
       float aLo = INFINITY, aHi = -INFINITY;
       if (beamValid) {
         const float e0 = w.oA + w.dA * w.t0, e1 = w.oA + w.dA * w.t1;
@@ -653,6 +671,7 @@
       for (int o = 32; o >= B; o >>= 1) maxSteps = max(maxSteps, __shfl_xor(maxSteps, o, 64));
       const uint32_t chunkOrd = setBase / B + tile;
       for (int sbase = 0; sbase < maxSteps; sbase += B) {
+        const int ln2 = opaqueLane(lane), q = ln2 / B, bl = ln2 % B;
         const int step = sbase + bl;
         const bool live = step < nsteps;
         const int cA = w.cA0 + step * w.K, cAe = min(cA + w.K - 1, w.cA1);
@@ -678,27 +697,30 @@
           if (haveBox) {
             const uint32_t nx1 = a.grid.dim[0] + 1, ny1 = a.grid.dim[1] + 1;
             const uint32_t *T = a.sat;
-            const size_t z0 = (size_t)bx.bz0 * ny1, z1 = (size_t)(bx.bz1 + 1) * ny1;
-            const uint32_t y0 = bx.by0, y1 = bx.by1 + 1, x0 = bx.bx0, x1 = bx.bx1 + 1;
-            cnt = (T[(z1 + y1) * nx1 + x1] - T[(z1 + y1) * nx1 + x0] - T[(z1 + y0) * nx1 + x1] + T[(z1 + y0) * nx1 + x0]) -
-                  (T[(z0 + y1) * nx1 + x1] - T[(z0 + y1) * nx1 + x0] - T[(z0 + y0) * nx1 + x1] + T[(z0 + y0) * nx1 + x0]);
+            const uint32_t z0 = (uint32_t)bx.bz0 * ny1, z1 = (uint32_t)(bx.bz1 + 1) * ny1;
+            const uint32_t y0 = bx.by0, y1 = bx.by1 + 1, x0 = 4u * (uint32_t)bx.bx0, x1 = 4u * (uint32_t)(bx.bx1 + 1);
+            const uint32_t r11 = (z1 + y1) * nx1 * 4u, r10 = (z1 + y0) * nx1 * 4u, r01 = (z0 + y1) * nx1 * 4u, r00 = (z0 + y0) * nx1 * 4u;
+            cnt = (ldU32At(T, r11 + x1) - ldU32At(T, r11 + x0) - ldU32At(T, r10 + x1) + ldU32At(T, r10 + x0)) -
+                  (ldU32At(T, r01 + x1) - ldU32At(T, r01 + x0) - ldU32At(T, r00 + x1) + ldU32At(T, r00 + x0));
           }
         }
+        const int ln3 = opaqueLane(lane), bl3 = ln3 % B;
+        const unsigned long long gm3 = groupMask(ln3 / B);
         uint32_t incl = cnt;
 #pragma unroll
         for (int o = 1; o < B; o <<= 1) {
           const uint32_t nv = __shfl_up(incl, o, 64);
-          if (bl >= o) incl += nv;
+          if (bl3 >= o) incl += nv;
         }
         const uint32_t excl = incl - cnt;
         const uint32_t id = excl / target;
         const uint32_t idPrev = __shfl_up(id, 1, 64), idNext = __shfl_down(id, 1, 64);
-        const bool first = live && (bl == 0 || id != idPrev);
-        const bool liveNext = bl < B - 1 && step + 1 < nsteps;
+        const bool first = live && (bl3 == 0 || id != idPrev);
+        const bool liveNext = bl3 < B - 1 && step + 1 < nsteps;
         const bool closes = live && (!liveNext || idNext != id);
-        const unsigned long long firstMask = __ballot(first) & gm;
-        const unsigned long long below = firstMask & (lane == 63 ? ~0ull : ((2ull << lane) - 1ull));
-        const int fl = below ? 63 - __clzll(below) : lane;
+        const unsigned long long firstMask = __ballot(first) & gm3;
+        const unsigned long long below = firstMask & (ln3 == 63 ? ~0ull : ((2ull << ln3) - 1ull));
+        const int fl = below ? 63 - __clzll(below) : ln3;
         const uint32_t exclFirst = __shfl(excl, fl, 64);
         const int cAFirst = __shfl(cA, fl, 64);
         const uint32_t staged = incl - exclFirst;
@@ -707,7 +729,7 @@
         if (emitMask) {
           if (nStaged + 64u > PLAN_STAGE) flush();
           if (emit) {
-            const uint32_t k = nStaged + (uint32_t)__popcll(emitMask & ((1ull << lane) - 1ull));
+            const uint32_t k = nStaged + (uint32_t)__popcll(emitMask & ((1ull << ln3) - 1ull));
             stItem[k] = make_uint4(setBase, nb | (chunkOrd << 8), (uint32_t)cAFirst, (uint32_t)cAe);
             stStaged[k] = staged;
           }
```

Result: faster. 6746 Mevals/s (median of 6 runs) (+3.2%).
